# liruiluo/VLA-Adapter

Measured on AMD Instinct MI355X. Metric: fine-tune samples/sec (224px img + 32-tok prompt), adapter-only, fwd+bwd+AdamW, higher is better.
Workload: dtype bf16

## Files before the change

### vla_adapter_amd/csrc/gemm_tn.hip

```cpp
#include <algorithm>
#include "gemm_epilogue.h"
#include "gemm_params.h"

namespace {

constexpr int TBK = 64;
constexpr int TILE_BYTES = TBK * 256;
constexpr int STAGE_BYTES = 2 * TILE_BYTES;
constexpr int LDS_BYTES = 2 * STAGE_BYTES;

struct TnP {
  const bf16_t* A; const bf16_t* B; bf16_t* C; const bf16_t* R; float* ws;
  int M, N1, N2, lda, ldb, ldc, ldr;
  long long sA, sB, sC, sR;
  float alpha;
  int gA, gB; long long sgA, sgB;
  int cgA, cgsA;
  int tiles_n2, ntiles, split, mslice;
};

__device__ __forceinline__ bf16x4 tr_read(const char* p) {
  return __builtin_amdgcn_ds_read_tr16_b64_v4i16((__attribute__((address_space(3))) bf16x4*)p);
}

__device__ __forceinline__ void tn_tile(const TnP& p, const int swz, const int bz, char* smem) {
  const int tid = threadIdx.x, lane = tid & 63;
  const int wid = __builtin_amdgcn_readfirstlane(tid >> 6);
  const int wr = wid >> 2, wc = wid & 3;
  const int b1 = swz / p.tiles_n2, b2 = swz - b1 * p.tiles_n2;
  const int n1_0 = b1 * 128, n2_0 = b2 * 128;
  const int zb = bz / p.split, zs = bz - zb * p.split;
  const int m_begin = zs * p.mslice, m_end = min(p.M, m_begin + p.mslice);
  const int nt = (m_end - m_begin + TBK - 1) / TBK;
  const char* Ab = reinterpret_cast<const char*>(p.A + (long long)zb * p.sA);
  const char* Bb = reinterpret_cast<const char*>(p.B + (long long)zb * p.sB);

  const bool isA = wid < 4;
  const int ld = isA ? p.lda : p.ldb, ncols = isA ? p.N1 : p.N2, c0 = isA ? n1_0 : n2_0;
  const int grp = isA ? p.gA : p.gB;
  const long long sgrp = isA ? p.sgA : p.sgB;
  const char* base = isA ? Ab : Bb;
  int rloc[4];
  long long coff[4];
#pragma unroll
  for (int i = 0; i < 4; ++i) {
    const int qp = (wid & 3) * 4 + i;
    const int r = 4 * qp + (lane >> 4);
    const int f = ((r & 3) << 2) | ((r >> 2) & 3);
    int col = c0 + (((lane & 15) ^ f) << 3);
    col = min(col, ncols - 8);
    if (isA && p.cgA > 0) col = (col / p.cgA) * p.cgsA + col % p.cgA;
    rloc[i] = r;
    coff[i] = (long long)col * 2;
  }
  auto stage = [&](int buf, int t) {
    const int mt = m_begin + t * TBK;
    const long long tb = grouped_row(mt, grp, sgrp, ld);
    const int lim = m_end - 1 - mt;
    char* dst = smem + buf * STAGE_BYTES + (isA ? 0 : TILE_BYTES) + (wid & 3) * 4096;
#pragma unroll
    for (int i = 0; i < 4; ++i) glds16(base + (tb + (long long)min(rloc[i], lim) * ld) * 2 + coff[i], dst + i * 1024);
  };

  const int kq = lane >> 4, qq = (lane >> 2) & 3, pp = lane & 3;
  int fa[4][2], fb[2][2];
#pragma unroll
  for (int e = 0; e < 2; ++e) {
    const int row = 8 * kq + qq + 4 * e, f = (qq << 2) | ((2 * kq + e) & 3);
#pragma unroll
    for (int i = 0; i < 4; ++i) fa[i][e] = 256 * row + ((((wr * 64 + i * 16) >> 3) + (pp >> 1)) ^ f) * 16 + 8 * (pp & 1);
#pragma unroll
    for (int i = 0; i < 2; ++i) fb[i][e] = TILE_BYTES + 256 * row + ((((wc * 32 + i * 16) >> 3) + (pp >> 1)) ^ f) * 16 + 8 * (pp & 1);
  }

  f32x4 acc[2][4];
#pragma unroll
  for (int a = 0; a < 2; ++a)
#pragma unroll
    for (int b = 0; b < 4; ++b) acc[a][b] = f32x4{0.f, 0.f, 0.f, 0.f};

  if (nt > 0) stage(0, 0);
  int buf = 0;
  for (int t = 0; t < nt; ++t) {
    asm volatile("s_waitcnt vmcnt(0)" ::: "memory");
    __builtin_amdgcn_s_barrier();
    asm volatile("" ::: "memory");
    if (t + 1 < nt) stage(buf ^ 1, t + 1);
    const char* sb = smem + buf * STAGE_BYTES;
    const int valid = m_end - (m_begin + t * TBK);
    bf16x8 fm[2][4], fn[2][2];
#pragma unroll
    for (int ks = 0; ks < 2; ++ks) {
#pragma unroll
      for (int i = 0; i < 4; ++i) {
        const bf16x4 lo = tr_read(sb + ks * 8192 + fa[i][0]), hi = tr_read(sb + ks * 8192 + fa[i][1]);
        fm[ks][i] = bf16x8{lo[0], lo[1], lo[2], lo[3], hi[0], hi[1], hi[2], hi[3]};
      }
#pragma unroll
      for (int i = 0; i < 2; ++i) {
        const bf16x4 lo = tr_read(sb + ks * 8192 + fb[i][0]), hi = tr_read(sb + ks * 8192 + fb[i][1]);
        fn[ks][i] = bf16x8{lo[0], lo[1], lo[2], lo[3], hi[0], hi[1], hi[2], hi[3]};
      }
    }
    if (valid < TBK) {
#pragma unroll
      for (int ks = 0; ks < 2; ++ks)
#pragma unroll
        for (int e = 0; e < 8; ++e)
          if (ks * 32 + 8 * kq + e >= valid) {
#pragma unroll
            for (int i = 0; i < 2; ++i) fn[ks][i][e] = 0;
          }
    }
#pragma unroll
    for (int ks = 0; ks < 2; ++ks)
#pragma unroll
      for (int ni = 0; ni < 2; ++ni)
#pragma unroll
        for (int mi = 0; mi < 4; ++mi)
          acc[ni][mi] = __builtin_amdgcn_mfma_f32_16x16x32_bf16(fn[ks][ni], fm[ks][mi], acc[ni][mi], 0, 0, 0);
    buf ^= 1;
  }

  const int w1 = n1_0 + wr * 64, w2 = n2_0 + wc * 32;
  const int lq = lane >> 4, lr = lane & 15;
  if (p.ws != nullptr) {
    float* plane = p.ws + ((long long)bz) * p.N1 * p.N2;
#pragma unroll
    for (int ni = 0; ni < 2; ++ni)
#pragma unroll
      for (int mi = 0; mi < 4; ++mi) {
        const int r = w1 + mi * 16 + lr, c = w2 + ni * 16 + lq * 4;
        if (r < p.N1 && c + 3 < p.N2) *reinterpret_cast<f32x4*>(plane + (long long)r * p.N2 + c) = acc[ni][mi];
      }
    return;
  }
  bf16_t* Cb = p.C + (long long)zb * p.sC;
  const bf16_t* Rb = p.R ? p.R + (long long)zb * p.sR : nullptr;
#pragma unroll
  for (int ni = 0; ni < 2; ++ni)
#pragma unroll
    for (int mi = 0; mi < 4; ++mi) {
      const int r = w1 + mi * 16 + lr, c = w2 + ni * 16 + lq * 4;
      if (r >= p.N1 || c + 3 >= p.N2) continue;
      float v[4];
#pragma unroll
      for (int j = 0; j < 4; ++j) v[j] = acc[ni][mi][j] * p.alpha;
      if (Rb) add_residual4(v, *reinterpret_cast<const uint2*>(Rb + (long long)r * p.ldr + c));
      *reinterpret_cast<uint2*>(Cb + (long long)r * p.ldc + c) = pack4(v);
    }
}

constexpr int T2_HT = 16384;
constexpr int T2_LDS = 8 * T2_HT;

#define TN_MMA_QUADRANT(Q, FN, FM)                                                                             \
  do {                                                                                                         \
    _Pragma("unroll") for (int ks = 0; ks < 2; ++ks)                                                           \
      _Pragma("unroll") for (int ni = 0; ni < 2; ++ni)                                                         \
        _Pragma("unroll") for (int mi = 0; mi < 4; ++mi)                                                       \
          Q[ni][mi] = __builtin_amdgcn_mfma_f32_16x16x32_bf16(FN[ks][ni], FM[ks][mi], Q[ni][mi], 0, 0, 0);     \
  } while (0)

__device__ __forceinline__ void tn256_tile(const TnP& p, const int swz, const int zb, char* smem) {
  const int tid = threadIdx.x, lane = tid & 63;
  const int wid = __builtin_amdgcn_readfirstlane(tid >> 6);
  const int wr = wid >> 2, wc = wid & 3;
  const int b1 = swz / p.tiles_n2, b2 = swz - b1 * p.tiles_n2;
  const int n1_0 = b1 * 256, n2_0 = b2 * 256;
  const int nt = (p.M + TBK - 1) / TBK;
  const char* Ab = reinterpret_cast<const char*>(p.A + (long long)zb * p.sA);
  const char* Bb = reinterpret_cast<const char*>(p.B + (long long)zb * p.sB);

  const int r0 = wid * 8 + (lane >> 4);
  unsigned ca[2][2], cb[2][2];
#pragma unroll
  for (int j = 0; j < 2; ++j) {
    const int r = r0 + 4 * j;
    const int f = ((r & 3) << 2) | ((r >> 2) & 3);
    const int lc = ((lane & 15) ^ f) << 3;
#pragma unroll
    for (int h = 0; h < 2; ++h) {
      int ga = n1_0 + (lc >> 6) * 128 + h * 64 + (lc & 63);
      ga = min(ga, p.N1 - 8);
      if (p.cgA > 0) ga = (ga / p.cgA) * p.cgsA + ga % p.cgA;
      ca[h][j] = (unsigned)ga * 2u;
      const int gb = min(n2_0 + (lc >> 5) * 64 + h * 32 + (lc & 31), p.N2 - 8);
      cb[h][j] = (unsigned)gb * 2u;
    }
  }
  const unsigned wdst = (unsigned)(size_t)((__attribute__((address_space(3))) char*)smem) + wid * 2048;
  auto stage_a = [&](int slot, int h, int t) {
    const int mt = t * TBK;
    const char* base = Ab + grouped_row(mt, p.gA, p.sgA, p.lda) * 2;
    const unsigned lim = (unsigned)(p.M - 1 - mt), ld2 = (unsigned)p.lda * 2u;
    glds16s(base, min((unsigned)r0, lim) * ld2 + ca[h][0], wdst + slot * T2_HT);
    glds16s(base, min((unsigned)r0 + 4u, lim) * ld2 + ca[h][1], wdst + slot * T2_HT + 1024);
  };
  auto stage_b = [&](int slot, int h, int t) {
    const int mt = t * TBK;
    const char* base = Bb + grouped_row(mt, p.gB, p.sgB, p.ldb) * 2;
    const unsigned lim = (unsigned)(p.M - 1 - mt), ld2 = (unsigned)p.ldb * 2u;
    glds16s(base, min((unsigned)r0, lim) * ld2 + cb[h][0], wdst + slot * T2_HT);
    glds16s(base, min((unsigned)r0 + 4u, lim) * ld2 + cb[h][1], wdst + slot * T2_HT + 1024);
  };

  const int kq = lane >> 4, qq = (lane >> 2) & 3, pp = lane & 3;
  int fa[4][2], fb[2][2];
#pragma unroll
  for (int e = 0; e < 2; ++e) {
    const int row = 8 * kq + qq + 4 * e, f = (qq << 2) | ((2 * kq + e) & 3);
#pragma unroll
    for (int i = 0; i < 4; ++i) fa[i][e] = 256 * row + ((((wr * 64 + i * 16) >> 3) + (pp >> 1)) ^ f) * 16 + 8 * (pp & 1);
#pragma unroll
    for (int i = 0; i < 2; ++i) fb[i][e] = 256 * row + ((((wc * 32 + i * 16) >> 3) + (pp >> 1)) ^ f) * 16 + 8 * (pp & 1);
  }
  auto read_a = [&](const char* sb, bf16x8 (&fm)[2][4]) {
#pragma unroll
    for (int ks = 0; ks < 2; ++ks)
#pragma unroll
      for (int i = 0; i < 4; ++i) {
        const bf16x4 lo = tr_read(sb + ks * 8192 + fa[i][0]), hi = tr_read(sb + ks * 8192 + fa[i][1]);
        fm[ks][i] = bf16x8{lo[0], lo[1], lo[2], lo[3], hi[0], hi[1], hi[2], hi[3]};
      }
  };
  auto read_b = [&](const char* sb, bf16x8 (&fn)[2][2]) {
#pragma unroll
    for (int ks = 0; ks < 2; ++ks)
#pragma unroll
      for (int i = 0; i < 2; ++i) {
        const bf16x4 lo = tr_read(sb + ks * 8192 + fb[i][0]), hi = tr_read(sb + ks * 8192 + fb[i][1]);
        fn[ks][i] = bf16x8{lo[0], lo[1], lo[2], lo[3], hi[0], hi[1], hi[2], hi[3]};
      }
  };
  auto mask_tail = [&](bf16x8 (&fn)[2][2], int valid) {
#pragma unroll
    for (int ks = 0; ks < 2; ++ks)
#pragma unroll
      for (int e = 0; e < 8; ++e)
        if (ks * 32 + 8 * kq + e >= valid) {
#pragma unroll
          for (int i = 0; i < 2; ++i) fn[ks][i][e] = 0;
        }
  };

  stage_b(0, 0, 0); stage_a(1, 0, 0); stage_b(2, 1, 0); stage_a(3, 1, 0);
  if (nt > 1) {
    stage_b(4, 0, 1); stage_a(5, 0, 1); stage_b(6, 1, 1);
    asm volatile("s_waitcnt vmcnt(6)" ::: "memory");
  } else {
    asm volatile("s_waitcnt vmcnt(0)" ::: "memory");
  }
  VLA_BARRIER();
  if (wr == 1) VLA_BARRIER();

  f32x4 acc[2][2][2][4];
#pragma unroll
  for (int a = 0; a < 2; ++a)
#pragma unroll
    for (int b = 0; b < 2; ++b)
#pragma unroll
      for (int c = 0; c < 2; ++c)
#pragma unroll
        for (int e = 0; e < 4; ++e) acc[a][b][c][e] = f32x4{0.f, 0.f, 0.f, 0.f};

  bf16x8 fm[2][4], fn0[2][2], fn1[2][2];
  int d = 0;
  for (int t = 0; t < nt; ++t) {
    const char* kb = smem + d * 4 * T2_HT;
    const int so = d * 4, sn = (d ^ 1) * 4;
    const int valid = p.M - t * TBK;
    {
      read_b(kb + 0 * T2_HT, fn0);
      read_a(kb + 1 * T2_HT, fm);
      read_b(kb + 2 * T2_HT, fn1);
      __builtin_amdgcn_sched_barrier(0);
      if (t + 1 < nt) {
        stage_a(sn + 3, 1, t + 1);
        if (t > 0) asm volatile("s_waitcnt vmcnt(8)" ::: "memory");
      } else if (t > 0) {
        asm volatile("s_waitcnt vmcnt(0)" ::: "memory");
      }
      asm volatile("s_waitcnt lgkmcnt(0)" ::: "memory");
      if (valid < TBK) { mask_tail(fn0, valid); mask_tail(fn1, valid); }
      VLA_BARRIER();
      __builtin_amdgcn_s_setprio(1);
      TN_MMA_QUADRANT(acc[0][0], fn0, fm);
      TN_MMA_QUADRANT(acc[0][1], fn1, fm);
      __builtin_amdgcn_s_setprio(0);
      VLA_BARRIER();
    }
    {
      read_a(kb + 3 * T2_HT, fm);
      __builtin_amdgcn_sched_barrier(0);
      if (t + 2 < nt) {
        stage_b(so + 0, 0, t + 2); stage_a(so + 1, 0, t + 2); stage_b(so + 2, 1, t + 2);
        asm volatile("s_waitcnt vmcnt(8)" ::: "memory");
      } else if (t + 1 < nt) {
        asm volatile("s_waitcnt vmcnt(2)" ::: "memory");
      } else {
        asm volatile("s_waitcnt vmcnt(0)" ::: "memory");
      }
      asm volatile("s_waitcnt lgkmcnt(0)" ::: "memory");
      VLA_BARRIER();
      __builtin_amdgcn_s_setprio(1);
      TN_MMA_QUADRANT(acc[1][1], fn1, fm);
      TN_MMA_QUADRANT(acc[1][0], fn0, fm);
      __builtin_amdgcn_s_setprio(0);
      VLA_BARRIER();
    }
    d ^= 1;
  }
  if (wr == 0) VLA_BARRIER();

  const int lq = lane >> 4, lr = lane & 15;
  bf16_t* Cb = p.C + (long long)zb * p.sC;
  const bf16_t* Rb = p.R ? p.R + (long long)zb * p.sR : nullptr;
#pragma unroll
  for (int mh = 0; mh < 2; ++mh)
#pragma unroll
    for (int nh = 0; nh < 2; ++nh)
#pragma unroll
      for (int ni = 0; ni < 2; ++ni)
#pragma unroll
        for (int mi = 0; mi < 4; ++mi) {
          const int r = n1_0 + wr * 128 + mh * 64 + mi * 16 + lr, c = n2_0 + wc * 64 + nh * 32 + ni * 16 + lq * 4;
          if (r >= p.N1 || c + 3 >= p.N2) continue;
          float v[4];
#pragma unroll
          for (int j = 0; j < 4; ++j) v[j] = acc[mh][nh][ni][mi][j] * p.alpha;
          if (Rb) add_residual4(v, *reinterpret_cast<const uint2*>(Rb + (long long)r * p.ldr + c));
          *reinterpret_cast<uint2*>(Cb + (long long)r * p.ldc + c) = pack4(v);
        }
}

__global__ __launch_bounds__(512) void gemm_tn256_kernel(TnP p) {
  extern __shared__ __attribute__((aligned(16))) char smem[];
  tn256_tile(p, xcd_order(blockIdx.x, p.ntiles), blockIdx.z, smem);
}

__global__ __launch_bounds__(512) void gemm_tn_kernel(TnP p) {
  extern __shared__ __attribute__((aligned(16))) char smem[];
  tn_tile(p, xcd_order(blockIdx.x, p.ntiles), blockIdx.z, smem);
}

constexpr int TN_GROUP_MAX = 48;
struct TnG {
  const bf16_t* A; const bf16_t* B; bf16_t* C;
  int M, N1, N2, lda, ldb, ldc, cgA, cgsA;
  float alpha; int tiles_n2;
};
struct TnGroup { TnG g[TN_GROUP_MAX]; int start[TN_GROUP_MAX + 1]; int count, total; };

__global__ __launch_bounds__(512) void gemm_tn_grouped_kernel(TnGroup G) {
  extern __shared__ __attribute__((aligned(16))) char smem[];
  const int t = xcd_order(blockIdx.x, G.total);
  int pi = 0;
  while (pi + 1 < G.count && t >= G.start[pi + 1]) ++pi;
  const TnG& g = G.g[pi];
  TnP p;
  p.A = g.A; p.B = g.B; p.C = g.C; p.R = nullptr; p.ws = nullptr;
  p.M = g.M; p.N1 = g.N1; p.N2 = g.N2; p.lda = g.lda; p.ldb = g.ldb; p.ldc = g.ldc; p.ldr = 0;
  p.sA = p.sB = p.sC = p.sR = 0;
  p.alpha = g.alpha;
  p.gA = p.gB = 0; p.sgA = p.sgB = 0;
  p.cgA = g.cgA; p.cgsA = g.cgsA;
  p.tiles_n2 = g.tiles_n2; p.ntiles = 0; p.split = 1; p.mslice = g.M;
  tn_tile(p, t - G.start[pi], 0, smem);
}

__global__ __launch_bounds__(512) void gemm_tn256_grouped_kernel(TnGroup G) {
  extern __shared__ __attribute__((aligned(16))) char smem[];
  const int t = xcd_order(blockIdx.x, G.total);
  int pi = 0;
  while (pi + 1 < G.count && t >= G.start[pi + 1]) ++pi;
  const TnG& g = G.g[pi];
  TnP p;
  p.A = g.A; p.B = g.B; p.C = g.C; p.R = nullptr; p.ws = nullptr;
  p.M = g.M; p.N1 = g.N1; p.N2 = g.N2; p.lda = g.lda; p.ldb = g.ldb; p.ldc = g.ldc; p.ldr = 0;
  p.sA = p.sB = p.sC = p.sR = 0;
  p.alpha = g.alpha;
  p.gA = p.gB = 0; p.sgA = p.sgB = 0;
  p.cgA = g.cgA; p.cgsA = g.cgsA;
  p.tiles_n2 = g.tiles_n2; p.ntiles = 0; p.split = 1; p.mslice = g.M;
  tn256_tile(p, t - G.start[pi], 0, smem);
}

constexpr int TN256_MIN_TILES = 128;
int tn_forced() {
  const char* e = getenv("VLA_TN_TILE");
  return e != nullptr ? atoi(e) : 0;
}
bool tn_eligible_256(int M, int N1, int N2, int split) { return split <= 1 && M >= 1024 && N1 >= 192 && N2 >= 192; }
long long tn_tiles_256(int N1, int N2) { return (long long)((N1 + 255) / 256) * ((N2 + 255) / 256); }

int tn_slices(int M, int asked) {
  if (asked <= 1) return 1;
  const int per = ((M + asked - 1) / asked + TBK - 1) / TBK * TBK;
  return (M + per - 1) / per;
}
struct TnPlan { int kernel, split; };
TnPlan plan_tn(const vla_gemm_tn_desc* d, int ncu, int forced, bool auto_split) {
  int asked = d->split;
  if (asked <= 1 && auto_split) {
    const long long tiles = (long long)((d->N1 + 127) / 128) * ((d->N2 + 127) / 128) * d->batch;
    asked = tiles * 2 <= ncu && d->M >= 1024 ? (int)std::max(1LL, std::min({16LL, 2 * ncu / tiles, (long long)d->M / 256})) : 1;
  }
  const int split = tn_slices(d->M, asked);
  const bool on256 = split <= 1 && forced != 128 &&
                     (forced == 256 || (tn_eligible_256(d->M, d->N1, d->N2, split) && tn_tiles_256(d->N1, d->N2) * d->batch >= TN256_MIN_TILES));
  return {on256 ? VLA_KERNEL_TN_256 : VLA_KERNEL_TN_128, split};
}

__global__ void tn_finalize_kernel(const float* __restrict__ ws, const bf16_t* __restrict__ R, bf16_t* __restrict__ C, int N1, int N2,
                                   int ldc, int ldr, long long sC, long long sR, float alpha, int split) {
  const long long plane = (long long)N1 * N2, total = plane / 4;
  const int b = blockIdx.y;
  const float* w = ws + (long long)b * split * plane;
  for (long long i = (long long)blockIdx.x * blockDim.x + threadIdx.x; i < total; i += (long long)gridDim.x * blockDim.x) {
    const int r = (int)(i * 4 / N2), c = (int)(i * 4 - (long long)r * N2);
    f32x4 a = *reinterpret_cast<const f32x4*>(w + i * 4);
    for (int s = 1; s < split; ++s) a += *reinterpret_cast<const f32x4*>(w + s * plane + i * 4);
    float v[4];
#pragma unroll
    for (int j = 0; j < 4; ++j) v[j] = a[j] * alpha;
    if (R) add_residual4(v, *reinterpret_cast<const uint2*>(R + b * sR + (long long)r * ldr + c));
    *reinterpret_cast<uint2*>(C + b * sC + (long long)r * ldc + c) = pack4(v);
  }
}

}

extern "C" int vla_gemm_bf16_tn(void* stream, const vla_gemm_tn_desc* d) {
  VLA_REQUIRE(d && d->A && d->B && d->C, "gemm_tn: null operand");
  VLA_REQUIRE(d->M > 0 && d->N1 > 0 && d->N2 > 0 && d->batch > 0, "gemm_tn: empty problem");
  VLA_REQUIRE(d->N1 % 8 == 0 && d->N2 % 8 == 0, "gemm_tn: N1 and N2 must be multiples of 8 (16-B column chunks)");
  VLA_REQUIRE(d->lda % 8 == 0 && d->ldb % 8 == 0 && d->ldc % 4 == 0, "gemm_tn: lda / ldb must be multiples of 8 elements, ldc of 4");
  VLA_REQUIRE(((uintptr_t)d->A & 15) == 0 && ((uintptr_t)d->B & 15) == 0 && ((uintptr_t)d->C & 7) == 0, "gemm_tn: A / B must be 16-B, C 8-B aligned");
  VLA_REQUIRE(d->sA % 8 == 0 && d->sB % 8 == 0 && d->sC % 4 == 0, "gemm_tn: batch strides must keep the alignment");
  VLA_REQUIRE(d->a_group >= 0 && d->b_group >= 0 && d->a_group % 64 == 0 && d->b_group % 64 == 0 && d->a_group_stride % 8 == 0 &&
                  d->b_group_stride % 8 == 0,
              "gemm_tn: contraction-row groups must be multiples of 64 rows (a K-tile never straddles a group) with 16-B aligned strides");
  VLA_REQUIRE(d->a_col_group >= 0 && d->a_col_group % 8 == 0 && d->a_col_group_stride % 8 == 0 &&
                  (d->a_col_group == 0 || d->a_col_group_stride >= d->a_col_group),
              "gemm_tn: column groups on A must be multiples of 8 columns");
  if (d->R) VLA_REQUIRE(((uintptr_t)d->R & 7) == 0 && d->ldr % 4 == 0 && d->sR % 4 == 0, "gemm_tn: R must be 8-B aligned");
  const TnPlan pl = plan_tn(d, vla_num_cus(), tn_forced(), false);
  const int split = pl.split;
  if (split > 1)
    VLA_REQUIRE(d->ws && ((uintptr_t)d->ws & 15) == 0 && d->N2 % 4 == 0, "gemm_tn: split needs an fp32 workspace [batch, split, N1, N2]");
  TnP p;
  p.A = (const bf16_t*)d->A; p.B = (const bf16_t*)d->B; p.C = (bf16_t*)d->C; p.R = (const bf16_t*)d->R;
  p.ws = split > 1 ? d->ws : nullptr;
  p.M = d->M; p.N1 = d->N1; p.N2 = d->N2; p.lda = d->lda; p.ldb = d->ldb; p.ldc = d->ldc; p.ldr = d->ldr;
  p.sA = d->sA; p.sB = d->sB; p.sC = d->sC; p.sR = d->sR;
  p.alpha = d->alpha == 0.f ? 1.f : d->alpha;
  p.gA = d->a_group; p.gB = d->b_group; p.sgA = d->a_group_stride; p.sgB = d->b_group_stride;
  p.cgA = d->a_col_group; p.cgsA = d->a_col_group_stride;
  p.tiles_n2 = (d->N2 + 127) / 128;
  p.ntiles = ((d->N1 + 127) / 128) * p.tiles_n2;
  p.split = split;
  p.mslice = split > 1 ? ((d->M + split - 1) / split + TBK - 1) / TBK * TBK : d->M;
  hipStream_t st = (hipStream_t)stream;
  if (pl.kernel == VLA_KERNEL_TN_256) {
    if (int rc = vla_lds_limit<gemm_tn256_kernel>(T2_LDS, "gemm_tn256_kernel")) return rc;
    p.tiles_n2 = (d->N2 + 255) / 256;
    p.ntiles = ((d->N1 + 255) / 256) * p.tiles_n2;
    hipLaunchKernelGGL(gemm_tn256_kernel, dim3(p.ntiles, 1, d->batch), dim3(512), T2_LDS, st, p);
    VLA_CHECK_LAUNCH("gemm_bf16_tn (256)");
    return VLA_OK;
  }
  if (int rc = vla_lds_limit<gemm_tn_kernel>(LDS_BYTES, "gemm_tn_kernel")) return rc;
  hipLaunchKernelGGL(gemm_tn_kernel, dim3(p.ntiles, 1, d->batch * split), dim3(512), LDS_BYTES, st, p);
  VLA_CHECK_LAUNCH("gemm_bf16_tn");
  if (split > 1) {
    const long long total = (long long)d->N1 * d->N2 / 4;
    const unsigned nblk = (unsigned)((total + 255) / 256 < 1024 ? (total + 255) / 256 : 1024);
    hipLaunchKernelGGL(tn_finalize_kernel, dim3(nblk, d->batch), dim3(256), 0, st, (const float*)d->ws, (const bf16_t*)d->R, (bf16_t*)d->C,
                       d->N1, d->N2, d->ldc, d->ldr, d->sC, d->sR, p.alpha, split);
    VLA_CHECK_LAUNCH("gemm_tn_finalize");
  }
  return VLA_OK;
}

extern "C" int vla_gemm_bf16_tn_grouped(void* stream, const vla_gemm_tn_desc* descs, int count) {
  VLA_REQUIRE(descs && count > 0 && count <= TN_GROUP_MAX, "gemm_tn_grouped: 1 .. 48 problems per launch");
  TnGroup G[2];
  int total[2] = {0, 0}, cnt[2] = {0, 0};
  const int forced = tn_forced();
  long long big = 0;
  for (int i = 0; i < count; ++i)
    if (tn_eligible_256(descs[i].M, descs[i].N1, descs[i].N2, descs[i].split)) big += tn_tiles_256(descs[i].N1, descs[i].N2);
  const bool any256 = forced == 256 || (forced != 128 && big >= TN256_MIN_TILES);
  for (int i = 0; i < count; ++i) {
    const vla_gemm_tn_desc* d = descs + i;
    VLA_REQUIRE(d->A && d->B && d->C && d->M > 0 && d->N1 > 0 && d->N2 > 0, "gemm_tn_grouped: null operand / empty problem");
    VLA_REQUIRE(d->batch == 1 && d->split <= 1 && !d->R && d->a_group == 0 && d->b_group == 0,
                "gemm_tn_grouped: plain problems only (batch 1, no split / addend / row groups)");
    VLA_REQUIRE(d->N1 % 8 == 0 && d->N2 % 8 == 0 && d->lda % 8 == 0 && d->ldb % 8 == 0 && d->ldc % 4 == 0, "gemm_tn_grouped: N1, N2, lda, ldb % 8, ldc % 4");
    VLA_REQUIRE(((uintptr_t)d->A & 15) == 0 && ((uintptr_t)d->B & 15) == 0 && ((uintptr_t)d->C & 7) == 0, "gemm_tn_grouped: alignment");
    VLA_REQUIRE(d->a_col_group >= 0 && d->a_col_group % 8 == 0 && d->a_col_group_stride % 8 == 0 &&
                    (d->a_col_group == 0 || d->a_col_group_stride >= d->a_col_group), "gemm_tn_grouped: bad column groups");
    const int k = (any256 && (forced == 256 || tn_eligible_256(d->M, d->N1, d->N2, d->split))) ? 1 : 0, tile = k ? 256 : 128;
    TnG& g = G[k].g[cnt[k]];
    g.A = (const bf16_t*)d->A; g.B = (const bf16_t*)d->B; g.C = (bf16_t*)d->C;
    g.M = d->M; g.N1 = d->N1; g.N2 = d->N2; g.lda = d->lda; g.ldb = d->ldb; g.ldc = d->ldc;
    g.cgA = d->a_col_group; g.cgsA = d->a_col_group_stride;
    g.alpha = d->alpha == 0.f ? 1.f : d->alpha;
    g.tiles_n2 = (d->N2 + tile - 1) / tile;
    G[k].start[cnt[k]] = total[k];
    total[k] += ((d->N1 + tile - 1) / tile) * g.tiles_n2;
    ++cnt[k];
  }
  for (int k = 1; k >= 0; --k) {
    if (cnt[k] == 0) continue;
    G[k].start[cnt[k]] = total[k];
    G[k].count = cnt[k]; G[k].total = total[k];
    if (k == 1) {
      if (int rc = vla_lds_limit<gemm_tn256_grouped_kernel>(T2_LDS, "gemm_tn256_grouped_kernel")) return rc;
      hipLaunchKernelGGL(gemm_tn256_grouped_kernel, dim3(total[k]), dim3(512), T2_LDS, (hipStream_t)stream, G[k]);
    } else {
      if (int rc = vla_lds_limit<gemm_tn_grouped_kernel>(LDS_BYTES, "gemm_tn_grouped_kernel")) return rc;
      hipLaunchKernelGGL(gemm_tn_grouped_kernel, dim3(total[k]), dim3(512), LDS_BYTES, (hipStream_t)stream, G[k]);
    }
    VLA_CHECK_LAUNCH("gemm_bf16_tn_grouped");
  }
  return VLA_OK;
}

extern "C" int vla_gemm_tn_plan(const vla_gemm_tn_desc* d, int num_cus, int* split) {
  if (!d || d->M <= 0 || d->N1 <= 0 || d->N2 <= 0 || d->batch <= 0) return VLA_ERR_ARG;
  const int ncu = num_cus > 0 ? num_cus : vla_num_cus(), forced = tn_forced();
  if (split) *split = plan_tn(d, ncu, forced, true).split;
  return plan_tn(d, ncu, forced, false).kernel;
}
```

### vla_adapter_amd/engine.py

```python
from __future__ import annotations

import contextlib
import math
import os
from dataclasses import dataclass, field
from typing import Dict, List, Optional, Tuple

import torch

from . import ops, schedule
from .ops import ACT_GELU, ACT_GELU_TANH, ACT_NONE, ACT_RELU, ACT_SWIGLU, BF16
from .schedule import Segment, capture_graph, chunks, turnaround_chunks

NUM_TOKENS = 64
IGNORE_INDEX = -100


def rup(n: int, m: int) -> int:
    return (n + m - 1) // m * m


def copy_flat(dst: torch.Tensor, src: torch.Tensor):
    n = src.numel()
    ops.copy2d(src, dst, 1, n, n, n)


@dataclass
class ViTCfg:
    d: int = 1152
    depth: int = 27
    heads: int = 16
    mlp: int = 4304
    patch: int = 14
    img: int = 224
    n_prefix: int = 0
    layerscale: bool = False
    eps: float = 1e-6
    gelu_tanh: bool = False

    @property
    def n_patches(self):
        return (self.img // self.patch) ** 2

    def as_oracle(self):
        return dict(d=self.d, depth=self.depth, heads=self.heads, mlp=self.mlp, patch=self.patch, n_prefix=self.n_prefix,
                    layerscale=self.layerscale, eps=self.eps, gelu_tanh=self.gelu_tanh)


SIGLIP_SO400M = ViTCfg(1152, 27, 16, 4304, 14, 224, 0, False)
DINOV2_L_REG4 = ViTCfg(1024, 24, 16, 4096, 14, 224, 5, True)


@dataclass
class LLMCfg:
    d: int = 896
    n_layers: int = 24
    heads: int = 14
    kv_heads: int = 2
    dh: int = 64
    inter: int = 4864
    eps: float = 1e-6
    theta: float = 1e6
    vocab: int = 151936

    def as_oracle(self):
        return dict(n_layers=self.n_layers, heads=self.heads, kv_heads=self.kv_heads, dh=self.dh, eps=self.eps, theta=self.theta)


@dataclass
class VLACfg:
    vit: List[ViTCfg] = field(default_factory=lambda: [SIGLIP_SO400M])
    llm: LLMCfg = field(default_factory=LLMCfg)
    n_img: int = 1
    num_blocks: int = 24
    action_dim: int = 7
    chunk: int = 8
    proprio_dim: int = 8
    pro: bool = True

    @property
    def fused(self):
        return len(self.vit) == 2

    @property
    def n_patches(self):
        return self.vit[0].n_patches * self.n_img

    @property
    def vis_dim(self):
        return sum(v.d for v in self.vit)


def config2() -> VLACfg:
    return VLACfg()


def tiny_config() -> VLACfg:
    return VLACfg(vit=[ViTCfg(192, 3, 3, 768, 14, 56, 0, False)],
                  llm=LLMCfg(256, 2, 4, 2, 64, 512, 1e-6, 1e6, 1024), num_blocks=2)


def config5_backbone() -> VLACfg:
    return VLACfg(vit=[DINOV2_L_REG4, SIGLIP_SO400M], llm=LLMCfg(1536, 28, 12, 2, 128, 8960, 1e-6, 1e6, 151936))


def qwen15b_geometry_config(n_layers: int = 2) -> VLACfg:
    return VLACfg(vit=[ViTCfg(192, 3, 3, 768, 14, 56, 0, False)],
                  llm=LLMCfg(1536, n_layers, 12, 2, 128, 8960, 1e-6, 1e6, 1024), num_blocks=n_layers)


def tiny_fused_config() -> VLACfg:
    return VLACfg(vit=[ViTCfg(192, 3, 3, 768, 14, 56, 5, True), ViTCfg(128, 3, 2, 512, 14, 56, 0, False)], n_img=2,
                  llm=LLMCfg(256, 2, 4, 2, 64, 512, 1e-6, 1e6, 1024), num_blocks=2)


def tiny_twin_config() -> VLACfg:
    return VLACfg(vit=[ViTCfg(128, 2, 2, 512, 14, 56, 5, True), ViTCfg(128, 2, 2, 512, 14, 56, 5, False)], n_img=2,
                  llm=LLMCfg(256, 2, 4, 2, 64, 512, 1e-6, 1e6, 1024), num_blocks=2)


def dinosiglip_05b_config(n_img: int = 2) -> VLACfg:
    return VLACfg(vit=[DINOV2_L_REG4, SIGLIP_SO400M], llm=LLMCfg(), n_img=n_img)


def _config5_two_images() -> VLACfg:
    c = config5_backbone()
    c.n_img = 2
    return c


NAMED_CONFIGS = {"config2": config2, "dinosiglip-0_5b": dinosiglip_05b_config, "config5": config5_backbone, "tiny": tiny_config,
                 "tiny_fused": tiny_fused_config, "tiny_twin": tiny_twin_config, "qwen15b-geometry": qwen15b_geometry_config}


class Linear:

    trains_vectors = False
    taps = None
    keep_norm_out = False
    _lane = "M"

    def __init__(self, device):
        self.dev = device
        self.fp8 = False
        self.Q: Dict[str, Tuple[torch.Tensor, torch.Tensor]] = {}
        self._qbuf, self._xq = {}, None

    def _q8_norm(self, x) -> bool:
        return self.fp8

    def _qscratch(self, rows: int, cols: int, slot: str):
        k = (rows, cols, slot, self._lane)
        b = self._qbuf.get(k)
        if b is None:
            b = self._qbuf[k] = (torch.empty(rows, cols, device=self.dev, dtype=torch.uint8), torch.empty(rows, device=self.dev, dtype=torch.float32))
        return b

    def _hand_over(self, y, q, s_):
        h = q if y is None else y
        self._xq = ((h.data_ptr(), tuple(h.shape)), q, s_)
        return h

    def _quant(self, x, slot: str):
        if self._xq is not None and self._xq[0] == (x.data_ptr(), tuple(x.shape)):
            hit, self._xq = self._xq, None
            return hit[1], hit[2]
        q, s_ = self._qscratch(x.shape[0], x.shape[1], slot)
        return ops.quant_fp8_rows(x, q, s_)

    def _ln(self, x, w, b, y, st, eps):
        if not self._q8_norm(x):
            return ops.layernorm_fwd(x, w, b, eps, out=y, stats=st)
        q, s_ = self._qscratch(x.shape[0], x.shape[1], "n")
        y = y if self.keep_norm_out else None
        ops.layernorm_fwd_q8(x, w, b, eps, q, s_, y=y, stats=st)
        return self._hand_over(y, q, s_)

    def _rms(self, x, w, out, rstd, eps):
        if not self._q8_norm(x):
            return ops.rmsnorm_fwd(x, w, eps, out=out, rstd=rstd)
        q, s_ = self._qscratch(x.shape[0], x.shape[1], "n")
        ops.rmsnorm_fwd_q8(x, w, eps, q, s_, rstd=rstd, y=out if self.keep_norm_out else None)
        return self._hand_over(out, q, s_)

    def _lin(self, key, x, W, bias=None, **kw):
        wq = self.Q.get(key)
        if wq is not None:
            xq, xs = self._quant(x, "f")
            return ops.gemm_nt(xq, wq[0], bias=bias, fp8=(xs, wq[1]), **kw)
        return ops.gemm_nt(x, W, bias=bias, **kw)

    def _lin_bwd(self, key, dy, x, WT, out=None, swiglu_gu=None, **kw):
        if swiglu_gu is not None:
            return ops.gemm_swiglu_bwd(dy, WT, swiglu_gu, out=out, **kw)
        return ops.gemm_nt(dy, WT, out=out)


class ViT:

    def __init__(self, cfg: ViTCfg, sd: Dict[str, torch.Tensor], device, j: int = 0):
        self.cfg, self.key = cfg, f"vit{j}."
        self.lin = Linear(device)
        d, P = cfg.d, cfg.patch
        g = lambda k: sd[k].to(device=device, dtype=BF16).contiguous()
        self.kpe = rup(3 * P * P, 64)
        wpe = torch.zeros(d, self.kpe, device=device, dtype=BF16)
        wpe[:, :3 * P * P] = g("patch_embed.proj.weight").reshape(d, -1)
        self.wpe, self.bpe = wpe, g("patch_embed.proj.bias")
        self.pos = g("pos_embed").reshape(-1, d)
        assert self.pos.shape[0] == cfg.n_patches, "pos_embed covers patches only (no_embed_class / no cls token)"
        self.prefix = None
        if cfg.n_prefix:
            toks = [g("cls_token").reshape(1, d)] + ([g("reg_token").reshape(-1, d)] if "reg_token" in sd else [])
            self.prefix = torch.cat(toks, 0)
            assert self.prefix.shape[0] == cfg.n_prefix
        self.mlp_pad = rup(cfg.mlp, 128)
        self.blocks = []
        for i in range(cfg.depth - 1):
            p = f"blocks.{i}."
            w1 = torch.zeros(self.mlp_pad, d, device=device, dtype=BF16)
            w1[:cfg.mlp] = g(p + "mlp.fc1.weight")
            b1 = torch.zeros(self.mlp_pad, device=device, dtype=BF16)
            b1[:cfg.mlp] = g(p + "mlp.fc1.bias")
            w2 = torch.zeros(d, self.mlp_pad, device=device, dtype=BF16)
            w2[:, :cfg.mlp] = g(p + "mlp.fc2.weight")
            wproj, bproj, b2 = g(p + "attn.proj.weight"), g(p + "attn.proj.bias"), g(p + "mlp.fc2.bias")
            blk = dict(n1w=g(p + "norm1.weight"), n1b=g(p + "norm1.bias"), wqkv=g(p + "attn.qkv.weight"),
                       bqkv=g(p + "attn.qkv.bias"), wproj=wproj, bproj=bproj, n2w=g(p + "norm2.weight"),
                       n2b=g(p + "norm2.bias"), w1=w1, b1=b1, w2=w2, b2=b2)
            if cfg.layerscale:
                blk["ls1"], blk["ls2"] = g(p + "ls1.scale_factor"), g(p + "ls2.scale_factor")
            self.blocks.append(blk)
        self.ls_folded = False
        self.fold_layerscale(True)

    def fold_layerscale(self, on: bool):
        if not self.cfg.layerscale or on == self.ls_folded:
            self.ls_folded = on and self.cfg.layerscale
            return
        for b in self.blocks:
            if on:
                ls1, ls2 = b["ls1"].float(), b["ls2"].float()
                b["wproj_f"], b["bproj_f"] = (b["wproj"].float() * ls1[:, None]).to(BF16), (b["bproj"].float() * ls1).to(BF16)
                b["w2_f"], b["b2_f"] = (b["w2"].float() * ls2[:, None]).to(BF16), (b["b2"].float() * ls2).to(BF16)
            else:
                for k in ("wproj_f", "bproj_f", "w2_f", "b2_f"):
                    b.pop(k, None)
        self.ls_folded = on

    def enable_fp8(self):
        for i, b in enumerate(self.blocks):
            self.lin.Q[f"{self.key}{i}.qkv"] = ops.quant_fp8_rows(b["wqkv"])
            self.lin.Q[f"{self.key}{i}.fc1"] = ops.quant_fp8_rows(b["w1"])
        self.lin.fp8 = True

    def forward(self, pixels: torch.Tensor, c0: int, out: Optional[torch.Tensor] = None, lin: Optional[Linear] = None, st=None):
        cfg = self.cfg
        lin = self.lin if lin is None else lin
        Bv, Np, d, T = pixels.shape[0], cfg.n_patches, cfg.d, cfg.n_patches + cfg.n_prefix
        cols = ops.im2col_patch(pixels, c0, cfg.patch, self.kpe)
        x = st["X"][0] if st is not None else torch.empty(Bv * T, d, device=pixels.device, dtype=BF16)
        if cfg.n_prefix:
            pe = ops.gemm_nt(cols, self.wpe, bias=self.bpe, residual=self.pos, res_mod=Np, out=st["pe"] if st is not None else None)
            x3 = x.view(Bv, T, d)
            ops.copy_rows3d(pe, x3[0, cfg.n_prefix:], Bv, Np, d, Np * d, d, T * d, d)
            ops.copy_rows3d(self.prefix, x3, Bv, cfg.n_prefix, d, 0, d, T * d, d)
        else:
            ops.gemm_nt(cols, self.wpe, bias=self.bpe, residual=self.pos, res_mod=Np, out=x)
        if st is not None:
            st["cols"] = cols
        nb = len(self.blocks)
        for i in range(nb):
            if st is not None:
                x = self.block(i, x, lin, st, st["X"][i + 1])
            else:
                x = self.block(i, x, lin, None, out if i == nb - 1 and out is not None else x)
        return x

    def block(self, i: int, x: torch.Tensor, lin: Linear, st, x_out: torch.Tensor) -> torch.Tensor:
        cfg, b, k = self.cfg, self.blocks[i], f"{self.key}{i}."
        d, T = cfg.d, cfg.n_patches + cfg.n_prefix
        Bv = x.shape[0] // T
        keep = lambda name: st[name][i] if st is not None and name in st else None
        sfx = "_f" if self.ls_folded else ""
        h = lin._ln(x, b["n1w"], b["n1b"], keep("H1"), keep("S1"), cfg.eps)
        qkv = lin._lin(k + "qkv", h, b["wqkv"], b["bqkv"], out=keep("QKV")).view(Bv, T, 3 * d)
        a = ops.attn_fwd(qkv[:, :, :d], qkv[:, :, d:2 * d], qkv[:, :, 2 * d:], cfg.heads, cfg.heads, d // cfg.heads, False,
                         out=st["A"][i].view(Bv, T, d) if st is not None else None, lse=keep("LSE")).view(Bv * T, d)
        xm = x if st is None else st["Xm"][i]
        self._residual(lin, k + "proj", a, b["wproj" + sfx], b["bproj" + sfx], b.get("ls1"), x, xm, keep("PA"))
        h = lin._ln(xm, b["n2w"], b["n2b"], keep("H2"), keep("S2"), cfg.eps)
        if st is None:
            m = lin._lin(k + "fc1", h, b["w1"], b["b1"], act=ACT_GELU_TANH if cfg.gelu_tanh else ACT_GELU)
        else:
            m = ops.gelu_fwd(lin._lin(k + "fc1", h, b["w1"], b["b1"], out=st["Mpre"][i]), out=st["Mact"][i])
        self._residual(lin, k + "fc2", m, b["w2" + sfx], b["b2" + sfx], b.get("ls2"), xm, x_out, keep("PM"))
        return x_out

    def _residual(self, lin, key, a, w, bias, ls, x, out, pre):
        if ls is not None and not self.ls_folded:
            ops.layerscale_fwd(lin._lin(key, a, w, bias, out=pre), ls, x, out=out)
        else:
            lin._lin(key, a, w, bias, out=out, residual=x)


class _BufferSets:

    def _track_alloc(self, before: dict):
        names = getattr(self, "_buf_names", set())
        self._buf_names = names | {k for k, v in self.__dict__.items() if k != "_buf_names" and (k not in before or before[k] is not v)}

    def buffer_set(self) -> dict:
        return {k: self.__dict__[k] for k in self._buf_names}

    def bind_buffer_set(self, bufs: dict):
        self.__dict__.update(bufs)


class LLM(_BufferSets):

    def __init__(self, cfg: LLMCfg, sd: Dict[str, torch.Tensor], device):
        self.cfg, self.device = cfg, device
        self.lin = Linear(device)
        D, H, KV, dh, I = cfg.d, cfg.heads, cfg.kv_heads, cfg.dh, cfg.inter
        assert D % 64 == 0 and I % 64 == 0 and (H + 2 * KV) * dh % 64 == 0 and I % 16 == 0
        g = lambda k: sd[k].to(device=device, dtype=BF16).contiguous()
        self.layers = []
        for i in range(cfg.n_layers):
            p = f"layers.{i}."
            wqkv = torch.cat([g(p + "self_attn.q_proj.weight"), g(p + "self_attn.k_proj.weight"), g(p + "self_attn.v_proj.weight")], 0)
            bqkv = torch.cat([g(p + "self_attn.q_proj.bias"), g(p + "self_attn.k_proj.bias"), g(p + "self_attn.v_proj.bias")], 0)
            wg, wu = g(p + "mlp.gate_proj.weight"), g(p + "mlp.up_proj.weight")
            wgu = torch.stack([wg.view(I // 16, 16, D), wu.view(I // 16, 16, D)], 1).reshape(2 * I, D).contiguous()
            wo, wd = g(p + "self_attn.o_proj.weight"), g(p + "mlp.down_proj.weight")
            self.layers.append(dict(n1=g(p + "input_layernorm.weight"), n2=g(p + "post_attention_layernorm.weight"),
                                    wqkv=wqkv.contiguous(), bqkv=bqkv.contiguous(), wo=wo, wgu=wgu, wd=wd,
                                    wqkvT=wqkv.t().contiguous(), woT=wo.t().contiguous(), wguT=wgu.t().contiguous(),
                                    wdT=wd.t().contiguous()))
        self.norm = g("norm.weight")
        self.embed = g("embed_tokens.weight")
        self._buf_key = None
        self.gu_row0 = 0
        self.per_layer, self.norm_grads = False, False
        self._flin = self._blin = self.lin

    def keep_per_layer(self, norm_grads: bool):
        self.per_layer, self.norm_grads = True, norm_grads
        self._buf_key = None

    def _alloc(self, B: int, S: int):
        if self._buf_key == (B, S):
            return
        before = dict(self.__dict__)
        c, dev = self.cfg, self.device
        n, M, D = c.n_layers, B * S, c.d
        W = (c.heads + 2 * c.kv_heads) * c.dh
        e = lambda *s, dt=BF16: torch.empty(*s, device=dev, dtype=dt)
        self.HS = e(n + 2, B, S, D)
        self.X1, self.QKV, self.AO = e(n, M, D), e(n, M, W), e(n, M, c.heads * c.dh)
        self.GU = e(n, M, 2 * c.inter)
        self.LSE = e(n, B, c.heads, S, dt=torch.float32)
        self.R1, self.R2, self.RF = e(n, M, dt=torch.float32), e(n, M, dt=torch.float32), e(M, dt=torch.float32)
        self.nbuf, self.hbuf = e(M, D), e(M, c.inter)
        self.d_a, self.d_b, self.d_gu, self.d_qkv, self.d_n = e(M, D), e(M, D), e(M, 2 * c.inter), e(M, W), e(M, D)
        if self.per_layer:
            self.N1, self.N2, self.Hs = e(n, M, D), e(n, M, D), e(n, M, c.inter)
            self.G_res, self.G_d1, self.G_gu, self.G_qkv = e(n, M, D), e(n, M, D), e(n, M, 2 * c.inter), e(n, M, W)
            self.d_last = e(M, D)
            if self.norm_grads:
                self.G_n1, self.G_n2 = e(n, M, D), e(n, M, D)
        self.cos, self.sin = ops.rope_half_tables(S, c.dh, c.theta, dev)
        self._buf_key = (B, S)
        self._track_alloc(before)

    def out_slot(self, i: int) -> int:
        n = self.cfg.n_layers
        return i + 1 if i < n - 1 else n + 1

    def forward(self, B: int, S: int, kmask_u8: torch.Tensor, keep_from_row: int = 0, n_run: Optional[int] = None):
        self.fwd_begin(B, S, kmask_u8, keep_from_row)
        self.fwd_layers(0, self.cfg.n_layers if n_run is None else n_run)

    def fwd_layers(self, lo: int, hi: int):
        for i in range(lo, hi):
            self.fwd_layer(i)
        if hi == self.cfg.n_layers:
            self.fwd_final()

    def fwd_begin(self, B: int, S: int, kmask_u8: torch.Tensor, keep_from_row: int = 0, lin: Optional[Linear] = None):
        self.kmask, self.B, self.S = kmask_u8, B, S
        self.gu_row0 = keep_from_row
        self._flin = self.lin if lin is None else lin

    def _keeps(self, i: int):
        return (self.N1[i], self.N2[i], self.Hs[i]) if self.per_layer else (self.nbuf, self.nbuf, self.hbuf)

    def _attn_views(self, t3):
        c = self.cfg
        a, b = c.heads * c.dh, (c.heads + c.kv_heads) * c.dh
        return t3[:, :, :a], t3[:, :, a:b], t3[:, :, b:]

    def fwd_layer(self, i: int):
        c, B, S, lin = self.cfg, self.B, self.S, self._flin
        D, H, KV, dh = c.d, c.heads, c.kv_heads, c.dh
        L, k = self.layers[i], f"llm.{i}."
        x, qkv, x1 = self.HS[i].view(-1, D), self.QKV[i], self.X1[i]
        n1, n2, h = self._keeps(i)
        n1 = lin._rms(x, L["n1"], n1, self.R1[i], c.eps)
        if dh in (64, 128):
            lin._lin(k + "qkv", n1, L["wqkv"], L["bqkv"], out=qkv, rope=(1, self.cos, self.sin, S, dh, (H + KV) * dh))
        else:
            lin._lin(k + "qkv", n1, L["wqkv"], L["bqkv"], out=qkv)
            ops.rope_half_(qkv[:, :H * dh], self.cos, self.sin, S, H, dh)
            ops.rope_half_(qkv[:, H * dh:(H + KV) * dh], self.cos, self.sin, S, KV, dh)
        ops.attn_fwd(*self._attn_views(qkv.view(B, S, -1)), H, KV, dh, True, self.kmask, out=self.AO[i].view(B, S, -1), lse=self.LSE[i])
        lin._lin(k + "o", self.AO[i], L["wo"], None, out=x1, residual=x)
        n2 = lin._rms(x1, L["n2"], n2, self.R2[i], c.eps)
        lin._lin(k + "gu", n2, L["wgu"], None, act=ACT_SWIGLU, out=self.GU[i], out2=h, c_live=(S, self.gu_row0) if self.gu_row0 else None)
        lin._lin(k + "down", h, L["wd"], None, out=self.HS[self.out_slot(i)].view(-1, D), residual=x1)

    def fwd_final(self):
        n, D = self.cfg.n_layers, self.cfg.d
        ops.rmsnorm_fwd(self.HS[n + 1].view(-1, D), self.norm, self.cfg.eps, out=self.HS[n].view(-1, D), rstd=self.RF)

    def enable_fp8(self):
        for i, L in enumerate(self.layers):
            self.lin.Q[f"llm.{i}.qkv"] = ops.quant_fp8_rows(L["wqkv"])
            self.lin.Q[f"llm.{i}.gu"] = ops.quant_fp8_rows(L["wgu"])
        self.lin.fp8 = True

    def backward(self, dHS: torch.Tensor, B: int, S: int, row0: int = 0, n_run: Optional[int] = None) -> torch.Tensor:
        n_run = self.cfg.n_layers if n_run is None else n_run
        self.bwd_begin(dHS, row0, n_run)
        for i in range(n_run - 1, -1, -1):
            self.bwd_layer(i, dHS)
        return self.bwd_result()

    def bwd_begin(self, dHS: torch.Tensor, row0: Optional[int] = 0, n_run: Optional[int] = None, lin: Optional[Linear] = None):
        n, S, D = self.cfg.n_layers, self.S, self.cfg.d
        self._n_run = n if n_run is None else n_run
        self._blin = lin = self.lin if lin is None else lin
        if row0 is None:
            self.r0, self.Rl, self._win = 0, S, None
        else:
            assert 0 <= row0 < S and row0 % 32 == 0, "live-row window must start on a multiple of 32"
            assert row0 >= self.gu_row0, "the forward dropped backward-only rows this window needs"
            self.r0, self.Rl = row0, S - row0
            self._win = (self.Rl, S, row0)
        Mr = self.B * self.Rl
        assert tuple(dHS.shape[1:]) == (self.B, self.Rl, D)
        d = (self.G_res[self._n_run - 1] if self.per_layer else self.d_a)[:Mr]
        if self._n_run == n:
            self._d = ops.rmsnorm_bwd(dHS[n].view(Mr, D), self.HS[n + 1].view(-1, D), self.norm, self.RF, out=d, x_rows=self._win)
            if lin.trains_vectors:
                ops.rmsnorm_dw(dHS[n].view(Mr, D), self.HS[n + 1].view(-1, D), self.RF, lin.A("llm.norm"))
        else:
            self._d = ops.copy2d(dHS[self._n_run].view(Mr, D), d, Mr, D, D, D)

    def bwd_layer(self, i: int, dHS: torch.Tensor):
        c, B, S, r0, R, lin = self.cfg, self.B, self.S, self.r0, self.Rl, self._blin
        M, D, H, KV, dh, I = B * S, c.d, c.heads, c.kv_heads, c.dh, c.inter
        Mr, tv, win = B * R, lin.trains_vectors, self._win
        L, k, d = self.layers[i], f"llm.{i}.", self._d
        _, n2, h = self._keeps(i)
        if self.per_layer:
            d1_out, d_out = self.G_d1[i], (self.G_res[i - 1] if i > 0 else self.d_last)[:Mr]
            d_gu, d_qkv = self.G_gu[i][:Mr], self.G_qkv[i][:Mr]
        else:
            d1_out, d_out, d_gu, d_qkv = self.d_b[:Mr], d, self.d_gu[:Mr], self.d_qkv[:Mr]
        if i < self._n_run - 1:
            ops.add_(d, dHS[i + 1].view(Mr, D))
        tap = lin.taps.get(("llm", i)) if lin.taps is not None else None
        if tap is not None:
            tap["d_out"] = d.clone()
        d_gu = lin._lin_bwd(k + "down", d, h, L["wdT"], out=d_gu, swiglu_gu=self.GU[i][r0:], **({"gu_group": (R, S * 2 * I)} if win else {}))
        d_n = lin._lin_bwd(k + "gu", d_gu, n2, L["wguT"], out=self.G_n2[i] if tv else self.d_n[:Mr])
        if tv:
            lin._defer(lambda dy=d_n, x=self.X1[i], r=self.R2[i], acc=lin.A(k + "n2"): ops.rmsnorm_dw(dy, x, r, acc))
        d1 = ops.rmsnorm_bwd(d_n, self.X1[i], L["n2"], self.R2[i], dres=d, out=d1_out, x_rows=win)
        dao = lin._lin_bwd(k + "o", d1, self.AO[i], L["woT"], out=self.d_n[:Mr])
        q, kk, v = self._attn_views(self.QKV[i].view(B, S, -1))
        dq, dk, dv = self._attn_views(d_qkv.view(B, R, -1))
        ops.attn_bwd(dao.view(B, R, -1), q[:, r0:], kk, v, self.AO[i].view(B, S, -1)[:, r0:], self.LSE[i], H, KV, dh, True,
                     self.kmask, dq=dq, dk=dk, dv=dv, rope=(self.cos, self.sin) if dh in (64, 128) else None, row0=r0)
        if dh not in (64, 128):
            cs, sn = self.cos[r0:], self.sin[r0:]
            ops.rope_half_(d_qkv[:, :H * dh], cs, sn, R, H, dh, sign=-1)
            ops.rope_half_(d_qkv[:, H * dh:(H + KV) * dh], cs, sn, R, KV, dh, sign=-1)
        d_n = lin._lin_bwd(k + "qkv", d_qkv, self._keeps(i)[0], L["wqkvT"], out=self.G_n1[i] if tv else self.d_n[:Mr])
        if tv:
            lin._defer(lambda dy=d_qkv, acc=lin.A(k + "bqkv"): ops.colsum_(dy, acc))
            lin._defer(lambda dy=d_n, x=self.HS[i].view(M, D), r=self.R1[i], acc=lin.A(k + "n1"): ops.rmsnorm_dw(dy, x, r, acc))
        self._d = ops.rmsnorm_bwd(d_n, self.HS[i].view(M, D), L["n1"], self.R1[i], dres=d1, out=d_out, x_rows=win)
        if tap is not None:
            tap["d_in"] = self._d.clone()

    def bwd_result(self) -> torch.Tensor:
        return self._d.view(self.B, self.Rl, self.cfg.d)


class FlatParams:

    def __init__(self, spec: List[Tuple[str, Tuple[int, ...]]], device):
        self.offsets, off = {}, 0
        for name, shape in spec:
            n = math.prod(shape)
            self.offsets[name] = (off, shape)
            off += rup(n, 8)
        self.numel = off
        self.data = torch.zeros(off, device=device, dtype=BF16)
        self.grad = torch.zeros(off, device=device, dtype=BF16)
        self.m = torch.zeros(off, device=device, dtype=BF16)
        self.v = torch.zeros(off, device=device, dtype=BF16)

    def view(self, name, buf=None):
        off, shape = self.offsets[name]
        return (self.data if buf is None else buf)[off:off + math.prod(shape)].view(shape)

    def g(self, name):
        return self.view(name, self.grad)


class Head(_BufferSets):

    H = 8

    def __init__(self, cfg: VLACfg, device):
        self.cfg, self.device, self.pro = cfg, device, cfg.pro
        D, nb, Da, Pd = cfg.llm.d, cfg.num_blocks, cfg.action_dim, cfg.proprio_dim
        assert D % 64 == 0 and (D // self.H) % 8 == 0
        self.D, self.nb, self.Din = D, nb, Da * D
        assert self.Din % 64 == 0
        seg = [("w_adp", (nb, 2 * D, D)), ("b_adp", (nb, 2 * D)),
               ("w_task", (nb, 2 * D, D)), ("b_task", (nb, 2 * D))] if cfg.pro else []
        spec = [("w_x", (nb, 3 * D, D)), ("b_x", (nb, 3 * D))] + seg + [
                ("w_o", (nb, D, D)), ("b_o", (nb, D)), ("w_ffn", (nb, D, D)), ("b_ffn", (nb, D)),
                ("ln_w", (nb, D)), ("ln_b", (nb, D)), ("gate", (nb, 8)),
                ("ln1_w", (self.Din,)), ("ln1_b", (self.Din,)), ("fc1_w", (D, self.Din)), ("fc1_b", (D,)),
                ("ln2_w", (D,)), ("ln2_b", (D,)), ("fc2_w", (Da, D)), ("fc2_b", (Da,)),
                ("p_fc1_w", (D, Pd)), ("p_fc1_b", (D,)), ("p_fc2_w", (D, D)), ("p_fc2_b", (D,)),
                ("action_queries", (NUM_TOKENS, D))]
        self.P = FlatParams(spec, device)
        self.film = {}
        z = lambda *s: torch.zeros(*s, device=device, dtype=BF16)
        self.T = dict(w_x=z(nb, D, 3 * D), w_o=z(nb, D, D), w_ffn=z(nb, D, D), p_fc2_w=z(D, D))
        if cfg.pro:
            self.T.update(w_adp=z(nb, D, 2 * D), w_task=z(nb, D, 2 * D))
        self.fc2T = z(D, 64)
        self.pfc1_pad = z(D, 64)
        self.dirty = True
        self._key = None
        self._prep_key = None
        self.rope_tab = None
        self.ref_softmax = bool(int(os.environ.get("VLA_HEAD_REF_SOFTMAX", "0")))

    _BLK_PRO = [("q_proj", "w_x", "b_x", 0), ("k_self", "w_x", "b_x", 1), ("v_self", "w_x", "b_x", 2),
                ("k_adapter", "w_adp", "b_adp", 0), ("v_adapter", "w_adp", "b_adp", 1),
                ("k_task", "w_task", "b_task", 0), ("v_task", "w_task", "b_task", 1),
                ("o_proj", "w_o", "b_o", 0), ("ffn.1", "w_ffn", "b_ffn", 0)]
    _BLK_ORIG = [("q_proj", "w_x", "b_x", 0), ("k_proj", "w_x", "b_x", 1), ("v_proj", "w_x", "b_x", 2),
                 ("o_proj", "w_o", "b_o", 0), ("ffn.1", "w_ffn", "b_ffn", 0)]

    @property
    def _BLK(self):
        return self._BLK_PRO if self.pro else self._BLK_ORIG

    def _kv(self, which: str, i: int):
        D = self.D
        if self.pro:
            return self.P.view("w_" + which)[i], self.P.view("b_" + which)[i], self.T["w_" + which][i]
        return self.P.view("w_x")[i, D:], self.P.view("b_x")[i, D:], self.T["w_x"][i][:, D:]

    def named_views(self, buf=None) -> Dict[str, torch.Tensor]:
        P, D, out = self.P, self.D, {}
        v = lambda n: P.view(n, buf)
        for i in range(self.nb):
            pre = f"model.mlp_resnet_blocks.{i}."
            for name, w, b, k in self._BLK:
                out[pre + name + ".weight"] = v(w)[i, k * D:(k + 1) * D]
                out[pre + name + ".bias"] = v(b)[i, k * D:(k + 1) * D]
            out[pre + "ffn.0.weight"], out[pre + "ffn.0.bias"] = v("ln_w")[i], v("ln_b")[i]
            out[pre + "gating_factor"] = v("gate")[i, :1]
        for a, b in (("model.layer_norm1.weight", "ln1_w"), ("model.layer_norm1.bias", "ln1_b"), ("model.fc1.weight", "fc1_w"),
                     ("model.fc1.bias", "fc1_b"), ("model.layer_norm2.weight", "ln2_w"), ("model.layer_norm2.bias", "ln2_b"),
                     ("model.fc2.weight", "fc2_w"), ("model.fc2.bias", "fc2_b")):
            out[a] = v(b)
        return out

    def proprio_views(self, buf=None):
        v = lambda n: self.P.view(n, buf)
        return {"fc1.weight": v("p_fc1_w"), "fc1.bias": v("p_fc1_b"), "fc2.weight": v("p_fc2_w"), "fc2.bias": v("p_fc2_b")}

    def load_state_dicts(self, head_sd: Dict[str, torch.Tensor], proprio_sd: Dict[str, torch.Tensor],
                         action_queries: Optional[torch.Tensor] = None):
        nv = self.named_views()
        for k, t in nv.items():
            t.copy_(head_sd[k].to(self.device, BF16).reshape(t.shape))
        for k, t in head_sd.items():
            if "film_gen" in k:
                self.film[k] = t.to(self.device, BF16)
        for k, t in self.proprio_views().items():
            t.copy_(proprio_sd[k].to(self.device, BF16))
        if action_queries is not None:
            self.P.view("action_queries").copy_(action_queries.to(self.device, BF16))
        self.dirty = True

    def head_state_dict(self):
        sd = {k: v.clone() for k, v in self.named_views().items()}
        sd.update(self.film)
        return sd

    @property
    def dirty(self) -> bool:
        return self._stale_fwd or self._stale_bwd

    @dirty.setter
    def dirty(self, v: bool):
        self._stale_fwd = self._stale_bwd = bool(v)

    def refresh_forward_operands(self):
        if self._stale_fwd:
            pd = self.cfg.proprio_dim
            ops.copy2d(self.P.view("p_fc1_w"), self.pfc1_pad, self.D, pd, pd, self.pfc1_pad.stride(0))
            self._stale_fwd = False

    def refresh_transposes(self):
        if not self._stale_bwd:
            return
        P = self.P
        for k in (("w_x", "w_adp", "w_task", "w_o", "w_ffn") if self.pro else ("w_x", "w_o", "w_ffn")):
            ops.transpose(P.view(k), out=self.T[k])
        ops.transpose(P.view("p_fc2_w"), out=self.T["p_fc2_w"])
        ops.transpose(P.view("fc2_w"), out=self.fc2T)
        self._stale_bwd = False

    def _alloc(self, B: int, Kt: int):
        if self._key == (B, Kt):
            return
        before = dict(self.__dict__)
        D, nb, T, dev = self.D, self.nb, self.cfg.chunk, self.device
        Ka = NUM_TOKENS + 1
        e = lambda *s, dt=BF16: torch.empty(*s, device=dev, dtype=dt)
        z = lambda *s, dt=BF16: torch.zeros(*s, device=dev, dtype=dt)
        R = B * T
        self.Ka, self.Kt, self.R = Ka, Kt, R
        self.h_adp = e(nb, B, Ka, D)
        self.KV_adp, self.KV_task = e(nb, B * Ka, 2 * D), e(nb, B * Kt, 2 * D)
        self.dKV_adp, self.dKV_task = e(nb, B * Ka, 2 * D), e(nb, B * Kt, 2 * D)
        self.X = e(nb + 1, R, D)
        self.QKVx, self.dQKVx = e(nb, R, 3 * D), e(nb, R, 3 * D)
        self.AOx, self.O2, self.LNo = e(nb, R, D), e(nb, R, D), e(nb, R, D)
        self.dO2, self.dFF = e(nb, R, D), e(nb, R, D)
        self.probs = e(nb, B, self.H, T, T + Ka + Kt, dt=torch.float32)
        self.stats = e(nb, R, 2, dt=torch.float32)
        bkeys = tuple(k for k in ("b_x", "b_adp", "b_task", "b_o", "b_ffn", "fc1_b", "fc2_b", "p_fc1_b", "p_fc2_b") if k in self.P.offsets)
        shapes = [("dgate", (nb,)), ("ln_dw", (nb, D)), ("ln_db", (nb, D)), ("ln1_dw", (self.Din,)), ("ln1_db", (self.Din,)),
                  ("ln2_dw", (D,)), ("ln2_db", (D,)), ("d_pf", (B, D))] + [("b:" + k, tuple(self.P.offsets[k][1])) for k in bkeys]
        self.acc32 = z(sum(rup(math.prod(sh), 4) for _, sh in shapes), dt=torch.float32)
        off, views = 0, {}
        for name, sh in shapes:
            views[name] = self.acc32[off:off + math.prod(sh)].view(sh)
            off += rup(math.prod(sh), 4)
        self.dgate, self.ln_dw, self.ln_db = views["dgate"], views["ln_dw"], views["ln_db"]
        self.ln1_dw, self.ln1_db, self.ln2_dw, self.ln2_db = views["ln1_dw"], views["ln1_db"], views["ln2_dw"], views["ln2_db"]
        self.b_f32 = {k: views["b:" + k] for k in bkeys}
        self.d_pf32 = views["d_pf"]
        self.row_idx_ka = torch.empty(B, Ka, device=dev, dtype=torch.int32)
        self.row_idx_live_ka = torch.empty(B, Ka, device=dev, dtype=torch.int32)
        self._idx_scratch = torch.empty(B, Ka, device=dev, dtype=torch.int32)
        self.guard = torch.zeros(1, device=dev, dtype=torch.float32)
        self.x_in = z(R, self.Din)
        self.pr_in = z(B, 64)
        self.h_task_c = e(nb, B * Kt, D) if Kt % 64 else None
        self.dfc2 = e(64, D)
        self.dpfc1 = e(D, 64)
        self.dh_adp = e(nb, B * Ka, D)
        self.dpad = z(R, 64)
        self.rope_tab = ops.rope_inter_tables(max(T, Ka, Kt), D // self.H, dev)
        self._key = (B, Kt)
        self._prep_key = None
        self._track_alloc(before)

    def forward(self, HS: torch.Tensor, pos1: torch.Tensor, proprio: torch.Tensor, Np: int,
                noise: Optional[torch.Tensor] = None) -> torch.Tensor:
        self.fwd_begin(HS, pos1, proprio, Np, noise)
        for i in range(self.nb):
            self.fwd_layer(i)
        return self.fwd_end()

    def fwd_begin(self, HS, pos1, proprio, Np, noise=None):
        cfg, P = self.cfg, self.P
        B, S = HS.shape[1], HS.shape[2]
        T = cfg.chunk
        self._alloc(B, Np)
        self.refresh_forward_operands()
        self.HSref, self.Np, self.S, self.B, self.pos1 = HS, Np, S, B, pos1
        assert proprio.dim() == 2 and proprio.stride(1) == 1 and proprio.dtype in (BF16, torch.float32)
        ops.copy2d(proprio, self.pr_in, B, cfg.proprio_dim, proprio.stride(0), 64)
        self.pp_pre = ops.gemm_nt(self.pr_in, self.pfc1_pad, bias=P.view("p_fc1_b"))
        self.pp_act = ops.gelu_fwd(self.pp_pre)
        self.pf = ops.gemm_nt(self.pp_act, P.view("p_fc2_w"), bias=P.view("p_fc2_b"))
        ops.head_index_prep(pos1, pos1, pos1, self.row_idx_ka, self._idx_scratch, None, B, S, Np, 0)
        ops.copy2d(self.pf, self.h_adp[0, 0, NUM_TOKENS], self.nb * B, self.D, self.D, self.Ka * self.D, src_mod=B)
        if noise is not None:
            assert tuple(noise.shape) == (T, self.Din) and noise.is_contiguous()
            ops.copy2d(noise, self.x_in, B * T, self.Din, self.Din, self.Din, src_mod=T)
        else:
            ops.zero_(self.x_in)
        self.x_ln, self.st1 = ops.layernorm_fwd(self.x_in, P.view("ln1_w"), P.view("ln1_b"), 1e-5, want_stats=True)
        ops.gemm_nt(self.x_ln, P.view("fc1_w"), bias=P.view("fc1_b"), act=ACT_RELU, out=self.X[0])

    def fwd_layer(self, i: int):
        cfg, P, D, H = self.cfg, self.P, self.D, self.H
        HS, B, S, Kt, Ka, T = self.HSref, self.B, self.S, self.Kt, self.Ka, cfg.chunk
        dh = D // H
        rc, rs_ = self.rope_tab
        hs2 = HS[i + 1].view(B * S, D)
        ops.gather_rows(hs2, self.row_idx_ka.view(-1), self.h_adp[i].view(B * Ka, D))
        fuse = self.pro and D % 64 == 0 and not os.environ.get("VLA_NO_KV_ROPE_FUSE")
        wa, ba, _ = self._kv("adp", i)
        ops.gemm_nt(self.h_adp[i].view(B * Ka, D), wa, bias=ba, out=self.KV_adp[i], rope=(2, rc, rs_, Ka, dh, D) if fuse else None)
        wt, bt, _ = self._kv("task", i)
        ops.gemm_nt(hs2[:B * Kt], wt, bias=bt, out=self.KV_task[i], a_group=(Kt, S * D), bias_post_round=B > 1,
                    rope=(2, rc, rs_, Kt, dh, D) if fuse else None)
        x = self.X[i]
        if self.pro:
            if not fuse:
                ops.rope_inter_(self.KV_adp[i][:, :D], rc, rs_, Ka, H, dh, 0)
                ops.rope_inter_(self.KV_task[i][:, :D], rc, rs_, Kt, H, dh, 0)
            ops.gemm_nt(x, P.view("w_x")[i], bias=P.view("b_x")[i], out=self.QKVx[i], rope=(2, rc, rs_, T, dh, 2 * D))
        else:
            ops.gemm_nt(x, P.view("w_x")[i], bias=P.view("b_x")[i], out=self.QKVx[i])
        self._attn(i, fwd=True)
        ops.gemm_nt(self.AOx[i], P.view("w_o")[i], bias=P.view("b_o")[i], residual=x, out=self.O2[i])
        ops.layernorm_fwd(self.O2[i], P.view("ln_w")[i], P.view("ln_b")[i], 1e-5, out=self.LNo[i], stats=self.stats[i])
        ops.gemm_nt(self.LNo[i], P.view("w_ffn")[i], bias=P.view("b_ffn")[i], act=ACT_RELU, out=self.X[i + 1])

    def fwd_end(self) -> torch.Tensor:
        P, nb = self.P, self.nb
        self.xf_ln, self.st2 = ops.layernorm_fwd(self.X[nb], P.view("ln2_w"), P.view("ln2_b"), 1e-5, want_stats=True)
        self.pred = ops.gemm_nt(self.xf_ln, P.view("fc2_w"), bias=P.view("fc2_b"))
        return self.pred.view(self.B, self.cfg.chunk, self.cfg.action_dim)

    def _attn(self, i: int, fwd: bool, dout=None):
        B, T, D, Ka, Kt, H = self.B, self.cfg.chunk, self.D, self.Ka, self.Kt, self.H
        qkv = self.QKVx[i].view(B, T, 3 * D)
        ka = self.KV_adp[i].view(B, Ka, 2 * D)
        kt = self.KV_task[i].view(B, Kt, 2 * D)
        args = (qkv[:, :, :D], qkv[:, :, D:2 * D], qkv[:, :, 2 * D:], ka[:, :, :D], ka[:, :, D:], kt[:, :, :D], kt[:, :, D:])
        gate = self.P.view("gate")[i]
        out = self.AOx[i].view(B, T, D)
        if fwd:
            ops.head_attn_fwd(*args, gate, H, self.ref_softmax, out=out, probs=self.probs[i])
        else:
            g = self.dQKVx[i].view(B, T, 3 * D)
            ga = self.dKV_adp[i].view(B, Ka, 2 * D)
            gt = self.dKV_task[i].view(B, Kt, 2 * D)
            ops.head_attn_bwd(dout.view(B, T, D), out, *args, gate, self.probs[i], self.dgate[i:i + 1], g[:, :, :D], g[:, :, D:2 * D],
                              g[:, :, 2 * D:], ga[:, :, :D], ga[:, :, D:], gt[:, :, :D], gt[:, :, D:], H,
                              rope=self.rope_tab if self.pro else None)

    def backward(self, dpred: torch.Tensor, dHS: torch.Tensor, row0: int = 0):
        self.prep_backward(self.pos1, self.Np, self.B, self.S, row0)
        self.bwd_begin(dpred, row0)
        for i in range(self.nb - 1, -1, -1):
            self.bwd_layer(i, dHS)
        self.bwd_end()

    def prep_backward(self, pos1: torch.Tensor, Np: int, B: int, S: int, row0: int, pos0=None, cnt0=None):
        self._alloc(B, Np)
        g = self.guard if pos0 is not None else None
        ops.head_index_prep(pos1, pos0 if pos0 is not None else pos1, cnt0 if cnt0 is not None else pos1, self._idx_scratch,
                            self.row_idx_live_ka, g, B, S, Np, row0)
        self._prep_key = (B, S, Np, row0)

    def bwd_begin(self, dpred: torch.Tensor, row0: int = 0):
        cfg, P, nb = self.cfg, self.P, self.nb
        R, Da = self.R, cfg.action_dim
        self.row0 = row0
        assert self._prep_key == (self.B, self.S, self.Np, row0), "prep_backward() first"
        self.refresh_transposes()
        ops.zero_(self.acc32)
        dp = dpred.reshape(R, Da)
        ops.zero_(self.dpad)
        ops.copy2d(dp, self.dpad, R, Da, Da, 64)
        ops.colsum_(dp, self.b_f32["fc2_b"])
        self._dw(self.dpad, self.xf_ln, out=self.dfc2)
        ops.copy2d(self.dfc2, P.g("fc2_w"), Da, self.D, self.D, self.D)
        d_ln2 = ops.gemm_nt(self.dpad, self.fc2T)
        self.dx = ops.layernorm_bwd(d_ln2, self.X[nb], P.view("ln2_w"), self.st2, self.ln2_dw, self.ln2_db)

    def bwd_layer(self, i: int, dHS: torch.Tensor):
        P, D = self.P, self.D
        B, S, Kt, Ka = self.B, self.S, self.Kt, self.Ka
        dff = self.dFF[i]
        ops.relu_bwd(self.dx, self.X[i + 1], out=dff)
        d_ln = ops.gemm_nt(dff, self.T["w_ffn"][i])
        do2 = self.dO2[i]
        ops.layernorm_bwd(d_ln, self.O2[i], P.view("ln_w")[i], self.stats[i], self.ln_dw[i], self.ln_db[i], out=do2)
        d_ao = ops.gemm_nt(do2, self.T["w_o"][i])
        self._attn(i, fwd=False, dout=d_ao)
        self.dx = ops.gemm_nt(self.dQKVx[i], self.T["w_x"][i], residual=do2)
        ops.gemm_nt(self.dKV_adp[i], self._kv("adp", i)[2], out=self.dh_adp[i])
        ops.scatter_add_rows(self.dh_adp[i], self.row_idx_live_ka.view(-1), dHS[i + 1].view(-1, D))
        if self.row0 == 0:
            ops.gemm_nt(self.dKV_task[i], self._kv("task", i)[2], out=dHS[i + 1].view(B * S, D)[:B * Kt], c_group=(Kt, S * D))

    def bwd_end(self):
        cfg, P, D, nb = self.cfg, self.P, self.D, self.nb
        B, Ka = self.B, self.Ka
        G = P.g
        dy1 = ops.relu_bwd(self.dx, self.X[0])
        ops.colsum_(dy1, self.b_f32["fc1_b"])
        self._dw(dy1, self.x_ln, out=G("fc1_w"))
        d_xln = ops.gemm_nt(dy1, self._t(P.view("fc1_w")))
        ops.layernorm_bwd(d_xln, self.x_in, P.view("ln1_w"), self.st1, self.ln1_dw, self.ln1_db, want_dx=False)
        ops.colsum_(self.dh_adp.view(nb, B, Ka, D)[:, :, NUM_TOKENS].transpose(0, 1), self.d_pf32)
        d_pf = ops.cast_f32_bf16(self.d_pf32)
        ops.colsum_(d_pf, self.b_f32["p_fc2_b"])
        self._dw(d_pf, self.pp_act, out=G("p_fc2_w"))
        d_act = ops.gemm_nt(d_pf, self.T["p_fc2_w"])
        d_pre = ops.gelu_bwd(d_act, self.pp_pre)
        ops.colsum_(d_pre, self.b_f32["p_fc1_b"])
        self._dw(d_pre, self.pr_in, out=self.dpfc1)
        ops.copy2d(self.dpfc1, G("p_fc1_w"), D, cfg.proprio_dim, 64, cfg.proprio_dim)
        Kt, S = self.Kt, self.S
        h_adp = self.h_adp.view(nb, B * Ka, D)
        if self.h_task_c is None:
            h_task, tg = self.HSref[1:nb + 1, 0, :Kt], (Kt, S * D)
        else:
            for i in range(nb):
                ops.copy_rows3d(self.HSref[i + 1], self.h_task_c[i], B, Kt, D, S * D, D, Kt * D, D)
            h_task, tg = self.h_task_c, None
        ops.gemm_tn(self.dQKVx, self.X[:nb], out=G("w_x"))
        ops.gemm_tn(self.dO2, self.AOx, out=G("w_o"))
        ops.gemm_tn(self.dFF, self.LNo, out=G("w_ffn"))
        ops.colsum_(self.dQKVx, self.b_f32["b_x"]); ops.colsum_(self.dO2, self.b_f32["b_o"]); ops.colsum_(self.dFF, self.b_f32["b_ffn"])
        if self.pro:
            ops.gemm_tn(self.dKV_adp, h_adp, out=G("w_adp"))
            ops.gemm_tn(self.dKV_task, h_task, out=G("w_task"), rows=B * Kt, b_group=tg)
            ops.colsum_(self.dKV_adp, self.b_f32["b_adp"]); ops.colsum_(self.dKV_task, self.b_f32["b_task"])
        else:
            gkv = G("w_x")[:, self.D:]
            ops.gemm_tn(self.dKV_adp, h_adp, out=gkv, accumulate=True)
            ops.gemm_tn(self.dKV_task, h_task, out=gkv, accumulate=True, rows=B * Kt, b_group=tg)
            bkv = self.b_f32["b_x"][:, self.D:]
            ops.colsum_(self.dKV_adp, bkv); ops.colsum_(self.dKV_task, bkv)
        for k, t in self.b_f32.items():
            ops.cast_f32_bf16(t, out=G(k))
        ops.cast_f32_bf16(self.ln_dw, out=G("ln_w")); ops.cast_f32_bf16(self.ln_db, out=G("ln_b"))
        ops.cast_f32_bf16(self.ln1_dw, out=G("ln1_w")); ops.cast_f32_bf16(self.ln1_db, out=G("ln1_b"))
        ops.cast_f32_bf16(self.ln2_dw, out=G("ln2_w")); ops.cast_f32_bf16(self.ln2_db, out=G("ln2_b"))
        ops.copy2d(self.dgate, G("gate"), nb, 1, 1, 8)

    def _t(self, w2d):
        return ops.transpose(w2d.contiguous())

    def _dw(self, dy, x, out=None):
        return ops.gemm_tn(dy, x, out=out, split=0)


class VLAEngine(schedule.StepControls):

    def __init__(self, cfg: VLACfg, weights: Dict, device="cuda"):
        self.cfg, self.device = cfg, device
        self.vits = [ViT(c, sd, device, j) for j, (c, sd) in enumerate(zip(cfg.vit, weights["vit"]))]
        self.llm = LLM(cfg.llm, weights["llm"], device)
        self.head = Head(cfg, device)
        self.head.load_state_dicts(weights["head"], weights["proprio"], weights.get("action_queries"))
        g = lambda k: weights["proj"][k].to(device=device, dtype=BF16).contiguous()
        self.proj = {k: g(k) for k in weights["proj"]}
        self.step_count = 0
        self._dHS = None
        self.full_llm_backward = bool(int(os.environ.get("VLA_FULL_LLM_BWD", "0")))
        self._row0 = None
        self.reducer = None
        self._init_step_controls(copy_flat, ops.add_)
        self.executed_steps = 0
        self.n_act = min(cfg.llm.n_layers, cfg.num_blocks)
        self.fp8_frozen = False
        self.side = None
        self._vis_bufs = {}
        self._val_pred = None
        self._predict_graphs, self._val_graphs = {}, None
        self._timeline = None
        self._graphs = self._g_vis = self._vis_ev = self._px_copied = self._pending_lr = self._reduced = None
        if os.environ.get("VLA_FP8_FROZEN"):
            self.enable_fp8_frozen()

    def enable_fp8_frozen(self):
        for v in self.vits:
            v.enable_fp8()
        self.llm.enable_fp8()
        self.fp8_frozen = True

    def _grad_buffers(self):
        return [self.head.P.grad]

    def _state_buffers(self):
        return [("head", self.head.P)]

    @property
    def frozen_row0(self) -> Optional[int]:
        return self._row0

    def _set_clip(self, clip):
        self.flush()
        self._clip = clip
        if clip is not None:
            clip.begin(self._clip_ranges())
            self._clip_events = (torch.cuda.Event(), torch.cuda.Event())

    def _clip_ranges(self):
        g, aq_off = self.head.P.grad, self.head.P.offsets["action_queries"][0]
        return [(g, 0, aq_off), (g, aq_off, self.head.P.numel)]

    def forward(self, batch: Dict[str, torch.Tensor], noise: Optional[torch.Tensor] = None, for_training: bool = False):
        self.forward_vlm(batch, for_training)
        return self.head.forward(self.llm.HS, self.pos1, batch["proprio"], self.Np, noise)

    def predict(self, batch: Dict[str, torch.Tensor], latency_hint: Optional[bool] = None) -> torch.Tensor:
        hint = batch["input_ids"].shape[0] == 1 if latency_hint is None else bool(latency_hint)
        key = (tuple(batch["input_ids"].shape), tuple(batch["pixel_values"].shape), batch["pixel_values"].dtype, hint)
        cache = self._predict_graphs
        if os.environ.get("VLA_PREDICT_EAGER"):
            return self.forward(batch, None)
        self._ensure_streams()
        if key not in cache:
            static = {k: v.clone() for k, v in batch.items()}
            with (ops.latency_hint() if hint else contextlib.nullcontext()):
                for _ in range(2):
                    self.forward(static, None)
                torch.cuda.synchronize()
                segs = self._predict_segments(static)
                graphs = schedule.capture(segs, {}, self._cap_stream)
            torch.cuda.synchronize()
            bound = dict(llm=self.llm.buffer_set(), head=self.head.buffer_set(),
                         eng={k: getattr(self, k) for k in ("B", "S", "Np", "feats", "patches", "qidx0", "pos0", "cnt0", "pos1", "cnt1", "_pred_out")},
                         hint=hint)
            cache[key] = (graphs, static, segs, bound)
        graphs, static, segs, bound = cache[key]
        self.llm.bind_buffer_set(bound["llm"])
        self.head.bind_buffer_set(bound["head"])
        self.__dict__.update(bound["eng"])
        for k, v in batch.items():
            static[k].copy_(v)
        self.head.refresh_forward_operands()
        ev = schedule.run(segs, self._stream_of, graphs, timeline=self._timeline)
        torch.cuda.current_stream().wait_event(ev[("end", 0)])
        return self._pred_out

    def _predict_segments(self, batch, noise: Optional[torch.Tensor] = None, loss_of: Optional[torch.Tensor] = None):
        llm, head = self.llm, self.head
        self._vision_begin(batch)
        segs = [Segment(f"V{j}", (lambda j=j: self._vision_backbone(j, batch)), None, ("v", j)) for j in range(len(self.vits))]
        ch = turnaround_chunks(self.n_act, 6, [4, 2], 1)

        def llm_fwd(c, lo, hi):
            if c == 0:
                self._vision_project()
                llm.fwd_begin(self.B, self.S, self._embed(batch), 0)
            llm.fwd_layers(lo, hi)

        def at_end():
            self._pred_out = head.fwd_end()
            if loss_of is not None:
                self._val_pred = self._pred_out
                self._val_loss3 = ops.l1_loss(self._pred_out, self._to_bf16(loss_of), want_grad=False)[0]

        return segs + schedule.pipeline_forward(head, ch, llm_fwd, lambda: (llm.HS, self.pos1, batch["proprio"], self.Np, noise), at_end,
                                                wait=[sg.signal for sg in segs], signal=("end", 0))

    def forward_vlm(self, batch: Dict[str, torch.Tensor], for_training: bool = False, action_queries: bool = True):
        self._vision(batch)
        mm = self._embed(batch, action_queries)
        self.llm.forward(self.B, self.S, mm, self.live_row0() if (for_training and action_queries) else 0,
                         n_run=self.n_act if for_training else None)

    def token_ce(self, labels: torch.Tensor):
        llm, B, S, Np = self.llm, self.B, self.S, self.Np
        n, D = self.cfg.llm.n_layers, self.cfg.llm.d
        W = getattr(llm, "lm_head", None)
        W = llm.embed if W is None else W
        V = W.shape[0]
        assert V % 8 == 0 and tuple(labels.shape) == (B, S - Np)
        logits = ops.gemm_nt(llm.HS[n].view(B * S, D), W, split_k=0).view(B, S, V)
        tgt = torch.full((B, S), IGNORE_INDEX, device=self.device, dtype=torch.int64)
        tgt[:, Np:S - 1] = labels[:, 1:]
        out2 = ops.token_ce(logits, tgt, torch.zeros(2, device=self.device, dtype=torch.float32))
        return out2[0] / out2[1], logits

    def _vision_and_embed(self, batch: Dict[str, torch.Tensor]) -> torch.Tensor:
        self._vision(batch)
        return self._embed(batch)

    def _vision(self, batch: Dict[str, torch.Tensor]):
        self._vision_begin(batch)
        for j in range(len(self.vits)):
            self._vision_backbone(j, batch)
        self._vision_project()

    def _vision_begin(self, batch: Dict[str, torch.Tensor]):
        cfg = self.cfg
        B, L = batch["input_ids"].shape
        Np = cfg.n_patches
        self.llm._alloc(B, L + Np)
        bufs = self._vis_bufs
        if (B, Np) not in bufs:
            bufs[(B, Np)] = (torch.empty(B, Np, cfg.vis_dim, device=self.device, dtype=BF16),
                             torch.empty(B, Np, cfg.llm.d, device=self.device, dtype=BF16))
        self.feats, self.patches = bufs[(B, Np)]
        self.B, self.S, self.Np = B, L + Np, Np

    def _vision_backbone(self, j: int, batch: Dict[str, torch.Tensor]):
        vit = self.vits[j]
        direct = len(self.vits) == 1 and self.cfg.n_img == 1 and vit.cfg.n_prefix == 0
        x = vit.forward(*self._stacked_pixels(j, batch["pixel_values"]), out=self.feats.view(self.B * self.Np, -1) if direct else None)
        if not direct:
            self._scatter_feats(j, x)

    def _stacked_pixels(self, j: int, px: torch.Tensor):
        cfg, nbk = self.cfg, len(self.cfg.vit)
        if cfg.n_img == 1:
            return px, 3 * j
        return torch.cat([px[:, 3 * (im * nbk + j):3 * (im * nbk + j) + 3] for im in range(cfg.n_img)], 0).contiguous(), 0

    def _scatter_feats(self, j: int, x: torch.Tensor):
        cfg, vc, B, feats = self.cfg, self.vits[j].cfg, self.B, self.feats
        npi, T, d, vis = vc.n_patches, vc.n_patches + vc.n_prefix, vc.d, cfg.vis_dim
        col = sum(v.cfg.d for v in self.vits[:j])
        x3 = x.view(-1, T, d)
        for im in range(cfg.n_img):
            ops.copy_rows3d(x3[im * B, vc.n_prefix:], feats[0, im * npi:, col:], B, npi, d, T * d, d, feats.shape[1] * vis, vis)

    def _vision_project(self):
        cfg, B, Np = self.cfg, self.B, self.Np
        f2 = self.feats.view(B * Np, -1)
        h = ops.gemm_nt(f2, self.proj["fc1.weight"], bias=self.proj["fc1.bias"], act=ACT_GELU)
        dst = self.patches.view(B * Np, cfg.llm.d)
        if cfg.fused:
            h = ops.gemm_nt(h, self.proj["fc2.weight"], bias=self.proj["fc2.bias"], act=ACT_GELU)
            ops.gemm_nt(h, self.proj["fc3.weight"], bias=self.proj["fc3.bias"], out=dst)
        else:
            ops.gemm_nt(h, self.proj["fc2.weight"], bias=self.proj["fc2.bias"], out=dst)

    def _embed(self, batch: Dict[str, torch.Tensor], action_queries: bool = True) -> torch.Tensor:
        cfg, llm = self.cfg, self.llm
        ids, labels, am = batch["input_ids"], batch.get("labels"), batch["attention_mask"]
        B, L = ids.shape
        Np = cfg.n_patches
        S = L + Np
        llm._alloc(B, S)
        X0 = llm.HS[0]
        ops.copy2d(self.patches, X0[0, 1], B * Np, cfg.llm.d, cfg.llm.d, cfg.llm.d, d_group=(Np, S * cfg.llm.d))
        if action_queries:
            self.qidx0, self.pos0, self.cnt0 = ops.action_mask(labels, 0)
            _, self.pos1, self.cnt1 = ops.action_mask(labels, 1)
        else:
            self.qidx0 = torch.full((B, L), -1, device=self.device, dtype=torch.int32)
        mm = torch.empty(B, S, device=self.device, dtype=torch.uint8)
        am8 = am.view(torch.uint8) if am.dtype == torch.bool and am.is_contiguous() else am.to(torch.uint8).contiguous()
        ops.embed_splice(ids, am8, self.qidx0, llm.embed, self.head.P.view("action_queries"), X0, mm, Np)
        self.B, self.S, self.Np = B, S, Np
        return mm

    def live_row0(self) -> int:
        if self.full_llm_backward:
            return 0
        first = self.pos0[:, 0]
        if bool((self.cnt0 < 1).any()):
            return 0
        return (self.Np + int(first.min())) // 32 * 32

    def _to_bf16(self, t: torch.Tensor) -> torch.Tensor:
        if t.dtype == BF16:
            return t
        t = t.contiguous()
        out = torch.empty(t.shape, device=t.device, dtype=BF16)
        n = t.shape[-1]
        return ops.copy2d(t, out, t.numel() // n, n, n, n)

    def _dhs(self, row0: int) -> torch.Tensor:
        B, S, D, n = self.B, self.S, self.cfg.llm.d, self.cfg.llm.n_layers
        if self._dHS is None or tuple(self._dHS.shape[1:3]) != (B, S - row0):
            self._dHS = torch.empty(n + 1, B, S - row0, D, device=self.device, dtype=BF16)
        ops.zero_(self._dHS)
        return self._dHS

    def _prep_backward(self, actions, row0: Optional[int] = None):
        frozen = row0 is not None
        self._row0_used = row0 = row0 if frozen else self.live_row0()
        self._dhs(row0)
        self.head.prep_backward(self.pos1, self.Np, self.B, self.S, row0, self.pos0, self.cnt0)
        self._guard = self.head.guard if frozen and row0 else None
        self._actions_bf = self._to_bf16(actions)

    def _turn_around(self, pred, gscale: float) -> torch.Tensor:
        loss3, dpred = ops.l1_loss(pred, self._actions_bf, True, gscale)
        if self._guard is not None:
            ops.add_scalar_f32_(loss3, self._guard)
        self.head.bwd_begin(dpred, self._row0_used)
        return loss3

    def _query_grad(self):
        dq = ops.action_query_grad(self.llm.bwd_result().contiguous(), self.pos0, self.Np, self._row0_used)
        ops.cast_f32_bf16(dq, out=self.head.P.g("action_queries"))

    def loss_and_backward(self, pred, actions, gscale: float = 1.0, exchange: bool = True):
        llm, head = self.llm, self.head
        exchange = exchange and self.reducer is not None
        self._prep_backward(actions)
        loss3 = self._turn_around(pred, gscale)
        for i in range(head.nb - 1, -1, -1):
            head.bwd_layer(i, self._dHS)
        head.bwd_end()
        aq_off = head.P.offsets["action_queries"][0]
        if exchange:
            self.reducer.reduce_async(head.P.grad, 0, aq_off)
        llm.backward(self._dHS, self.B, self.S, self._row0_used, n_run=self.n_act)
        self._query_grad()
        if exchange:
            self.reducer.reduce_async(head.P.grad, aq_off, None)
        return loss3

    def optimizer_step(self, lr: float, beta1=0.9, beta2=0.999, eps=1e-8, wd=0.01):
        self._apply_update(lr, beta1, beta2, eps, wd, two_stream=False, join=False)

    def train_step(self, batch, lr: float, noise=None):
        self.executed_steps += 1
        pred = self.forward(batch, noise, for_training=True)
        loss3 = self.loss_and_backward(pred, batch["actions"], 1.0 / self.ga, exchange=self.ga == 1)
        if self._accum.fold():
            if self.ga > 1 and self.reducer is not None:
                self.reducer.reduce_async(self.head.P.grad, 0, None)
            self.optimizer_step(lr)
        return loss3

    def _ensure_streams(self):
        if self.side is None:
            self.side = torch.cuda.Stream()
            self._cap_main = torch.cuda.Stream()
            self.vis_stream = torch.cuda.Stream()
            self._vstreams = [self.vis_stream] + [torch.cuda.Stream() for _ in range(max(0, len(self.vits) - 1))]

    def _segments(self, batch, noise):
        llm, head = self.llm, self.head
        n = self.n_act
        fch = turnaround_chunks(n, 4, [2, 1, 1], 1)
        if os.environ.get("VLA_FWD_CHUNKS"):
            fch = chunks(n, [int(x) for x in os.environ["VLA_FWD_CHUNKS"].split(",")])

        def llm_fwd(c, lo, hi):
            if c == 0:
                mm = self._embed(batch)
                self._prep_backward(batch["actions"], self._row0)
                llm.fwd_begin(self.B, self.S, mm, self._row0_used)
            llm.fwd_layers(lo, hi)

        def turn_around():
            self._loss3 = self._turn_around(head.fwd_end(), 1.0 / self.ga)

        def llm_bwd(k, lo, hi):
            if k == 0:
                llm.bwd_begin(self._dHS, self._row0_used, n)
            for i in range(hi - 1, lo - 1, -1):
                llm.bwd_layer(i, self._dHS)
            if k == len(fch) - 1:
                self._query_grad()

        return (schedule.pipeline_forward(head, fch, llm_fwd, lambda: (llm.HS, self.pos1, batch["proprio"], self.Np, noise), turn_around,
                                          refresh=True)
                + schedule.pipeline_backward(head, fch, llm_bwd, lambda: self._dHS)
                + [Segment("H", head.bwd_end, None, ("end", 0))])

    def _stream_of(self, name: str, main):
        return main if name == "M" else self.side if name == "H" else self._vstreams[int(name[1:])]

    def _cap_stream(self, name: str):
        return self._cap_main if name == "M" else self._stream_of(name, None)

    def _fwd_bwd(self, batch, noise, vision: bool = True):
        self.executed_steps += 1
        if vision:
            self._vision(batch)
        torch.cuda.current_stream().wait_event(schedule.run(self._segments(batch, noise), self._stream_of)[("end", 0)])
        return self._loss3

    def capture(self, batch: Dict[str, torch.Tensor], noise: Optional[torch.Tensor] = None, warmup: int = 2,
                conservative_rows: bool = False, row0: Optional[int] = None):
        self._ensure_streams()
        self._static_batch, self._static_noise = batch, noise
        self._row0 = None
        self._vision_and_embed(batch)
        self._row0 = self.live_row0()
        if conservative_rows and not self.full_llm_backward:
            self._row0 = min(self._row0, (self.cfg.n_patches + 1) // 32 * 32)
        if row0 is not None:
            assert 0 <= int(row0) < self.S and int(row0) % 32 == 0, f"row0 {row0}: a multiple of 32 inside the sequence"
            self._row0 = int(row0)
        for _ in range(warmup):
            self.head.dirty = True
            self._fwd_bwd(batch, noise)
        torch.cuda.synchronize()
        self.head.dirty = True
        self._next_px = batch["pixel_values"].clone()
        self._px_stage = batch["pixel_values"].clone()
        self._g_vis = capture_graph(lambda: self._vision(dict(batch, pixel_values=self._px_stage)), torch.cuda.graph_pool_handle(),
                                    self.vis_stream)
        self._vis_ev = None
        self._segs = self._segments(batch, noise)
        self._graphs = schedule.capture(self._segs, {}, self._cap_stream)
        torch.cuda.synchronize()
        self._pending_lr = None
        m_fwd = [k for k, sg in enumerate(self._segs) if sg.stream == "M" and sg.signal is not None and sg.signal[0] == "f"]
        self._vis_after = m_fwd[min(len(m_fwd) - 1, max(0, int(os.environ.get("VLA_VIS_AFTER", len(m_fwd) - 4))))]
        assert self._segs[self._vis_after].signal is not None
        self._launch_vision()

    def stage_next_pixels(self, pixel_values: torch.Tensor):
        if self._px_copied is not None:
            torch.cuda.current_stream().wait_event(self._px_copied)
        self._next_px.copy_(pixel_values)

    def _launch_vision(self, after_event=None):
        V, cur = self.vis_stream, torch.cuda.current_stream()
        if after_event is not None:
            V.wait_event(after_event)
        else:
            V.wait_stream(cur)
        tl = self._timeline
        with torch.cuda.stream(V):
            if tl is not None:
                t0 = torch.cuda.Event(enable_timing=True)
                t0.record(V)
            copy_flat(self._px_stage, self._next_px)
            self._px_copied = torch.cuda.Event()
            self._px_copied.record(V)
            self._g_vis.replay()
            self._vis_ev = torch.cuda.Event(enable_timing=tl is not None)
            self._vis_ev.record(V)
            if tl is not None:
                tl.append(("V", -1, t0, self._vis_ev))

    def train_step_pipelined(self, batch, lr: float, noise=None):
        self._ensure_streams()
        loss3 = self._fwd_bwd(batch, noise)
        if self.reducer is not None:
            self.reducer.reduce_async(self.head.P.grad, 0, None)
        self.optimizer_step(lr)
        return loss3

    def train_step_graphed(self, lr: float):
        cur = torch.cuda.current_stream()
        self.executed_steps += 1
        self.flush(join=False)
        cur.wait_event(self._vis_ev)
        def after(k, seg, ev):
            if k == self._vis_after:
                self._launch_vision(ev)
        self._h_end = schedule.run(self._segs, self._stream_of, self._graphs, after=after,
                                   timeline=self._timeline)[("end", 0)]
        cur.wait_event(self._px_copied)
        if self.ga > 1:
            cur.wait_event(self._h_end)
            if not self._accum.fold():
                return self._loss3
            self._h_end = torch.cuda.Event()
            self._h_end.record(cur)
        if self.reducer is not None:
            aq_off = self.head.P.offsets["action_queries"][0]
            ev_aq = self.reducer.reduce_async(self.head.P.grad, aq_off, None)
            ev_head = self.reducer.reduce_async(self.head.P.grad, 0, aq_off, after_event=self._h_end)
            self._reduced = (ev_aq, ev_head)
        self._pending_lr = lr
        return self._loss3

    def flush(self, join: bool = True):
        if self._pending_lr is None:
            return
        lr, self._pending_lr = self._pending_lr, None
        self._apply_update(lr, two_stream=True, join=join)

    def _apply_update(self, lr: float, beta1=0.9, beta2=0.999, eps=1e-8, wd=0.01, *, two_stream: bool, join: bool):
        cur, P, clip = torch.cuda.current_stream(), self.head.P, self._clip
        hs = self.side if two_stream else cur
        aq_off = P.offsets["action_queries"][0]
        assert aq_off + rup(math.prod(P.offsets["action_queries"][1]), 8) == P.numel, "action_queries must close the flat buffer"
        self.step_count += 1
        gscale = 1.0
        if self.reducer is not None:
            ev_aq, ev_head = self._reduced or (None, None)
            if ev_aq is not None and ev_head is not None:
                cur.wait_event(ev_aq)
                hs.wait_event(ev_head)
                self.reducer.joined()
            else:
                self.reducer.wait(*((cur, hs) if two_stream else (cur,)))
            self._reduced = None
            gscale = self.reducer.grad_scale
        if two_stream and self.ga > 1:
            hs.wait_event(self._h_end)
        if clip is not None:
            r_head, r_aq = self._clip_ranges()
            head_summed, finalised = self._clip_events
            clip.begin([r_head, r_aq])
            with torch.cuda.stream(hs):
                clip.sumsq(*r_head, gscale)
                head_summed.record(hs)
            clip.sumsq(*r_aq, gscale)
            cur.wait_event(head_summed)
            clip.finalise()
            finalised.record(cur)
            hs.wait_event(finalised)

        def adam(sl):
            args = (self.step_count, lr, beta1, beta2, eps, wd)
            if clip is None:
                ops.adamw_(P.data[sl], P.grad[sl], P.m[sl], P.v[sl], *args, gscale=gscale)
            else:
                ops.adamw_clipped_(P.data[sl], P.grad[sl], P.m[sl], P.v[sl], clip.coef, *args, gscale=gscale)
        with torch.cuda.stream(hs):
            adam(slice(None, aq_off))
            side_done = torch.cuda.Event()
            side_done.record()
        adam(slice(aq_off, None))
        if join:
            cur.wait_event(side_done)
        self.head.dirty = True

    def begin_validation(self):
        self.flush()
        if self._vis_ev is not None:
            torch.cuda.current_stream().wait_event(self._vis_ev)
        self.head.refresh_forward_operands()

    def end_validation(self):
        if self._g_vis is not None:
            self._launch_vision()

    def val_forward(self, batch: Dict[str, torch.Tensor], noise: Optional[torch.Tensor] = None) -> torch.Tensor:
        pred = self._val_pred = self.forward(batch, noise)
        return ops.l1_loss(pred, self._to_bf16(batch["actions"]), want_grad=False)[0]

    @property
    def val_pred(self) -> torch.Tensor:
        return self._val_pred.view(self.B, self.cfg.chunk, self.cfg.action_dim)

    def val_step_graphed(self, batch: Dict[str, torch.Tensor], noise: Optional[torch.Tensor] = None) -> torch.Tensor:
        self._ensure_streams()

        def make():
            segs = self._predict_segments(batch, noise, loss_of=batch["actions"])
            return schedule.capture(segs, {}, self._cap_stream), segs

        def replay(graphs, segs):
            self.head.refresh_forward_operands()
            torch.cuda.current_stream().wait_event(schedule.run(segs, self._stream_of, graphs)[("end", 0)])
        return schedule.captured_validation(self, batch, noise, make, replay)
```

### vla_adapter_amd/native.py

```python
from __future__ import annotations

import ctypes as C
import os

_HERE = os.path.dirname(os.path.abspath(__file__))
LIB_PATH = (os.environ.get("VLA_NATIVE_LIB") or None) or os.path.join(_HERE, "libvla_native.so")

ACT_NONE, ACT_GELU, ACT_RELU, ACT_GELU_TANH, ACT_SWIGLU, ACT_SWIGLU_BWD = 0, 1, 2, 3, 4, 5
KERNEL_NT_SKINNY, KERNEL_NT_64x128_S6, KERNEL_NT_128x128_S4, KERNEL_NT_128x128, KERNEL_NT_128x64, KERNEL_NT_256 = 0, 8, 9, 10, 11, 12
KERNEL_TN_128, KERNEL_TN_256 = 16, 17
ABI_VERSION = 8


class NativeLibraryMissing(ImportError):
    pass


class GemmDesc(C.Structure):
    _fields_ = [("A", C.c_void_p), ("B", C.c_void_p), ("C", C.c_void_p), ("bias", C.c_void_p), ("R", C.c_void_p),
                ("C2", C.c_void_p),
                ("M", C.c_int), ("N", C.c_int), ("K", C.c_int), ("lda", C.c_int), ("ldb", C.c_int), ("ldc", C.c_int),
                ("ldr", C.c_int), ("ldc2", C.c_int), ("res_mod", C.c_int), ("act", C.c_int), ("batch", C.c_int),
                ("sA", C.c_longlong), ("sB", C.c_longlong), ("sC", C.c_longlong), ("sR", C.c_longlong),
                ("sC2", C.c_longlong), ("sBias", C.c_longlong), ("alpha", C.c_float),
                ("a_group", C.c_int), ("c_group", C.c_int), ("a_group_stride", C.c_longlong), ("c_group_stride", C.c_longlong),
                ("rope_mode", C.c_int), ("rope_T", C.c_int), ("rope_dh", C.c_int), ("rope_cols", C.c_int),
                ("rope_cos", C.c_void_p), ("rope_sin", C.c_void_p),
                ("r_group", C.c_int), ("r_group_stride", C.c_longlong), ("c_live_mod", C.c_int), ("c_live_from", C.c_int),
                ("split_k", C.c_int), ("ws", C.c_void_p), ("bias_post_round", C.c_int),
                ("fp8", C.c_int), ("a_scale", C.c_void_p), ("b_scale", C.c_void_p),
                ("A2", C.c_void_p), ("B2", C.c_void_p), ("K2", C.c_int), ("lda2", C.c_int), ("ldb2", C.c_int)]


class GemmTnDesc(C.Structure):
    _fields_ = [("A", C.c_void_p), ("B", C.c_void_p), ("C", C.c_void_p), ("R", C.c_void_p),
                ("M", C.c_int), ("N1", C.c_int), ("N2", C.c_int), ("lda", C.c_int), ("ldb", C.c_int), ("ldc", C.c_int),
                ("ldr", C.c_int), ("batch", C.c_int),
                ("sA", C.c_longlong), ("sB", C.c_longlong), ("sC", C.c_longlong), ("sR", C.c_longlong), ("alpha", C.c_float),
                ("a_group", C.c_int), ("b_group", C.c_int), ("a_group_stride", C.c_longlong), ("b_group_stride", C.c_longlong),
                ("a_col_group", C.c_int), ("a_col_group_stride", C.c_int), ("split", C.c_int), ("ws", C.c_void_p)]


class AttnDesc(C.Structure):
    _fields_ = [("q", C.c_void_p), ("k", C.c_void_p), ("v", C.c_void_p), ("o", C.c_void_p), ("lse", C.c_void_p),
                ("kmask", C.c_void_p),
                ("q_sb", C.c_longlong), ("k_sb", C.c_longlong), ("v_sb", C.c_longlong), ("o_sb", C.c_longlong),
                ("q_ss", C.c_int), ("k_ss", C.c_int), ("v_ss", C.c_int), ("o_ss", C.c_int),
                ("B", C.c_int), ("Sq", C.c_int), ("Sk", C.c_int), ("Hq", C.c_int), ("Hkv", C.c_int), ("dh", C.c_int),
                ("causal", C.c_int), ("scale", C.c_float),
                ("dout", C.c_void_p), ("dq", C.c_void_p), ("dk", C.c_void_p), ("dv", C.c_void_p), ("delta", C.c_void_p),
                ("do_sb", C.c_longlong), ("dq_sb", C.c_longlong), ("dk_sb", C.c_longlong), ("dv_sb", C.c_longlong),
                ("do_ss", C.c_int), ("dq_ss", C.c_int), ("dk_ss", C.c_int), ("dv_ss", C.c_int),
                ("rope_cos", C.c_void_p), ("rope_sin", C.c_void_p),
                ("q_off", C.c_int), ("dkv_k0", C.c_int), ("lse_hs", C.c_int)]


class HeadAttnDesc(C.Structure):
    _fields_ = [("q", C.c_void_p), ("k_self", C.c_void_p), ("v_self", C.c_void_p), ("k_adp", C.c_void_p),
                ("v_adp", C.c_void_p), ("k_task", C.c_void_p), ("v_task", C.c_void_p), ("gate", C.c_void_p),
                ("out", C.c_void_p), ("probs", C.c_void_p),
                ("B", C.c_int), ("T", C.c_int), ("Ka", C.c_int), ("Kt", C.c_int), ("H", C.c_int), ("dh", C.c_int),
                ("ld_q", C.c_int), ("ld_self", C.c_int), ("ld_adp", C.c_int), ("ld_task", C.c_int), ("ld_out", C.c_int),
                ("gate_on_adapter", C.c_int),
                ("dout", C.c_void_p), ("dq", C.c_void_p), ("dk_self", C.c_void_p), ("dv_self", C.c_void_p),
                ("dk_adp", C.c_void_p), ("dv_adp", C.c_void_p), ("dk_task", C.c_void_p), ("dv_task", C.c_void_p),
                ("dgate", C.c_void_p), ("rope_cos", C.c_void_p), ("rope_sin", C.c_void_p),
                ("ws", C.c_void_p), ("ws_floats", C.c_longlong), ("ref_softmax", C.c_int)]


_P, _I, _L, _F, _D = C.c_void_p, C.c_int, C.c_longlong, C.c_float, C.c_double
_PROTOS = {
    "vla_version": ([], _I),
    "vla_desc_size": ([_I], _I),
    "vla_gemm256_extent_ok": ([C.POINTER(GemmDesc)], _I),
    "vla_gemm_nt_plan": ([C.POINTER(GemmDesc), _I, _I, C.POINTER(C.c_int)], _I),
    "vla_gemm_tn_plan": ([C.POINTER(GemmTnDesc), _I, C.POINTER(C.c_int)], _I),
    "vla_gemm_latency_hint": ([C.c_int], _I),
    "vla_gemm_bf16_tn": ([_P, C.POINTER(GemmTnDesc)], _I),
    "vla_gemm_bf16_tn_grouped": ([_P, C.POINTER(GemmTnDesc), _I], _I),
    "vla_copy_rows3d": ([_P, _P, _P, _I, _I, _I, _L, _L, _L, _L], _I),
    "vla_layerscale_fwd": ([_P, _P, _P, _P, _P, _L, _I], _I),
    "vla_layerscale_bwd": ([_P, _P, _P, _P, _P, _P, _I, _I], _I),
    "vla_gemm_bf16_nt": ([_P, C.POINTER(GemmDesc)], _I),
    "vla_transpose_bf16": ([_P, _P, _P, _I, _I, _I, _I, _I, _L, _L], _I),
    "vla_layernorm_fwd": ([_P, _P, _P, _P, _P, _P, _I, _I, _I, _I, _F], _I),
    "vla_layernorm_bwd": ([_P, _P, _P, _P, _P, _P, _P, _P, _I, _I, _I, _I, _I], _I),
    "vla_rmsnorm_fwd": ([_P, _P, _P, _P, _P, _I, _I, _F], _I),
    "vla_rmsnorm_bwd": ([_P, _P, _P, _P, _P, _P, _P, _I, _I, _I, _I, _I], _I),
    "vla_attn_fwd": ([_P, C.POINTER(AttnDesc)], _I),
    "vla_attn_bwd": ([_P, C.POINTER(AttnDesc)], _I),
    "vla_rope_half": ([_P, _P, _P, _P, _I, _I, _I, _I, _I, _I], _I),
    "vla_rope_interleaved": ([_P, _P, _P, _P, _I, _I, _I, _I, _I, _I], _I),
    "vla_im2col_patch": ([_P, _P, _P, _I, _I, _I, _I, _I, _I, _I, _I], _I),
    "vla_image_normalize_u8": ([_P, _P, _P, _I, _I, _I, _I, _I, C.POINTER(C.c_float), C.POINTER(C.c_float), _I], _I),
    "vla_action_tokenize": ([_P, _P, _P, _P, _L, _I, _F, _F, _L], _I),
    "vla_action_mask": ([_P, _P, _P, _P, _P, _I, _I, _I], _I),
    "vla_embed_splice": ([_P, _P, _P, _P, _P, _P, _P, _P, _I, _I, _I, _I, _I], _I),
    "vla_action_query_grad": ([_P, _P, _P, _P, _I, _I, _I, _I, _I], _I),
    "vla_gather_rows": ([_P, _P, _P, _P, _I, _I, _I, _I], _I),
    "vla_scatter_add_rows": ([_P, _P, _P, _P, _I, _I, _I, _I], _I),
    "vla_add_bf16": ([_P, _P, _P, _P, _L], _I),
    "vla_gelu_fwd": ([_P, _P, _P, _L], _I),
    "vla_gelu_bwd": ([_P, _P, _P, _P, _L], _I),
    "vla_relu_bwd": ([_P, _P, _P, _P, _L], _I),
    "vla_swiglu_bwd": ([_P, _P, _P, _P, _I, _I], _I),
    "vla_swiglu_fwd": ([_P, _P, _P, _I, _I], _I),
    "vla_colsum_bf16": ([_P, _P, _P, _I, _I, _I, _I, _L, _L], _I),
    "vla_cast_f32_bf16": ([_P, _P, _P, _L], _I),
    "vla_cast_bf16_f32": ([_P, _P, _P, _L], _I),
    "vla_rmsnorm_dw": ([_P, _P, _P, _P, _P, _I, _I], _I),
    "vla_embed_grad": ([_P, _P, _P, _P, _P, _I, _I, _I, _I, _I], _I),
    "vla_resample_u8": ([_P, _P, _P, _L, _I, _I, _I, _P, _P, _I], _I),
    "vla_augment_slab_floats": ([_I, _I, _I], _L),
    "vla_augment_stats": ([_P, _P, _P, _P, _I, _I, _I, _I, C.c_uint, C.POINTER(C.c_float), C.c_ulonglong, _L, _L], _I),
    "vla_augment_apply": ([_P, _P, _P, _P, _P, _P, _I, _I, _I, _I, _I, C.POINTER(C.c_float), C.POINTER(C.c_float), _I, C.c_uint,
                           C.POINTER(C.c_float), C.c_ulonglong, _L, _L], _I),
    "vla_token_ce": ([_P, _P, _L, _P, _I, _I, _P], _I),
    "vla_token_ce_bwd": ([_P, _P, _L, _P, _I, _I, _P, _F, _P, _L], _I),
    "vla_token_ce_metrics": ([_P, _P, _L, _P, _P, _I, _I, _P, _P, _P, _L, _I], _I),
    "vla_token_metrics_finish": ([_P, _P, _D, _P], _I),
    "vla_token_row_class": ([_P, _P, _P, _I, _I, _I, _L, _I], _I),
    "vla_copy2d": ([_P, _P, _P, _L, _I, _L, _L, _I, _I, _I, _I, _L], _I),
    "vla_fill_zero": ([_P, _P, _L], _I),
    "vla_dropout_bf16": ([_P, _P, _P, _L, C.c_int, _L, _L, C.c_float, C.c_ulonglong, _P], _I),
    "vla_dropout_bwd_add_bf16": ([_P, _P, _P, _L, C.c_int, _L, _L, C.c_float, C.c_ulonglong, _P], _I),
    "vla_inc_i32": ([_P, _P], _I),
    "vla_quant_fp8_rows": ([_P, _P, _P, _P, _I, _I, _I, _I], _I),
    "vla_rmsnorm_fwd_q8": ([_P, _P, _P, _P, _P, _P, _P, _I, _I, _I, _F], _I),
    "vla_layernorm_fwd_q8": ([_P, _P, _P, _P, _P, _P, _P, _P, _I, _I, _I, _I, _I, _F], _I),
    "vla_head_index_prep": ([_P, _P, _P, _P, _P, _P, _P, _I, _I, _I, _I], _I),
    "vla_add_scalar_f32": ([_P, _P, _P, _I], _I),
    "vla_head_attn_fwd": ([_P, C.POINTER(HeadAttnDesc)], _I),
    "vla_head_attn_bwd": ([_P, C.POINTER(HeadAttnDesc)], _I),
    "vla_l1_loss": ([_P, _P, _P, _P, _P, _I, _I, _I, _F], _I),
    "vla_adamw_bf16": ([_P, _P, _P, _P, _P, _L, _D, _D, _D, _D, _D, _I, _I, _F], _I),
    "vla_adamw_clipped_bf16": ([_P, _P, _P, _P, _P, _L, _D, _D, _D, _D, _D, _I, _I, _F, _P], _I),
    "vla_grad_sumsq_slots": ([_L], _L),
    "vla_grad_sumsq": ([_P, _P, _L, _I, _F, _P], _I),
    "vla_grad_norm_finalise": ([_P, _P, _L, _F, _P], _I),
    "vla_normalize_bounds": ([_P, _P, _P, _L, _I, _P, _P, _P, _P], _I),
    "vla_collate_tokens": ([_P, _P, _P, _L, _P, _P, _P, _P, _P, _I, _I, _I, _I, _F, _F, _L, _L, _L, _I, C.c_ulonglong, _L, _L], _I),
}
ABI_SYMBOLS = sorted(list(_PROTOS) + ["vla_last_error"])


SERVE_PROTOS = {
    "vla_serve_tokens": ([_P, _P, _P, _L, _P, _P, _P, _P, _P, _I, _I, _I, _L, _L, _L, _L, _L], _I),
    "vla_normalize_proprio_serve": ([_P, _P, _I, _P, _L, _I, _P, _P, _P], _I),
    "vla_unnormalize_actions": ([_P, _P, _P, _I, _I, _I, _I, _I, _P, _P, _P, _P], _I),
    "vla_serve_gather_hidden": ([_P, _P, _P, _P, _I, _I, _I, _I, _I, _L, _I], _I),
}
SERVE_SYMBOLS = sorted(SERVE_PROTOS)

EPISODE_PROTOS = {
    "vla_episode_sample": ([_P, _P, _P, _P, _I, C.c_ulonglong, _L, _L, _L, _I, _I, _P, _P, _P], _I),
    "vla_episode_gather": ([_P, _P, _P, _P, _P, _P, _P, _P, _P, _P, _P, _P, _P, _P, _I, _I, _L, _L, _I, _I, _I, _L, _I], _I),
}
EPISODE_SYMBOLS = sorted(EPISODE_PROTOS)

MIXTURE_PROTOS = {
    "vla_mixture_sample": ([_P, _P, _P, _P, _P, _P, _I, _I, C.c_ulonglong, _L, _L, _L, _I, _I, _P, _P, _P, _P], _I),
    "vla_normalize_bounds_rows": ([_P, _P, _P, _L, _I, _I, _P, _I, _P, _P, _P, _P], _I),
}
MIXTURE_SYMBOLS = sorted(MIXTURE_PROTOS)

HELDOUT_PROTOS = {
    "vla_heldout_sweep": ([_P, _P, _P, _P, _P, _I, _I, _L, _L, _L, _L, _I, _I, _P, _P, _P, _P, _P], _I),
    "vla_heldout_l1_accumulate": ([_P, _P, _P, _P, _P, _I, _I, _I, _I, _P, _P], _I),
}
HELDOUT_SYMBOLS = sorted(HELDOUT_PROTOS)

DIGEST_PROTOS = {
    "vla_state_digest_slots": ([], _I),
    "vla_state_digest": ([_P, _P, _L, C.c_ulonglong, _P, _L, _P], _I),
    "vla_token_ce_metrics_ordered": ([_P, _P, _L, _P, _P, _I, _I, _P, _P, _P, _L, _I, _P], _I),
}
DIGEST_SYMBOLS = sorted(DIGEST_PROTOS)

_lib = None


def load():
    global _lib
    if _lib is not None:
        return _lib
    if not os.path.exists(LIB_PATH):
        raise NativeLibraryMissing(
            f"{LIB_PATH} not found: build it with `python -c 'import __graft_entry__ as g; g.build()'` "
            f"(or `make -C {os.path.join(_HERE, 'csrc')}`).  There is no CPU/PyTorch fallback.")
    lib = C.CDLL(LIB_PATH)
    for name, (args, res) in list(_PROTOS.items()) + list(SERVE_PROTOS.items()) + list(EPISODE_PROTOS.items()) + list(MIXTURE_PROTOS.items()) + list(HELDOUT_PROTOS.items()) + list(DIGEST_PROTOS.items()):
        fn = getattr(lib, name, None)
        if fn is None:
            raise NativeLibraryMissing(f"{LIB_PATH} does not export {name}: it was built from an older source tree, rebuild (make -C csrc)")
        fn.argtypes, fn.restype = args, res
    lib.vla_last_error.argtypes, lib.vla_last_error.restype = [], C.c_char_p
    if lib.vla_version() != ABI_VERSION:
        raise NativeLibraryMissing(f"{LIB_PATH} speaks ABI {lib.vla_version()}, this binding ABI {ABI_VERSION}: rebuild (make -C csrc)")
    for which, st in enumerate((GemmDesc, AttnDesc, HeadAttnDesc, GemmTnDesc)):
        if lib.vla_desc_size(which) != C.sizeof(st):
            raise NativeLibraryMissing(f"{LIB_PATH}: sizeof({st.__name__}) is {lib.vla_desc_size(which)} in the library, {C.sizeof(st)} in the binding")
    _lib = lib
    return lib


class NativeError(RuntimeError):
    pass


def check(rc: int, what: str = ""):
    if rc != 0:
        msg = load().vla_last_error().decode(errors="replace")
        raise NativeError(f"libvla_native: {what} failed with code {rc}: {msg}")
```

### vla_adapter_amd/ops.py

```python
from __future__ import annotations

import ctypes as C
import math
from typing import Optional, Tuple

import torch

from . import native as N
from .native import ACT_GELU, ACT_GELU_TANH, ACT_NONE, ACT_RELU, ACT_SWIGLU, ACT_SWIGLU_BWD

BF16 = torch.bfloat16


def _lib():
    return N.load()


def _st():
    return C.c_void_p(torch.cuda.current_stream().cuda_stream)


def _p(t: Optional[torch.Tensor]):
    return None if t is None else C.c_void_p(t.data_ptr())


def _chk_bf16(*ts):
    for t in ts:
        if t is not None:
            assert t.is_cuda and t.dtype == BF16, f"expected CUDA bf16 tensor, got {t.device} {t.dtype}"


def gemm_nt(a: torch.Tensor, b: torch.Tensor, *, bias=None, residual=None, res_mod: int = 0, act: int = ACT_NONE,
            out: Optional[torch.Tensor] = None, out2: Optional[torch.Tensor] = None, alpha: float = 1.0,
            want_pre: bool = True, a_group=None, c_group=None, r_group=None, rope=None, c_live=None,
            split_k: Optional[int] = None, bias_post_round: bool = False, fp8=None, ext=None, query_256: bool = False,
            query_plan: bool = False):
    if fp8 is not None:
        assert a.dtype == torch.uint8 and b.dtype == torch.uint8 and a.dim() == 2 and split_k in (None, 0, 1)
        _chk_bf16(bias, residual, out, out2)
        split_k = 0
    else:
        _chk_bf16(a, b, bias, residual, out, out2)
    assert a.stride(-1) == 1 and b.stride(-1) == 1
    batched = a.dim() == 3
    if batched:
        nb, M, K = a.shape
        sA = a.stride(0)
        sB = b.stride(0) if b.dim() == 3 else 0
        Nn = b.shape[-2]
    else:
        nb, (M, K), sA, sB, Nn = 1, a.shape, 0, 0, b.shape[0]
    assert b.shape[-1] == K, f"K mismatch {a.shape} x {b.shape}"
    d = N.GemmDesc()
    d.A, d.B = a.data_ptr(), b.data_ptr()
    d.M, d.N, d.K, d.lda, d.ldb, d.batch = M, Nn, K, a.stride(-2), b.stride(-2), nb
    d.sA, d.sB, d.act, d.alpha, d.res_mod = sA, sB, act, alpha, res_mod
    shape = (nb, M, Nn) if batched else (M, Nn)
    if act == ACT_SWIGLU:
        if out is None and want_pre:
            out = torch.empty(shape, device=a.device, dtype=BF16)
        hshape = shape[:-1] + (Nn // 2,)
        if out2 is None:
            out2 = torch.empty(hshape, device=a.device, dtype=BF16)
        assert out2.shape == hshape and out2.stride(-1) == 1
        d.C2, d.ldc2, d.sC2 = out2.data_ptr(), out2.stride(-2), (out2.stride(0) if batched else 0)
    elif out is None:
        out = torch.empty(shape, device=a.device, dtype=BF16)
    if out is not None:
        assert tuple(out.shape) == tuple(shape) and out.stride(-1) == 1, f"out shape {out.shape} != {shape}"
        d.C, d.ldc, d.sC = out.data_ptr(), out.stride(-2), (out.stride(0) if batched else 0)
    if bias is not None:
        assert bias.shape[-1] == Nn and bias.stride(-1) == 1
        d.bias = bias.data_ptr()
        d.sBias = bias.stride(0) if bias.dim() == 2 else 0
    if residual is not None:
        assert residual.stride(-1) == 1 and residual.shape[-1] == Nn
        assert res_mod > 0 or r_group is not None or tuple(residual.shape) == tuple(shape)
        d.R, d.ldr = residual.data_ptr(), residual.stride(-2)
        d.sR = residual.stride(0) if (batched and residual.dim() == 3) else 0
    if a_group is not None:
        d.a_group, d.a_group_stride = a_group
    if c_group is not None:
        d.c_group, d.c_group_stride = c_group
    if r_group is not None:
        d.r_group, d.r_group_stride = r_group
    if c_live is not None:
        d.c_live_mod, d.c_live_from = c_live
    if rope is not None:
        mode, cos_t, sin_t, T, dh, ncols = rope
        assert cos_t.dtype == torch.float32 and cos_t.is_contiguous() and sin_t.is_contiguous() and cos_t.shape[0] >= T
        assert cos_t.shape[1] == (dh // 2 if mode == 1 else dh)
        d.rope_mode, d.rope_T, d.rope_dh, d.rope_cols = mode, T, dh, ncols
        d.rope_cos, d.rope_sin = cos_t.data_ptr(), sin_t.data_ptr()
    if fp8 is not None:
        sa, sb = fp8
        assert sa.dtype == torch.float32 and sb.dtype == torch.float32 and sa.numel() == M and sb.numel() == Nn and sa.is_contiguous() and sb.is_contiguous()
        d.fp8, d.a_scale, d.b_scale = 1, sa.data_ptr(), sb.data_ptr()
    if ext is not None:
        a2, b2 = ext
        _chk_bf16(a2, b2)
        assert not batched and a2.dim() == 2 and b2.dim() == 2 and a2.shape[0] == M and b2.shape[0] == Nn and a2.shape[1] == b2.shape[1]
        assert a2.stride(1) == 1 and b2.stride(1) == 1 and a2.shape[1] % 64 == 0 and split_k in (None, 0, 1)
        d.A2, d.B2, d.K2, d.lda2, d.ldb2 = a2.data_ptr(), b2.data_ptr(), a2.shape[1], a2.stride(0), b2.stride(0)
        split_k = 0
    if bias_post_round:
        assert bias is not None
        d.bias_post_round = 1
    if split_k is None and not batched and K >= 2048:
        split_k = _nt_plan(d)[1]
    if split_k and split_k > 1:
        d.split_k, d.ws = split_k, _splitk_ws(split_k * M * Nn, a.device).data_ptr()
    if query_plan or query_256:
        plan = _nt_plan(d)
        return plan if query_plan else plan[0] == N.KERNEL_NT_256
    N.check(_lib().vla_gemm_bf16_nt(_st(), C.byref(d)), "gemm_bf16_nt")
    if act == ACT_SWIGLU:
        return out, out2
    return out


def _nt_plan(d) -> Tuple[int, int]:
    split = C.c_int(0)
    kernel = _lib().vla_gemm_nt_plan(C.byref(d), -1, 0, C.byref(split))
    N.check(min(kernel, 0), "gemm_nt_plan")
    return kernel, split.value


def gemm_plan(a: torch.Tensor, b: torch.Tensor, **kw) -> Tuple[int, int]:
    return gemm_nt(a, b, query_plan=True, **kw)


class latency_hint:

    def __enter__(self):
        self.prev = _lib().vla_gemm_latency_hint(1)
        return self

    def __exit__(self, *exc):
        _lib().vla_gemm_latency_hint(self.prev)
        return False


_SPLITK_WS = {}


def _splitk_ws(numel: int, device) -> torch.Tensor:
    key = (torch.cuda.current_stream().cuda_stream, str(device))
    ws = _SPLITK_WS.get(key)
    if ws is None or ws.numel() < numel:
        ws = _SPLITK_WS[key] = torch.empty(max(numel, 8 << 20), device=device, dtype=torch.float32)
    return ws


def gemm_swiglu_bwd(d: torch.Tensor, w_downT: torch.Tensor, gu: torch.Tensor, out: Optional[torch.Tensor] = None,
                    gu_group=None, ext=None, fp8=None, query_plan: bool = False):
    if fp8 is not None:
        assert ext is not None and d.dtype == torch.uint8 and w_downT.dtype == torch.uint8
        _chk_bf16(gu, out)
    else:
        _chk_bf16(d, w_downT, gu, out)
    M, K = d.shape
    I = w_downT.shape[0]
    assert gu.shape[-1] == 2 * I and gu.stride(-1) == 1 and w_downT.shape[1] == K
    assert gu_group is not None or gu.shape[0] == M
    if out is None:
        out = torch.empty(M, 2 * I, device=d.device, dtype=BF16)
    assert out.shape == (M, 2 * I)
    desc = N.GemmDesc()
    desc.A, desc.B, desc.C, desc.R = d.data_ptr(), w_downT.data_ptr(), out.data_ptr(), gu.data_ptr()
    desc.M, desc.N, desc.K, desc.lda, desc.ldb, desc.ldc, desc.ldr, desc.batch = M, I, K, d.stride(0), w_downT.stride(0), out.stride(0), gu.stride(0), 1
    desc.act, desc.alpha = ACT_SWIGLU_BWD, 1.0
    if gu_group is not None:
        desc.r_group, desc.r_group_stride = gu_group
    if ext is not None:
        a2, b2 = ext
        _chk_bf16(a2, b2)
        assert a2.shape == (M, b2.shape[1]) and b2.shape[0] == I and a2.stride(1) == 1 and b2.stride(1) == 1 and a2.shape[1] % 64 == 0
        desc.A2, desc.B2, desc.K2, desc.lda2, desc.ldb2 = a2.data_ptr(), b2.data_ptr(), a2.shape[1], a2.stride(0), b2.stride(0)
    if fp8 is not None:
        sa, sb = fp8
        assert sa.dtype == torch.float32 and sb.dtype == torch.float32 and sa.numel() == M and sb.numel() == I and sa.is_contiguous() and sb.is_contiguous()
        desc.fp8, desc.a_scale, desc.b_scale = 1, sa.data_ptr(), sb.data_ptr()
    if query_plan:
        return _nt_plan(desc)
    N.check(_lib().vla_gemm_bf16_nt(_st(), C.byref(desc)), "gemm_bf16_nt(swiglu_bwd)")
    return out


_TN_WS = {}


def gemm_tn(a: torch.Tensor, b: torch.Tensor, *, out: Optional[torch.Tensor] = None, alpha: float = 1.0, accumulate: bool = False,
            a_group=None, b_group=None, a_cols=None, rows: Optional[int] = None, split: Optional[int] = None) -> torch.Tensor:
    _chk_bf16(a, b, out)
    assert a.stride(-1) == 1 and b.stride(-1) == 1 and a.dim() == b.dim()
    batched = a.dim() == 3
    nb = a.shape[0] if batched else 1
    M = rows if rows is not None else a.shape[-2]
    assert rows is not None or b.shape[-2] == M
    N1, N2 = a.shape[-1], b.shape[-1]
    d = N.GemmTnDesc()
    a_ptr = a.data_ptr()
    if a_cols is not None:
        N1, cg, cgs, off = a_cols
        assert cg % 8 == 0 and cgs % 8 == 0 and off % 8 == 0
        d.a_col_group, d.a_col_group_stride = cg, cgs
        a_ptr += off * 2
    shape = (nb, N1, N2) if batched else (N1, N2)
    if out is None:
        assert not accumulate
        out = torch.empty(shape, device=a.device, dtype=BF16)
    assert tuple(out.shape) == shape and out.stride(-1) == 1, f"out shape {tuple(out.shape)} != {shape}"
    d.A, d.B, d.C = a_ptr, b.data_ptr(), out.data_ptr()
    d.M, d.N1, d.N2, d.lda, d.ldb, d.ldc, d.batch = M, N1, N2, a.stride(-2), b.stride(-2), out.stride(-2), nb
    d.sA, d.sB, d.sC = (a.stride(0), b.stride(0), out.stride(0)) if batched else (0, 0, 0)
    d.alpha = alpha
    if accumulate:
        d.R, d.ldr, d.sR = out.data_ptr(), out.stride(-2), d.sC
    if a_group is not None:
        d.a_group, d.a_group_stride = a_group
    if b_group is not None:
        d.b_group, d.b_group_stride = b_group
    if split is None and M >= 1024:
        split_c = C.c_int(0)
        N.check(min(_lib().vla_gemm_tn_plan(C.byref(d), 0, C.byref(split_c)), 0), "gemm_tn_plan")
        split = split_c.value
    if split and split > 1:
        key = (torch.cuda.current_stream().cuda_stream, str(a.device))
        need = nb * split * N1 * N2
        ws = _TN_WS.get(key)
        if ws is None or ws.numel() < need:
            ws = _TN_WS[key] = torch.empty(max(need, 4 << 20), device=a.device, dtype=torch.float32)
        d.split, d.ws = split, ws.data_ptr()
    N.check(_lib().vla_gemm_bf16_tn(_st(), C.byref(d)), "gemm_bf16_tn")
    return out


TN_GROUP_MAX = 48


def tn_problem(a: torch.Tensor, b: torch.Tensor, out: torch.Tensor, alpha: float = 1.0, a_cols=None) -> "N.GemmTnDesc":
    _chk_bf16(a, b, out)
    assert a.dim() == 2 and b.dim() == 2 and a.stride(1) == 1 and b.stride(1) == 1 and out.stride(1) == 1 and a.shape[0] == b.shape[0]
    d = N.GemmTnDesc()
    N1, a_ptr = a.shape[1], a.data_ptr()
    if a_cols is not None:
        N1, cg, cgs, off = a_cols
        d.a_col_group, d.a_col_group_stride = cg, cgs
        a_ptr += off * 2
    assert tuple(out.shape) == (N1, b.shape[1]), f"out shape {tuple(out.shape)} != {(N1, b.shape[1])}"
    d.A, d.B, d.C = a_ptr, b.data_ptr(), out.data_ptr()
    d.M, d.N1, d.N2, d.lda, d.ldb, d.ldc, d.batch, d.alpha = a.shape[0], N1, b.shape[1], a.stride(0), b.stride(0), out.stride(0), 1, alpha
    d._keep = (a, b, out)
    return d


def gemm_tn_grouped(problems):
    for i in range(0, len(problems), TN_GROUP_MAX):
        chunk = problems[i:i + TN_GROUP_MAX]
        arr = (N.GemmTnDesc * len(chunk))(*chunk)
        N.check(_lib().vla_gemm_bf16_tn_grouped(_st(), arr, len(chunk)), "gemm_bf16_tn_grouped")


def copy_rows3d(src: torch.Tensor, dst: torch.Tensor, groups: int, rows: int, cols: int, s_sg: int, s_sr: int, d_sg: int, d_sr: int):
    _chk_bf16(src, dst)
    N.check(_lib().vla_copy_rows3d(_st(), _p(src), _p(dst), groups, rows, cols, s_sg, s_sr, d_sg, d_sr), "copy_rows3d")
    return dst


def layerscale_fwd(a: torch.Tensor, ls: torch.Tensor, x: torch.Tensor, out: Optional[torch.Tensor] = None) -> torch.Tensor:
    _chk_bf16(a, ls, x, out)
    assert a.is_contiguous() and x.is_contiguous() and a.shape == x.shape and ls.numel() == a.shape[-1]
    out = torch.empty_like(x) if out is None else out
    N.check(_lib().vla_layerscale_fwd(_st(), _p(a), _p(ls), _p(x), _p(out), a.numel() // a.shape[-1], a.shape[-1]), "layerscale_fwd")
    return out


def layerscale_bwd(dy: torch.Tensor, a: Optional[torch.Tensor], ls: torch.Tensor, dls_f32: Optional[torch.Tensor] = None,
                   out: Optional[torch.Tensor] = None) -> torch.Tensor:
    _chk_bf16(dy, a, ls, out)
    assert dy.is_contiguous() and (a is None or (a.is_contiguous() and a.shape == dy.shape))
    out = torch.empty_like(dy) if out is None else out
    N.check(_lib().vla_layerscale_bwd(_st(), _p(dy), _p(a), _p(ls), _p(out), _p(dls_f32), dy.numel() // dy.shape[-1], dy.shape[-1]), "layerscale_bwd")
    return out


def transpose(x: torch.Tensor, ld_out: Optional[int] = None, out: Optional[torch.Tensor] = None) -> torch.Tensor:
    _chk_bf16(x, out)
    assert x.stride(-1) == 1
    batched = x.dim() == 3
    nb = x.shape[0] if batched else 1
    R, Cc = x.shape[-2:]
    ld = ld_out or R
    if out is None:
        shape = (nb, Cc, ld) if batched else (Cc, ld)
        out = torch.empty(shape, device=x.device, dtype=BF16)
        if ld != R:
            zero_(out)
    N.check(_lib().vla_transpose_bf16(_st(), _p(x), _p(out), R, Cc, x.stride(-2), out.stride(-2), nb,
                                      x.stride(0) if batched else 0, out.stride(0) if batched else 0), "transpose")
    return out


def layernorm_fwd(x, w, b, eps: float, want_stats: bool = False, out=None, stats=None):
    _chk_bf16(x, w, b)
    cols = x.shape[-1]
    x2 = x.reshape(-1, cols)
    assert x2.stride(-1) == 1
    y = torch.empty_like(x2) if out is None else out
    if want_stats and stats is None:
        stats = torch.empty(x2.shape[0], 2, device=x.device, dtype=torch.float32)
    N.check(_lib().vla_layernorm_fwd(_st(), _p(x2), _p(w), _p(b), _p(y), _p(stats), x2.shape[0], cols, x2.stride(0),
                                     y.stride(0), eps), "layernorm_fwd")
    return (y.view(x.shape), stats) if want_stats else y.view(x.shape)


def layernorm_bwd(dy, x, w, stats, dw: Optional[torch.Tensor] = None, db: Optional[torch.Tensor] = None,
                  want_dx: bool = True, out=None):
    _chk_bf16(dy, x, w)
    cols = x.shape[-1]
    x2, dy2 = x.reshape(-1, cols), dy.reshape(-1, cols)
    dx = out if out is not None else torch.empty_like(x2) if want_dx else None
    N.check(_lib().vla_layernorm_bwd(_st(), _p(dy2), _p(x2), _p(w), _p(stats), _p(dx), _p(dw), _p(db), x2.shape[0], cols,
                                     x2.stride(0), dy2.stride(0), dx.stride(0) if dx is not None else cols), "layernorm_bwd")
    return dx.view(x.shape) if dx is not None else None


def rmsnorm_fwd(x, w, eps: float, want_rstd: bool = False, out=None, rstd=None):
    _chk_bf16(x, w)
    cols = x.shape[-1]
    assert x.is_contiguous()
    rows = x.numel() // cols
    y = torch.empty_like(x) if out is None else out
    if want_rstd and rstd is None:
        rstd = torch.empty(rows, device=x.device, dtype=torch.float32)
    N.check(_lib().vla_rmsnorm_fwd(_st(), _p(x), _p(w), _p(y), _p(rstd), rows, cols, eps), "rmsnorm_fwd")
    return (y, rstd) if want_rstd else y


def rmsnorm_fwd_q8(x, w, eps: float, q8: torch.Tensor, qscale: torch.Tensor, rstd: Optional[torch.Tensor] = None, y: Optional[torch.Tensor] = None):
    _chk_bf16(x, w, y)
    cols = x.shape[-1]
    assert x.is_contiguous() and q8.dtype == torch.uint8 and q8.stride(-1) == 1
    rows = x.numel() // cols
    N.check(_lib().vla_rmsnorm_fwd_q8(_st(), _p(x), _p(w), _p(y), _p(rstd), _p(q8), _p(qscale), rows, cols, q8.stride(-2), eps), "rmsnorm_fwd_q8")
    return q8, qscale


def layernorm_fwd_q8(x2, w, b, eps: float, q8: torch.Tensor, qscale: torch.Tensor, y: Optional[torch.Tensor] = None, stats=None):
    _chk_bf16(x2, w, b, y)
    rows, cols = x2.shape
    assert x2.stride(-1) == 1 and q8.dtype == torch.uint8 and q8.stride(-1) == 1
    N.check(_lib().vla_layernorm_fwd_q8(_st(), _p(x2), _p(w), _p(b), _p(y), _p(stats), _p(q8), _p(qscale), rows, cols, x2.stride(0),
                                        y.stride(0) if y is not None else 0, q8.stride(0), eps), "layernorm_fwd_q8")
    return q8, qscale


def rmsnorm_bwd(dy, x, w, rstd, dres=None, out=None, x_rows=None):
    _chk_bf16(dy, x, w, dres)
    cols = x.shape[-1]
    assert x.is_contiguous() and dy.is_contiguous()
    rows = dy.numel() // cols
    g, gr, r0 = x_rows if x_rows is not None else (0, 0, 0)
    if x_rows is None:
        assert x.numel() == dy.numel()
    else:
        assert rows % g == 0 and (rows // g) * gr * cols <= x.numel() and rstd.numel() * cols >= (rows // g) * gr * cols
    dx = torch.empty_like(dy) if out is None else out
    if dres is not None:
        assert dres.is_contiguous() and dres.numel() >= dy.numel()
    N.check(_lib().vla_rmsnorm_bwd(_st(), _p(dy), _p(x), _p(w), _p(rstd), _p(dres), _p(dx), rows, cols, g, gr, r0), "rmsnorm_bwd")
    return dx


def rmsnorm_dw(dy, x, rstd, acc_f32):
    rows, cols = dy.shape
    N.check(_lib().vla_rmsnorm_dw(_st(), _p(dy), _p(x), _p(rstd), _p(acc_f32), rows, cols), "rmsnorm_dw")
    return acc_f32


def _attn_desc(q, k, v, o, lse, kmask, causal, scale, Hq, Hkv, dh):
    d = N.AttnDesc()
    B, Sq, Sk = q.shape[0], q.shape[1], k.shape[1]
    d.q, d.k, d.v, d.o = q.data_ptr(), k.data_ptr(), v.data_ptr(), o.data_ptr()
    d.lse = lse.data_ptr() if lse is not None else None
    d.kmask = kmask.data_ptr() if kmask is not None else None
    d.q_sb, d.k_sb, d.v_sb, d.o_sb = q.stride(0), k.stride(0), v.stride(0), o.stride(0)
    d.q_ss, d.k_ss, d.v_ss, d.o_ss = q.stride(1), k.stride(1), v.stride(1), o.stride(1)
    d.B, d.Sq, d.Sk, d.Hq, d.Hkv, d.dh, d.causal, d.scale = B, Sq, Sk, Hq, Hkv, dh, int(causal), scale
    return d


def attn_fwd(q, k, v, Hq: int, Hkv: int, dh: int, causal: bool, kmask=None, scale: Optional[float] = None,
             want_lse: bool = False, out=None, lse=None):
    _chk_bf16(q, k, v)
    assert q.stride(-1) == 1 and k.stride(-1) == 1 and v.stride(-1) == 1
    B, Sq = q.shape[:2]
    if kmask is not None:
        assert kmask.dtype == torch.uint8 and kmask.is_contiguous() and tuple(kmask.shape) == (B, k.shape[1])
    o = torch.empty(B, Sq, Hq * dh, device=q.device, dtype=BF16) if out is None else out
    if want_lse and lse is None:
        lse = torch.empty(B, Hq, Sq, device=q.device, dtype=torch.float32)
    d = _attn_desc(q, k, v, o, lse, kmask, causal, scale if scale is not None else dh ** -0.5, Hq, Hkv, dh)
    N.check(_lib().vla_attn_fwd(_st(), C.byref(d)), "attn_fwd")
    return (o, lse) if want_lse else o


def attn_bwd(dout, q, k, v, o, lse, Hq: int, Hkv: int, dh: int, causal: bool, kmask=None,
             scale: Optional[float] = None, dq=None, dk=None, dv=None, rope=None, row0: int = 0, delta=None):
    _chk_bf16(dout, q, k, v, o)
    B, Sq, Sk = q.shape[0], q.shape[1], k.shape[1]
    assert Sq + row0 == Sk or row0 == 0
    dq = torch.empty(B, Sq, Hq * dh, device=q.device, dtype=BF16) if dq is None else dq
    dk = torch.empty(B, Sk - row0, Hkv * dh, device=q.device, dtype=BF16) if dk is None else dk
    dv = torch.empty(B, Sk - row0, Hkv * dh, device=q.device, dtype=BF16) if dv is None else dv
    if delta is None:
        delta = torch.empty(B, Hq, Sq, device=q.device, dtype=torch.float32)
    assert delta.dtype == torch.float32 and delta.is_contiguous() and delta.numel() >= B * Hq * Sq
    d = _attn_desc(q, k, v, o, lse, kmask, causal, scale if scale is not None else dh ** -0.5, Hq, Hkv, dh)
    if row0:
        assert causal and row0 % 32 == 0 and lse.shape == (B, Hq, Sk) and lse.is_contiguous()
        d.q_off, d.dkv_k0, d.lse_hs = row0, row0, Sk
        d.lse = lse.data_ptr() + 4 * row0
    d.dout, d.dq, d.dk, d.dv, d.delta = dout.data_ptr(), dq.data_ptr(), dk.data_ptr(), dv.data_ptr(), delta.data_ptr()
    d.do_sb, d.dq_sb, d.dk_sb, d.dv_sb = dout.stride(0), dq.stride(0), dk.stride(0), dv.stride(0)
    d.do_ss, d.dq_ss, d.dk_ss, d.dv_ss = dout.stride(1), dq.stride(1), dk.stride(1), dv.stride(1)
    if rope is not None:
        assert rope[0].shape == (Sk, dh // 2) and rope[0].dtype == torch.float32
        d.rope_cos, d.rope_sin = rope[0].data_ptr(), rope[1].data_ptr()
    N.check(_lib().vla_attn_bwd(_st(), C.byref(d)), "attn_bwd")
    return dq, dk, dv


def rope_half_tables(S: int, dh: int, theta: float, device) -> Tuple[torch.Tensor, torch.Tensor]:
    inv = 1.0 / (theta ** (torch.arange(0, dh, 2, dtype=torch.float32) / dh))
    f = torch.arange(S, dtype=torch.float32)[:, None] * inv[None, :]
    return (f.cos().to(BF16).float().to(device).contiguous(), f.sin().to(BF16).float().to(device).contiguous())


def rope_half_(x2d: torch.Tensor, cos_t, sin_t, S: int, nheads: int, dh: int, sign: int = 1):
    _chk_bf16(x2d)
    assert x2d.stride(-1) == 1 and cos_t.shape == (S, dh // 2)
    N.check(_lib().vla_rope_half(_st(), _p(x2d), _p(cos_t), _p(sin_t), x2d.shape[0], S, nheads, dh, x2d.stride(0), sign),
            "rope_half")
    return x2d


def rope_inter_tables(T: int, dh: int, device, base: float = 10000.0):
    inv = (1.0 / (base ** (torch.arange(0, dh, 2).float() / dh))).to(BF16)
    f = torch.einsum("i,j->ij", torch.arange(T, dtype=BF16), inv)
    e = torch.cat([f, f], dim=-1)
    return (e.cos().float().to(device).contiguous(), e.sin().float().to(device).contiguous())


def rope_inter_(x2d: torch.Tensor, cos_t, sin_t, T: int, nheads: int, dh: int, mode: int = 0):
    _chk_bf16(x2d)
    assert x2d.stride(-1) == 1 and cos_t.shape[0] >= T and cos_t.shape[1] == dh
    N.check(_lib().vla_rope_interleaved(_st(), _p(x2d), _p(cos_t), _p(sin_t), x2d.shape[0], T, nheads, dh, x2d.stride(0),
                                        mode), "rope_interleaved")
    return x2d


def im2col_patch(pixels: torch.Tensor, c0: int, P: int, ldo: int) -> torch.Tensor:
    assert pixels.is_cuda and pixels.is_contiguous() and pixels.dtype in (BF16, torch.float32)
    B, Ct, H, W = pixels.shape
    out = torch.empty(B * (H // P) * (W // P), ldo, device=pixels.device, dtype=BF16)
    N.check(_lib().vla_im2col_patch(_st(), _p(pixels), _p(out), B, Ct, c0, H, W, P, ldo,
                                    int(pixels.dtype == torch.float32)), "im2col_patch")
    return out


def action_mask(labels: torch.Tensor, shift: int):
    assert labels.is_cuda and labels.dtype == torch.int64 and labels.is_contiguous()
    B, L = labels.shape
    qidx = torch.empty(B, L - shift, device=labels.device, dtype=torch.int32)
    pos = torch.empty(B, 64, device=labels.device, dtype=torch.int32)
    cnt = torch.empty(B, device=labels.device, dtype=torch.int32)
    N.check(_lib().vla_action_mask(_st(), _p(labels), _p(qidx), _p(pos), _p(cnt), B, L, shift), "action_mask")
    return qidx, pos, cnt


def embed_splice(ids, attn_mask_u8, qidx, table, action_queries, out, mm_mask, Np: int):
    B, L = ids.shape
    D = table.shape[1]
    assert ids.dtype == torch.int64 and ids.is_contiguous() and out.is_contiguous() and tuple(out.shape) == (B, L + Np, D)
    assert tuple(action_queries.shape) == (64, D) and qidx.shape == (B, L)
    N.check(_lib().vla_embed_splice(_st(), _p(ids), _p(attn_mask_u8), _p(qidx), _p(table), _p(action_queries), _p(out),
                                    _p(mm_mask), B, L, Np, D, table.shape[0]), "embed_splice")


def action_query_grad(dx, pos, Np: int, row0: int = 0) -> torch.Tensor:
    B, S, D = dx.shape
    assert dx.is_contiguous()
    dq = torch.empty(64, D, device=dx.device, dtype=torch.float32)
    N.check(_lib().vla_action_query_grad(_st(), _p(dx), _p(pos), _p(dq), B, S, Np, D, row0), "action_query_grad")
    return dq


def gather_rows(src2d, idx, out2d):
    N.check(_lib().vla_gather_rows(_st(), _p(src2d), _p(idx), _p(out2d), idx.numel(), out2d.shape[-1], src2d.stride(0),
                                   out2d.stride(0)), "gather_rows")
    return out2d


def scatter_add_rows(src2d, idx, out2d):
    N.check(_lib().vla_scatter_add_rows(_st(), _p(src2d), _p(idx), _p(out2d), idx.numel(), src2d.shape[-1], src2d.stride(0),
                                        out2d.stride(0)), "scatter_add_rows")
    return out2d


def add_(a, b):
    assert a.is_contiguous() and b.is_contiguous() and a.numel() == b.numel()
    N.check(_lib().vla_add_bf16(_st(), _p(a), _p(b), _p(a), a.numel()), "add_bf16")
    return a


def gelu_fwd(x, out=None):
    y = torch.empty_like(x) if out is None else out
    N.check(_lib().vla_gelu_fwd(_st(), _p(x), _p(y), x.numel()), "gelu_fwd")
    return y


def gelu_bwd(dy, x, out=None):
    dx = torch.empty_like(x) if out is None else out
    N.check(_lib().vla_gelu_bwd(_st(), _p(dy), _p(x), _p(dx), x.numel()), "gelu_bwd")
    return dx


def relu_bwd(dy, y, out=None):
    dx = torch.empty_like(y) if out is None else out
    N.check(_lib().vla_relu_bwd(_st(), _p(dy), _p(y), _p(dx), y.numel()), "relu_bwd")
    return dx


def swiglu_bwd(dh, gu, out=None):
    M, I = dh.shape
    assert gu.shape == (M, 2 * I) and dh.is_contiguous() and gu.is_contiguous()
    dgu = torch.empty_like(gu) if out is None else out
    N.check(_lib().vla_swiglu_bwd(_st(), _p(dh), _p(gu), _p(dgu), M, I), "swiglu_bwd")
    return dgu


def swiglu_fwd(gu, out=None):
    M, I2 = gu.shape
    assert gu.is_contiguous() and I2 % 32 == 0
    h = torch.empty(M, I2 // 2, device=gu.device, dtype=BF16) if out is None else out
    N.check(_lib().vla_swiglu_fwd(_st(), _p(gu), _p(h), M, I2 // 2), "swiglu_fwd")
    return h


def colsum_(x, out_f32):
    if x.dim() == 3:
        assert out_f32.shape == (x.shape[0], x.shape[2]) and out_f32.stride(-1) == 1 and x.stride(-1) == 1
        N.check(_lib().vla_colsum_bf16(_st(), _p(x), _p(out_f32), x.shape[1], x.shape[2], x.stride(1), x.shape[0], x.stride(0),
                                       out_f32.stride(0)), "colsum")
    else:
        N.check(_lib().vla_colsum_bf16(_st(), _p(x), _p(out_f32), x.shape[0], x.shape[1], x.stride(0), 1, 0, 0), "colsum")
    return out_f32


def cast_f32_bf16(x, out=None):
    y = torch.empty(x.shape, device=x.device, dtype=BF16) if out is None else out
    N.check(_lib().vla_cast_f32_bf16(_st(), _p(x), _p(y), x.numel()), "cast")
    return y


def head_attn_desc(q, ks, vs, ka, va, kt, vt, gate, probs, out, H: int):
    d = N.HeadAttnDesc()
    B, T = q.shape[:2]
    d.q, d.k_self, d.v_self, d.k_adp, d.v_adp, d.k_task, d.v_task = (t.data_ptr() for t in (q, ks, vs, ka, va, kt, vt))
    d.gate, d.probs, d.out = gate.data_ptr(), probs.data_ptr(), out.data_ptr()
    d.B, d.T, d.Ka, d.Kt, d.H, d.dh = B, T, ka.shape[1], kt.shape[1], H, out.shape[-1] // H
    d.ld_q, d.ld_self, d.ld_adp, d.ld_task, d.ld_out = q.stride(1), ks.stride(1), ka.stride(1), kt.stride(1), out.stride(1)
    for t, n in ((vs, ks), (va, ka), (vt, kt)):
        assert t.stride(1) == n.stride(1) and t.stride(-1) == 1
    return d


def head_attn_fwd(q, ks, vs, ka, va, kt, vt, gate, H: int = 8, ref_softmax: bool = False, out=None, probs=None):
    _chk_bf16(q, ks, vs, ka, va, kt, vt, gate)
    B, T = q.shape[:2]
    D = q.shape[-1]
    Nn = T + ka.shape[1] + kt.shape[1]
    out = torch.empty(B, T, D, device=q.device, dtype=BF16) if out is None else out
    probs = torch.empty(B, H, T, Nn, device=q.device, dtype=torch.float32) if probs is None else probs
    d = head_attn_desc(q, ks, vs, ka, va, kt, vt, gate, probs, out, H)
    d.ref_softmax = int(ref_softmax)
    N.check(_lib().vla_head_attn_fwd(_st(), C.byref(d)), "head_attn_fwd")
    return out, probs


def head_attn_bwd(dout, out, q, ks, vs, ka, va, kt, vt, gate, probs, dgate_f32, dq, dks, dvs, dka, dva, dkt, dvt, H: int = 8,
                  rope=None):
    _chk_bf16(dout, out, dq, dks, dvs, dka, dva, dkt, dvt)
    d = head_attn_desc(q, ks, vs, ka, va, kt, vt, gate, probs, out, H)
    d.dout = dout.data_ptr()
    assert dout.stride(1) == out.stride(1) and dout.stride(-1) == 1
    for g, f in ((dq, q), (dks, ks), (dvs, vs), (dka, ka), (dva, va), (dkt, kt), (dvt, vt)):
        assert g.stride(1) == f.stride(1) and g.stride(-1) == 1, "grad views must mirror forward strides"
    d.dq, d.dk_self, d.dv_self, d.dk_adp, d.dv_adp, d.dk_task, d.dv_task = (t.data_ptr() for t in (dq, dks, dvs, dka, dva, dkt, dvt))
    d.dgate = dgate_f32.data_ptr()
    if rope is not None:
        assert rope[0].shape[0] >= max(q.shape[1], ka.shape[1], kt.shape[1]) and rope[0].shape[1] == d.dh
        d.rope_cos, d.rope_sin = rope[0].data_ptr(), rope[1].data_ptr()
    ntile = (d.T + d.Ka + d.Kt + 31) // 32
    ws = _splitk_ws(d.B * d.H * ntile * (d.T * d.dh + 1), q.device)
    d.ws, d.ws_floats = ws.data_ptr(), ws.numel()
    N.check(_lib().vla_head_attn_bwd(_st(), C.byref(d)), "head_attn_bwd")


def l1_loss(pred, target, want_grad: bool = True, gscale: float = 1.0):
    _chk_bf16(pred, target)
    B, Cc, Da = pred.shape
    loss3 = torch.empty(3, device=pred.device, dtype=torch.float32)
    dpred = torch.empty_like(pred) if want_grad else None
    N.check(_lib().vla_l1_loss(_st(), _p(pred.contiguous()), _p(target.contiguous()), _p(loss3), _p(dpred), B, Cc, Da, gscale),
            "l1_loss")
    return loss3, dpred


def adamw_(p, g, m, v, step: int, lr: float, beta1=0.9, beta2=0.999, eps=1e-8, wd=0.01, gscale: float = 1.0):
    assert p.dtype == BF16 and m.dtype == BF16 and v.dtype == BF16 and g.dtype in (BF16, torch.float32)
    assert p.is_contiguous() and g.is_contiguous() and m.is_contiguous() and v.is_contiguous()
    assert p.numel() == g.numel() == m.numel() == v.numel()
    N.check(_lib().vla_adamw_bf16(_st(), _p(p), _p(g), _p(m), _p(v), p.numel(), lr, beta1, beta2, eps, wd, step,
                                  int(g.dtype == torch.float32), gscale), "adamw")


def grad_sumsq_slots(n: int) -> int:
    return int(_lib().vla_grad_sumsq_slots(int(n)))


def grad_sumsq_(g, slots, gscale: float = 1.0) -> int:
    assert g.dtype in (BF16, torch.float32) and g.is_contiguous() and slots.dtype == torch.float32 and slots.is_contiguous()
    k = grad_sumsq_slots(g.numel())
    assert 0 < k <= slots.numel(), "grad_sumsq_: slot buffer too short"
    N.check(_lib().vla_grad_sumsq(_st(), _p(g), g.numel(), int(g.dtype == torch.float32), gscale, _p(slots)), "grad_sumsq")
    return k


def grad_norm_finalise_(slots, max_norm: float, out):
    assert slots.dtype == torch.float32 and slots.is_contiguous() and out.dtype == torch.float32 and out.is_contiguous() and out.numel() >= 2
    N.check(_lib().vla_grad_norm_finalise(_st(), _p(slots), slots.numel(), float(max_norm), _p(out)), "grad_norm_finalise")
    return out


def adamw_clipped_(p, g, m, v, coef, step: int, lr: float, beta1=0.9, beta2=0.999, eps=1e-8, wd=0.01, gscale: float = 1.0):
    assert p.dtype == BF16 and m.dtype == BF16 and v.dtype == BF16 and g.dtype in (BF16, torch.float32)
    assert p.is_contiguous() and g.is_contiguous() and m.is_contiguous() and v.is_contiguous()
    assert p.numel() == g.numel() == m.numel() == v.numel()
    assert coef.dtype == torch.float32 and coef.numel() == 1 and coef.device == p.device
    N.check(_lib().vla_adamw_clipped_bf16(_st(), _p(p), _p(g), _p(m), _p(v), p.numel(), lr, beta1, beta2, eps, wd, step,
                                          int(g.dtype == torch.float32), gscale, _p(coef)), "adamw_clipped")


_DT = {BF16: 0, torch.float32: 1}


def copy2d(src: torch.Tensor, dst: torch.Tensor, rows: int, cols: int, ld_src: int, ld_dst: int, src_mod: int = 0, d_group=None):
    g, gs = d_group if d_group is not None else (0, 0)
    N.check(_lib().vla_copy2d(_st(), _p(src), _p(dst), rows, cols, ld_src, ld_dst, _DT[src.dtype], _DT[dst.dtype], src_mod, g, gs), "copy2d")
    return dst


def quant_fp8_rows(x: torch.Tensor, out: Optional[torch.Tensor] = None, scale: Optional[torch.Tensor] = None):
    assert x.dtype == BF16 and x.dim() == 2 and x.stride(1) == 1
    rows, cols = x.shape
    if out is None:
        out = torch.empty(rows, cols, device=x.device, dtype=torch.uint8)
    if scale is None:
        scale = torch.empty(rows, device=x.device, dtype=torch.float32)
    assert out.dtype == torch.uint8 and out.stride(1) == 1 and tuple(out.shape) == (rows, cols)
    N.check(_lib().vla_quant_fp8_rows(_st(), _p(x), _p(out), _p(scale), rows, cols, x.stride(0), out.stride(0)), "quant_fp8_rows")
    return out, scale


def dropout(x: torch.Tensor, out: torch.Tensor, p: float, seed: int, step: Optional[torch.Tensor] = None):
    _chk_bf16(x, out)
    assert x.dim() == 2 and x.shape == out.shape and x.stride(1) == 1 and out.stride(1) == 1
    N.check(_lib().vla_dropout_bf16(_st(), _p(x), _p(out), x.shape[0], x.shape[1], x.stride(0), out.stride(0), float(p), int(seed) & (2 ** 64 - 1),
                                    _p(step) if step is not None else None), "dropout")
    return out


def dropout_bwd_add_(dx: torch.Tensor, u: torch.Tensor, p: float, seed: int, step: Optional[torch.Tensor] = None):
    _chk_bf16(dx, u)
    assert u.dim() == 2 and u.shape == dx.shape and u.stride(1) == 1 and dx.stride(1) == 1
    N.check(_lib().vla_dropout_bwd_add_bf16(_st(), _p(u), _p(dx), u.shape[0], u.shape[1], u.stride(0), dx.stride(0), float(p), int(seed) & (2 ** 64 - 1),
                                            _p(step) if step is not None else None), "dropout_bwd_add")
    return dx


def inc_i32_(t: torch.Tensor):
    assert t.dtype == torch.int32 and t.numel() >= 1
    N.check(_lib().vla_inc_i32(_st(), _p(t)), "inc_i32")
    return t


def zero_(t: torch.Tensor):
    assert t.is_contiguous()
    N.check(_lib().vla_fill_zero(_st(), _p(t), t.numel() * t.element_size()), "fill_zero")
    return t


def head_index_prep(pos1, pos0, cnt0, gather, scatter, guard, B: int, S: int, Np: int, row0: int):
    N.check(_lib().vla_head_index_prep(_st(), _p(pos1), _p(pos0), _p(cnt0), _p(gather), _p(scatter), _p(guard), B, S, Np, row0), "head_index_prep")


def embed_grad(dx, ids, qidx, out, Np: int):
    B, L = ids.shape
    V, D = out.shape
    N.check(_lib().vla_embed_grad(_st(), _p(dx), _p(ids), _p(qidx), _p(out), B, L, Np, D, V), "embed_grad")
    return out


def token_ce(logits, tgt, out_f32):
    V = logits.shape[-1]
    N.check(_lib().vla_token_ce(_st(), _p(logits), V, _p(tgt), logits.numel() // V, V, _p(out_f32)), "token_ce")
    return out_f32


TOKENIZER_LEN, N_BINS = 151643, 256
TOKEN_METRIC_NAMES = ("action_accuracy", "l1_loss", "next_actions_accuracy", "next_actions_l1_loss")


def token_row_class(labels: torch.Tensor, shift: int = 1, tokenizer_len: int = TOKENIZER_LEN, n_bins: int = N_BINS,
                    action_dim: Optional[int] = None, out: Optional[torch.Tensor] = None):
    from .constants import ACTION_DIM
    assert labels.is_cuda and labels.dtype == torch.int64 and labels.is_contiguous() and labels.dim() == 2
    B, L = labels.shape
    if out is None:
        out = torch.empty(B, L - shift, device=labels.device, dtype=torch.uint8)
    assert out.dtype == torch.uint8 and out.is_contiguous() and out.numel() == B * (L - shift)
    N.check(_lib().vla_token_row_class(_st(), _p(labels), _p(out), B, L, shift, tokenizer_len - (n_bins + 1),
                                       ACTION_DIM if action_dim is None else action_dim), "token_row_class")
    return out


def token_ce_metrics(logits, tgt, row_class, out_f32, counters_u64, pred_ids=None, tokenizer_len: int = TOKENIZER_LEN,
                     n_bins: int = N_BINS, terms: Optional[torch.Tensor] = None):
    _chk_bf16(logits)
    assert logits.dim() == 2 and logits.stride(1) == 1
    rows, V = logits.shape
    assert tgt.dtype == torch.int64 and tgt.is_contiguous() and tgt.numel() == rows
    assert row_class.dtype == torch.uint8 and row_class.is_contiguous() and row_class.numel() == rows
    assert out_f32.dtype == torch.float32 and out_f32.numel() >= 2
    assert counters_u64.dtype in (torch.int64, torch.uint64) and counters_u64.is_contiguous() and counters_u64.numel() == 6
    assert pred_ids is None or (pred_ids.dtype == torch.int32 and pred_ids.is_contiguous() and pred_ids.numel() == rows)
    if terms is not None:
        assert terms.dtype == torch.float32 and terms.is_contiguous() and terms.numel() == rows and terms.device == logits.device
        N.check(_lib().vla_token_ce_metrics_ordered(_st(), _p(logits), logits.stride(0), _p(tgt), _p(row_class), rows, V, _p(out_f32),
                                                    _p(counters_u64), _p(pred_ids), tokenizer_len, n_bins, _p(terms)), "token_ce_metrics_ordered")
        return out_f32
    N.check(_lib().vla_token_ce_metrics(_st(), _p(logits), logits.stride(0), _p(tgt), _p(row_class), rows, V, _p(out_f32),
                                        _p(counters_u64), _p(pred_ids), tokenizer_len, n_bins), "token_ce_metrics")
    return out_f32


def token_metrics_finish(counters, n_bins: int = N_BINS, min_action: float = -1.0, max_action: float = 1.0, out=None) -> dict:
    assert counters.dtype in (torch.int64, torch.uint64) and counters.is_contiguous() and counters.numel() == 6
    if out is None:
        out = torch.empty(4, device=counters.device, dtype=torch.float32)
    assert out.dtype == torch.float32 and out.is_contiguous() and out.numel() == 4
    N.check(_lib().vla_token_metrics_finish(_st(), _p(counters), (max_action - min_action) / (n_bins - 1), _p(out)), "token_metrics_finish")
    return {k: out[i] for i, k in enumerate(TOKEN_METRIC_NAMES)}


def token_ce_bwd(logits, tgt, sums_f32, gscale: float, out):
    V = logits.shape[-1]
    N.check(_lib().vla_token_ce_bwd(_st(), _p(logits), V, _p(tgt), logits.numel() // V, V, _p(sums_f32), gscale, _p(out), V),
            "token_ce_bwd")
    return out


def add_scalar_f32_(x: torch.Tensor, s: torch.Tensor):
    N.check(_lib().vla_add_scalar_f32(_st(), _p(x), _p(s), x.numel()), "add_scalar_f32")
    return x


def image_normalize_u8_(img_u8: torch.Tensor, out: torch.Tensor, c0: int, mean, std):
    assert img_u8.dtype == torch.uint8 and img_u8.is_contiguous() and img_u8.dim() == 4 and img_u8.shape[-1] == 3
    B, H, W, _ = img_u8.shape
    assert out.is_contiguous() and out.shape[0] == B and tuple(out.shape[2:]) == (H, W) and out.dtype in (BF16, torch.float32)
    m3, s3 = (C.c_float * 3)(*[float(x) for x in mean]), (C.c_float * 3)(*[float(x) for x in std])
    N.check(_lib().vla_image_normalize_u8(_st(), _p(img_u8), _p(out), B, H, W, out.shape[1], c0, m3, s3,
                                          int(out.dtype == torch.float32)), "image_normalize_u8")
    return out


AUG_CROP, AUG_BRIGHTNESS, AUG_CONTRAST, AUG_SATURATION, AUG_HUE, AUG_DRAW = 1, 2, 4, 8, 16, 32
AUG_NPARAM = 9
AUG_P_U, AUG_P_Y1, AUG_P_X1, AUG_P_Y2, AUG_P_X2, AUG_P_BRIGHT, AUG_P_CONTRAST, AUG_P_SAT, AUG_P_HUE = range(9)


def image_augment_normalize_(frames_u8: torch.Tensor, out: torch.Tensor, norms, ops_mask: int, cfg7, params: torch.Tensor,
                             seed: int = 0, rank: int = 0, step: int = 0, frames_out: Optional[torch.Tensor] = None):
    assert frames_u8.dtype == torch.uint8 and frames_u8.is_contiguous() and frames_u8.dim() == 5 and frames_u8.shape[-1] == 3
    B, n_img, H, W, _ = frames_u8.shape
    nb = len(norms)
    assert out.is_contiguous() and tuple(out.shape) == (B, 3 * nb * n_img, H, W) and out.dtype in (BF16, torch.float32)
    assert params.dtype == torch.float32 and params.is_contiguous() and tuple(params.shape) == (B * n_img, AUG_NPARAM)
    assert frames_out is None or (frames_out.dtype == torch.uint8 and frames_out.is_contiguous() and frames_out.shape == frames_u8.shape)
    mean = (C.c_float * (3 * nb))(*[float(x) for mu, _ in norms for x in mu])
    std = (C.c_float * (3 * nb))(*[float(x) for _, sd in norms for x in sd])
    cfg = (C.c_float * 7)(*[float(x) for x in cfg7])
    n = B * n_img
    slab = None
    if ops_mask & AUG_CONTRAST:
        slab = torch.empty(_lib().vla_augment_slab_floats(n, H, W), device=frames_u8.device, dtype=torch.float32)
        N.check(_lib().vla_augment_stats(_st(), _p(frames_u8), _p(params), _p(slab), n, H, W, n_img, ops_mask, cfg, seed, rank, step),
                "augment_stats")
    N.check(_lib().vla_augment_apply(_st(), _p(frames_u8), _p(params), _p(slab), _p(out), _p(frames_out), n, H, W, n_img, nb, mean, std,
                                     int(out.dtype == torch.float32), ops_mask, cfg, seed, rank, step), "augment_apply")
    return out


def action_tokenize(actions_f32: torch.Tensor, bins_f64: torch.Tensor, tokenizer_len: int, lo: float = -1.0, hi: float = 1.0):
    assert actions_f32.dtype == torch.float32 and actions_f32.is_contiguous() and bins_f64.dtype == torch.float64 and bins_f64.is_contiguous()
    ids = torch.empty(actions_f32.shape, device=actions_f32.device, dtype=torch.int64)
    N.check(_lib().vla_action_tokenize(_st(), _p(actions_f32), _p(bins_f64), _p(ids), actions_f32.numel(), bins_f64.numel(), lo, hi,
                                       tokenizer_len), "action_tokenize")
    return ids


def normalize_bounds(x_f32: torch.Tensor, low: torch.Tensor, high: torch.Tensor, mask: Optional[torch.Tensor] = None,
                     zero_mask: Optional[torch.Tensor] = None):
    D = x_f32.shape[-1]
    assert x_f32.dtype == torch.float32 and x_f32.is_contiguous() and x_f32.numel() > 0
    for t, dt in ((low, torch.float32), (high, torch.float32), (mask, torch.uint8), (zero_mask, torch.uint8)):
        assert t is None or (t.dtype == dt and t.is_contiguous() and t.numel() == D and t.device == x_f32.device), "per-dimension statistics: [D] on x's device"
    out = torch.empty_like(x_f32)
    N.check(_lib().vla_normalize_bounds(_st(), _p(x_f32), _p(out), x_f32.numel(), D, _p(low), _p(high), _p(mask), _p(zero_mask)), "normalize_bounds")
    return out


def collate_tokens(prompt_flat: torch.Tensor, prompt_off: torch.Tensor, actions_f32: torch.Tensor, bins_f64: torch.Tensor, L: int, *,
                   tokenizer_len: int, lo: float = -1.0, hi: float = 1.0, pad_id: int, ignore_index: int = -100, num_tokens: int = 64,
                   seed: int = 0, rank: int = 0, step: int = 0):
    B, n_act = actions_f32.shape
    dev = actions_f32.device
    assert actions_f32.dtype == torch.float32 and actions_f32.is_contiguous() and bins_f64.dtype == torch.float64 and bins_f64.is_contiguous()
    assert prompt_flat.dtype == torch.int64 and prompt_flat.is_contiguous() and prompt_flat.dim() == 1
    assert prompt_off.dtype == torch.int32 and prompt_off.is_contiguous() and tuple(prompt_off.shape) == (B + 1,)
    assert prompt_flat.device == dev and prompt_off.device == dev and bins_f64.device == dev
    assert L > 0
    ids, labels = torch.empty(B, L, device=dev, dtype=torch.int64), torch.empty(B, L, device=dev, dtype=torch.int64)
    am = torch.empty(B, L, device=dev, dtype=torch.uint8)
    N.check(_lib().vla_collate_tokens(_st(), _p(prompt_flat) if prompt_flat.numel() else None, _p(prompt_off), prompt_flat.numel(), _p(actions_f32),
                                      _p(bins_f64), _p(ids), _p(labels), _p(am), B, n_act, L, bins_f64.numel(), lo, hi, tokenizer_len, pad_id,
                                      ignore_index, num_tokens, int(seed) & (2 ** 64 - 1), int(rank), int(step)), "collate_tokens")
    return ids, labels, am


def serve_tokens(prompt_flat: torch.Tensor, prompt_off: torch.Tensor, L: int, *, pad_id: int, num_tokens: int = 64, fill_id: int = 1,
                 stop_id: int = 2, action_label: int = 151387, ignore_index: int = -100):
    B, dev = prompt_off.numel() - 1, prompt_off.device
    assert prompt_flat.dtype == torch.int64 and prompt_flat.is_contiguous() and prompt_flat.dim() == 1
    assert prompt_off.dtype == torch.int32 and prompt_off.is_contiguous() and prompt_off.dim() == 1 and B >= 1
    assert prompt_flat.device == dev and prompt_off.is_cuda
    if L < num_tokens + 2:
        raise ValueError(f"serve_tokens: L = {L} cannot hold one prompt id, {num_tokens} placeholders and the stop id")
    ids, labels = torch.empty(B, L, device=dev, dtype=torch.int64), torch.empty(B, L, device=dev, dtype=torch.int64)
    am = torch.empty(B, L, device=dev, dtype=torch.uint8)
    hid_row, row_ok = torch.empty(B, device=dev, dtype=torch.int32), torch.empty(B, device=dev, dtype=torch.uint8)
    N.check(_lib().vla_serve_tokens(_st(), _p(prompt_flat) if prompt_flat.numel() else None, _p(prompt_off), prompt_flat.numel(), _p(ids),
                                    _p(labels), _p(am), _p(hid_row), _p(row_ok), B, int(L), num_tokens, fill_id, stop_id, action_label, pad_id,
                                    ignore_index), "serve_tokens")
    return ids, labels, am, hid_row, row_ok


def _chk_stats64(D, dev, low, high, mask):
    for t, dt in ((low, torch.float64), (high, torch.float64), (mask, torch.uint8)):
        assert t is None or (t.dtype == dt and t.is_contiguous() and t.numel() == D and t.device == dev), "per-dimension statistics: [D] on the operand's device"


def normalize_proprio_serve(x: torch.Tensor, low: torch.Tensor, high: torch.Tensor, mask: Optional[torch.Tensor] = None) -> torch.Tensor:
    D = x.shape[-1]
    assert x.is_cuda and x.dtype in (torch.float32, torch.float64) and x.is_contiguous() and x.numel() > 0
    _chk_stats64(D, x.device, low, high, mask)
    out = torch.empty(x.shape, device=x.device, dtype=torch.float32)
    N.check(_lib().vla_normalize_proprio_serve(_st(), _p(x), int(x.dtype == torch.float64), _p(out), x.numel(), D, _p(low), _p(high), _p(mask)),
            "normalize_proprio_serve")
    return out


def unnormalize_actions(pred: torch.Tensor, low: torch.Tensor, high: torch.Tensor, mask: Optional[torch.Tensor] = None,
                        row_ok: Optional[torch.Tensor] = None, out: Optional[torch.Tensor] = None) -> torch.Tensor:
    _chk_bf16(pred)
    B, Da = pred.shape[0], low.numel()
    p2 = pred.reshape(B, -1) if pred.dim() != 2 else pred
    assert p2.stride(1) == 1 and p2.shape[1] % Da == 0
    _chk_stats64(Da, pred.device, low, high, mask)
    assert row_ok is None or (row_ok.dtype == torch.uint8 and row_ok.is_contiguous() and row_ok.numel() == B and row_ok.device == pred.device)
    if out is None:
        out = torch.empty(pred.shape, device=pred.device, dtype=torch.float64)
    o2 = out.view(B, -1) if out.dim() != 2 else out
    assert out.dtype == torch.float64 and o2.stride(1) == 1 and o2.shape == p2.shape
    N.check(_lib().vla_unnormalize_actions(_st(), _p(p2), _p(o2), B, p2.shape[1], Da, p2.stride(0), o2.stride(0), _p(low), _p(high), _p(mask),
                                           _p(row_ok)), "unnormalize_actions")
    return out


def serve_gather_hidden(hs: torch.Tensor, hid_row: torch.Tensor, Np: int, T: int = 64, out: Optional[torch.Tensor] = None) -> torch.Tensor:
    _chk_bf16(hs)
    B, S, D = hs.shape
    assert hs.stride(2) == 1 and hid_row.dtype == torch.int32 and hid_row.is_contiguous() and hid_row.numel() == B and hid_row.device == hs.device
    if out is None:
        out = torch.empty(B, 1, T, D, device=hs.device, dtype=BF16)
    assert out.is_contiguous() and out.numel() == B * T * D and out.dtype == BF16
    N.check(_lib().vla_serve_gather_hidden(_st(), _p(hs), _p(hid_row), _p(out), B, S, Np, T, D, hs.stride(0), hs.stride(1)), "serve_gather_hidden")
    return out


def episode_sample(valid_off: torch.Tensor, episode_off: torch.Tensor, prompt_off: torch.Tensor, seed: int, rank: int, world: int, step: int,
                   Pmax: int, ep: torch.Tensor, row: torch.Tensor, out_off: torch.Tensor) -> None:
    E, B, dev = valid_off.numel() - 1, ep.numel(), valid_off.device
    for t, dt, n in ((valid_off, torch.int64, E + 1), (episode_off, torch.int64, E + 1), (prompt_off, torch.int32, E + 1), (ep, torch.int32, B),
                     (row, torch.int64, B), (out_off, torch.int32, B + 1)):
        assert t.is_cuda and t.device == dev and t.dtype == dt and t.dim() == 1 and t.numel() == n and t.is_contiguous(), "episode_sample: bad operand"
    N.check(_lib().vla_episode_sample(_st(), _p(valid_off), _p(episode_off), _p(prompt_off), E, int(seed) & (2 ** 64 - 1), int(rank), int(world),
                                      int(step), B, int(Pmax), _p(ep), _p(row), _p(out_off)), "episode_sample")


def episode_gather(frames: torch.Tensor, actions: torch.Tensor, proprio: torch.Tensor, episode_off: torch.Tensor, prompt_flat: torch.Tensor,
                   prompt_off: torch.Tensor, ep: torch.Tensor, row: torch.Tensor, out_off: torch.Tensor, out_frames: torch.Tensor,
                   out_actions: torch.Tensor, out_proprio: torch.Tensor, out_prompt: torch.Tensor, Pmax: int) -> None:
    B, E, T, dev = ep.numel(), episode_off.numel() - 1, frames.shape[0], frames.device
    chunk, A, Pd = out_actions.shape[1], actions.shape[1], proprio.shape[1]
    row_bytes = frames[0].numel()
    for t in (frames, actions, proprio, episode_off, prompt_flat, prompt_off, ep, row, out_off, out_frames, out_actions, out_proprio, out_prompt):
        assert t.is_cuda and t.device == dev and t.is_contiguous(), "episode_gather: operands are contiguous tensors on one device"
    assert frames.dtype == torch.uint8 and out_frames.dtype == torch.uint8 and tuple(out_frames.shape) == (B,) + tuple(frames.shape[1:])
    assert actions.dtype == torch.float32 and tuple(actions.shape) == (T, A) and out_actions.dtype == torch.float32 and tuple(out_actions.shape) == (B, chunk, A)
    assert proprio.dtype == torch.float32 and tuple(proprio.shape) == (T, Pd) and out_proprio.dtype == torch.float32 and tuple(out_proprio.shape) == (B, Pd)
    assert episode_off.dtype == torch.int64 and prompt_off.dtype == torch.int32 and prompt_off.numel() == E + 1 and prompt_flat.dtype == torch.int64
    assert ep.dtype == torch.int32 and row.dtype == torch.int64 and row.numel() == B and out_off.dtype == torch.int32 and out_off.numel() == B + 1
    assert out_prompt.dtype == torch.int64 and out_prompt.numel() == B * Pmax
    N.check(_lib().vla_episode_gather(_st(), _p(frames), _p(actions), _p(proprio), _p(episode_off), _p(prompt_flat) if prompt_flat.numel() else None,
                                      _p(prompt_off), _p(ep), _p(row), _p(out_off), _p(out_frames), _p(out_actions), _p(out_proprio),
                                      _p(out_prompt) if out_prompt.numel() else None, B, E, T, row_bytes, chunk, A, Pd, prompt_flat.numel(), int(Pmax)),
            "episode_gather")


def mixture_sample(valid_off: torch.Tensor, episode_off: torch.Tensor, prompt_off: torch.Tensor, dataset_off: torch.Tensor,
                   quota_off: torch.Tensor, seed: int, rank: int, world: int, step: int, Pmax: int, ds: torch.Tensor, ep: torch.Tensor,
                   row: torch.Tensor, out_off: torch.Tensor) -> None:
    E, D, B, dev = valid_off.numel() - 1, dataset_off.numel() - 1, ep.numel(), valid_off.device
    for t, dt, n in ((valid_off, torch.int64, E + 1), (episode_off, torch.int64, E + 1), (prompt_off, torch.int32, E + 1),
                     (dataset_off, torch.int32, D + 1), (quota_off, torch.int64, D + 1), (ds, torch.int32, B), (ep, torch.int32, B),
                     (row, torch.int64, B), (out_off, torch.int32, B + 1)):
        assert t.is_cuda and t.device == dev and t.dtype == dt and t.dim() == 1 and t.numel() == n and t.is_contiguous(), "mixture_sample: bad operand"
    N.check(_lib().vla_mixture_sample(_st(), _p(valid_off), _p(episode_off), _p(prompt_off), _p(dataset_off), _p(quota_off), E, D,
                                      int(seed) & (2 ** 64 - 1), int(rank), int(world), int(step), B, int(Pmax), _p(ds), _p(ep), _p(row),
                                      _p(out_off)), "mixture_sample")


def normalize_bounds_rows(x_f32: torch.Tensor, sel: torch.Tensor, low: torch.Tensor, high: torch.Tensor, mask: Optional[torch.Tensor] = None,
                          zero_mask: Optional[torch.Tensor] = None):
    R, D = x_f32.shape[0], x_f32.shape[-1]
    assert x_f32.dim() >= 2 and x_f32.dtype == torch.float32 and x_f32.is_contiguous() and x_f32.numel() > 0
    assert low.dim() == 2 and low.shape[1] == D, "per-set statistics: [n_sets, D]"
    n_sets, dev = low.shape[0], x_f32.device
    assert sel.dtype == torch.int32 and sel.is_contiguous() and tuple(sel.shape) == (R,) and sel.device == dev, "sel: int32 [R] on x's device"
    for t, dt in ((low, torch.float32), (high, torch.float32), (mask, torch.uint8), (zero_mask, torch.uint8)):
        assert t is None or (t.dtype == dt and t.is_contiguous() and tuple(t.shape) == (n_sets, D) and t.device == dev), \
            "per-set statistics: [n_sets, D] on x's device"
    out = torch.empty_like(x_f32)
    N.check(_lib().vla_normalize_bounds_rows(_st(), _p(x_f32), _p(out), R, x_f32.numel() // R, D, _p(sel), n_sets, _p(low), _p(high), _p(mask),
                                             _p(zero_mask)), "normalize_bounds_rows")
    return out


def heldout_sweep(val_off: torch.Tensor, episode_off: torch.Tensor, prompt_off: torch.Tensor, dataset_off: Optional[torch.Tensor], rank: int,
                  world: int, batch_j: int, stride: int, Pmax: int, ds: torch.Tensor, ep: torch.Tensor, row: torch.Tensor, out_off: torch.Tensor,
                  valid: torch.Tensor) -> None:
    E, B, dev = val_off.numel() - 1, ep.numel(), val_off.device
    D = 1 if dataset_off is None else dataset_off.numel() - 1
    for t, dt, n in ((val_off, torch.int64, E + 1), (episode_off, torch.int64, E + 1), (prompt_off, torch.int32, E + 1),
                     (dataset_off, torch.int32, D + 1), (ds, torch.int32, B), (ep, torch.int32, B), (row, torch.int64, B),
                     (out_off, torch.int32, B + 1), (valid, torch.uint8, B)):
        assert t is None or (t.is_cuda and t.device == dev and t.dtype == dt and t.dim() == 1 and t.numel() == n and t.is_contiguous()), \
            "heldout_sweep: bad operand"
    N.check(_lib().vla_heldout_sweep(_st(), _p(val_off), _p(episode_off), _p(prompt_off), _p(dataset_off), E, D, int(rank), int(world),
                                     int(batch_j), int(stride), B, int(Pmax), _p(ds), _p(ep), _p(row), _p(out_off), _p(valid)), "heldout_sweep")


def heldout_l1_accumulate(pred: torch.Tensor, target: torch.Tensor, ds: Optional[torch.Tensor], valid: torch.Tensor, acc: torch.Tensor,
                          cnt: torch.Tensor) -> None:
    _chk_bf16(pred, target)
    B, Cc, A = pred.shape
    D, dev = acc.shape[0], pred.device
    assert pred.is_contiguous() and target.is_contiguous() and tuple(target.shape) == (B, Cc, A) and target.device == dev
    assert acc.dtype == torch.float64 and acc.is_contiguous() and tuple(acc.shape) == (D, Cc, A) and acc.device == dev
    assert cnt.dtype == torch.int64 and cnt.is_contiguous() and tuple(cnt.shape) == (D,) and cnt.device == dev
    assert valid.dtype == torch.uint8 and valid.is_contiguous() and tuple(valid.shape) == (B,) and valid.device == dev
    assert ds is None or (ds.dtype == torch.int32 and ds.is_contiguous() and tuple(ds.shape) == (B,) and ds.device == dev)
    N.check(_lib().vla_heldout_l1_accumulate(_st(), _p(pred), _p(target), _p(ds), _p(valid), B, Cc, A, D, _p(acc), _p(cnt)), "heldout_l1_accumulate")


_DIGEST_SCRATCH = {}


def state_digest(t: torch.Tensor, salt: int = 0, out: Optional[torch.Tensor] = None, scratch: Optional[torch.Tensor] = None) -> torch.Tensor:
    assert t.is_cuda and t.element_size() == 2 and t.is_contiguous(), f"state_digest: a contiguous CUDA tensor of 16-bit elements, got {t.dtype} {t.device}"
    n = t.numel()
    if n == 0:
        raise ValueError("state_digest: an empty view has no digest")
    if out is None:
        out = torch.empty(1, device=t.device, dtype=torch.int64)
    assert out.dtype == torch.int64 and out.numel() == 1 and out.device == t.device, "state_digest: out is int64 [1] on t's device"
    if scratch is None:
        scratch = _DIGEST_SCRATCH.get(t.device)
        if scratch is None:
            scratch = _DIGEST_SCRATCH[t.device] = torch.empty(_lib().vla_state_digest_slots(), device=t.device, dtype=torch.int64)
    assert scratch.dtype == torch.int64 and scratch.is_contiguous() and scratch.device == t.device and scratch.numel() >= 1
    N.check(_lib().vla_state_digest(_st(), _p(t), n, int(salt) & (2 ** 64 - 1), _p(scratch), scratch.numel(), _p(out)), "state_digest")
    return out


def digest_value(d) -> int:
    return int(d.item() if isinstance(d, torch.Tensor) else d) & (2 ** 64 - 1)
```

Baseline: 1312.

## Fuse bias column-sums into weight-gradient TN GEMMs and group them into one launch

Adds a colsum variant of the TN GEMM kernels that reduces the A-operand tile already staged in LDS into per-column bias gradients, so the separate colsum passes no longer reread the activation gradients from memory. It also adds a persistent grouped launcher that covers batched, accumulating and row-grouped problems and can cap workgroups, and the adapter backward batches its weight-gradient GEMMs through it. In exchange the GEMM inner loop gains extra LDS reads and adds, a cross-wave reduction at the end, and a bias round trip through bf16 where the old path accumulated in fp32 buffers.

```diff
diff --git a/include/vla_gemm_tn_bias.h b/include/vla_gemm_tn_bias.h
--- /dev/null
+++ b/include/vla_gemm_tn_bias.h
@@ -0,0 +1,18 @@
+#ifndef VLA_GEMM_TN_BIAS_H
+#define VLA_GEMM_TN_BIAS_H
+
+#include "vla_native.h"
+
+#ifdef __cplusplus
+extern "C" {
+#endif
+
+int vla_gemm_bf16_tn_colsum(void* stream, const vla_gemm_tn_desc* desc , void* colsum, long long colsum_stride);
+
+int vla_gemm_bf16_tn_grouped_ex(void* stream, const vla_gemm_tn_desc* descs , int count, void* const* colsum ,
+                                const long long* colsum_stride , int max_workgroups);
+
+#ifdef __cplusplus
+}
+#endif
+#endif
diff --git a/vla_adapter_amd/csrc/gemm_tn.hip b/vla_adapter_amd/csrc/gemm_tn.hip
--- a/vla_adapter_amd/csrc/gemm_tn.hip
+++ b/vla_adapter_amd/csrc/gemm_tn.hip
@@ -1,6 +1,8 @@
 #include <algorithm>
+#include <vector>
 #include "gemm_epilogue.h"
 #include "gemm_params.h"
+#include "../../include/vla_gemm_tn_bias.h"
 
 namespace {
 
@@ -17,14 +19,30 @@
   int gA, gB; long long sgA, sgB;
   int cgA, cgsA;
   int tiles_n2, ntiles, split, mslice;
+  bf16_t* cs; long long sCs; int cs_acc; float* wcs;
 };
+
+__device__ __forceinline__ unsigned cs_word(const char* tile, int r, int lane) {
+  const int f = ((r & 3) << 2) | ((r >> 2) & 3);
+  return *reinterpret_cast<const unsigned*>(tile + 256 * r + (((lane >> 2) ^ f) << 4) + ((lane & 3) << 2));
+}
+__device__ __forceinline__ void cs_store(const TnP& p, int bz, int zb, int c, float s) {
+  if (p.wcs != nullptr) { p.wcs[(long long)bz * p.N1 + c] = s; return; }
+  bf16_t* o = p.cs + (long long)zb * p.sCs + c;
+  float v = rbf(s);
+  if (p.cs_acc) v += bf2f(*o);
+  *o = f2bf(v);
+}
 
 __device__ __forceinline__ bf16x4 tr_read(const char* p) {
   return __builtin_amdgcn_ds_read_tr16_b64_v4i16((__attribute__((address_space(3))) bf16x4*)p);
 }
 
+template <bool CS>
 __device__ __forceinline__ void tn_tile(const TnP& p, const int swz, const int bz, char* smem) {
-  const int tid = threadIdx.x, lane = tid & 63;
+  int tid = threadIdx.x;
+  if (CS) asm volatile("" : "+v"(tid));
+  const int lane = tid & 63;
   const int wid = __builtin_amdgcn_readfirstlane(tid >> 6);
   const int wr = wid >> 2, wc = wid & 3;
   const int b1 = swz / p.tiles_n2, b2 = swz - b1 * p.tiles_n2;
@@ -79,6 +97,8 @@
 #pragma unroll
     for (int b = 0; b < 4; ++b) acc[a][b] = f32x4{0.f, 0.f, 0.f, 0.f};
 
+  const bool docs = CS && p.cs != nullptr && b2 == 0;
+  float cs0 = 0.f, cs1 = 0.f;
   if (nt > 0) stage(0, 0);
   int buf = 0;
   for (int t = 0; t < nt; ++t) {
@@ -88,6 +108,13 @@
     if (t + 1 < nt) stage(buf ^ 1, t + 1);
     const char* sb = smem + buf * STAGE_BYTES;
     const int valid = m_end - (m_begin + t * TBK);
+    if (CS && docs) {
+#pragma unroll
+      for (int j = 0; j < 8; ++j) {
+        const unsigned w = cs_word(sb, wid * 8 + j, lane);
+        if (wid * 8 + j < valid) { cs0 += bf_lo(w); cs1 += bf_hi(w); }
+      }
+    }
     bf16x8 fm[2][4], fn[2][2];
 #pragma unroll
     for (int ks = 0; ks < 2; ++ks) {
@@ -122,6 +149,18 @@
     buf ^= 1;
   }
 
+  if (CS && docs) {
+    float* sc = reinterpret_cast<float*>(smem);
+    __syncthreads();
+    sc[wid * 128 + 2 * lane] = cs0; sc[wid * 128 + 2 * lane + 1] = cs1;
+    __syncthreads();
+    if (tid < 128 && n1_0 + tid < p.N1) {
+      float s = sc[tid];
+#pragma unroll
+      for (int w = 1; w < 8; ++w) s += sc[w * 128 + tid];
+      cs_store(p, bz, zb, n1_0 + tid, s);
+    }
+  }
   const int w1 = n1_0 + wr * 64, w2 = n2_0 + wc * 32;
   const int lq = lane >> 4, lr = lane & 15;
   if (p.ws != nullptr) {
@@ -162,8 +201,11 @@
           Q[ni][mi] = __builtin_amdgcn_mfma_f32_16x16x32_bf16(FN[ks][ni], FM[ks][mi], Q[ni][mi], 0, 0, 0);     \
   } while (0)
 
+template <bool CS>
 __device__ __forceinline__ void tn256_tile(const TnP& p, const int swz, const int zb, char* smem) {
-  const int tid = threadIdx.x, lane = tid & 63;
+  int tid = threadIdx.x;
+  if (CS) asm volatile("" : "+v"(tid));
+  const int lane = tid & 63;
   const int wid = __builtin_amdgcn_readfirstlane(tid >> 6);
   const int wr = wid >> 2, wc = wid & 3;
   const int b1 = swz / p.tiles_n2, b2 = swz - b1 * p.tiles_n2;
@@ -264,6 +306,9 @@
 #pragma unroll
         for (int e = 0; e < 4; ++e) acc[a][b][c][e] = f32x4{0.f, 0.f, 0.f, 0.f};
 
+  const bool docs = CS && p.cs != nullptr && b2 == 0;
+  float csum[2][2] = {{0.f, 0.f}, {0.f, 0.f}};
+  unsigned csw[8];
   bf16x8 fm[2][4], fn0[2][2], fn1[2][2];
   int d = 0;
   for (int t = 0; t < nt; ++t) {
@@ -274,6 +319,10 @@
       read_b(kb + 0 * T2_HT, fn0);
       read_a(kb + 1 * T2_HT, fm);
       read_b(kb + 2 * T2_HT, fn1);
+      if (CS && docs) {
+#pragma unroll
+        for (int j = 0; j < 8; ++j) csw[j] = cs_word(kb + 1 * T2_HT, wid * 8 + j, lane);
+      }
       __builtin_amdgcn_sched_barrier(0);
       if (t + 1 < nt) {
         stage_a(sn + 3, 1, t + 1);
@@ -286,12 +335,21 @@
       VLA_BARRIER();
       __builtin_amdgcn_s_setprio(1);
       TN_MMA_QUADRANT(acc[0][0], fn0, fm);
+      if (CS && docs) {
+#pragma unroll
+        for (int j = 0; j < 8; ++j)
+          if (wid * 8 + j < valid) { csum[0][0] += bf_lo(csw[j]); csum[0][1] += bf_hi(csw[j]); }
+      }
       TN_MMA_QUADRANT(acc[0][1], fn1, fm);
       __builtin_amdgcn_s_setprio(0);
       VLA_BARRIER();
     }
     {
       read_a(kb + 3 * T2_HT, fm);
+      if (CS && docs) {
+#pragma unroll
+        for (int j = 0; j < 8; ++j) csw[j] = cs_word(kb + 3 * T2_HT, wid * 8 + j, lane);
+      }
       __builtin_amdgcn_sched_barrier(0);
       if (t + 2 < nt) {
         stage_b(so + 0, 0, t + 2); stage_a(so + 1, 0, t + 2); stage_b(so + 2, 1, t + 2);
@@ -305,6 +363,11 @@
       VLA_BARRIER();
       __builtin_amdgcn_s_setprio(1);
       TN_MMA_QUADRANT(acc[1][1], fn1, fm);
+      if (CS && docs) {
+#pragma unroll
+        for (int j = 0; j < 8; ++j)
+          if (wid * 8 + j < valid) { csum[1][0] += bf_lo(csw[j]); csum[1][1] += bf_hi(csw[j]); }
+      }
       TN_MMA_QUADRANT(acc[1][0], fn0, fm);
       __builtin_amdgcn_s_setprio(0);
       VLA_BARRIER();
@@ -312,6 +375,22 @@
     d ^= 1;
   }
   if (wr == 0) VLA_BARRIER();
+
+  if (CS && docs) {
+    float* sc = reinterpret_cast<float*>(smem);
+#pragma unroll
+    for (int h = 0; h < 2; ++h) {
+      const int tc = ((2 * lane) >> 6) * 128 + h * 64 + ((2 * lane) & 63);
+      sc[wid * 256 + tc] = csum[h][0]; sc[wid * 256 + tc + 1] = csum[h][1];
+    }
+    __syncthreads();
+    if (tid < 256 && n1_0 + tid < p.N1) {
+      float s = sc[tid];
+#pragma unroll
+      for (int w = 1; w < 8; ++w) s += sc[w * 256 + tid];
+      cs_store(p, zb, zb, n1_0 + tid, s);
+    }
+  }
 
   const int lq = lane >> 4, lr = lane & 15;
   bf16_t* Cb = p.C + (long long)zb * p.sC;
@@ -336,12 +415,22 @@
 
 __global__ __launch_bounds__(512) void gemm_tn256_kernel(TnP p) {
   extern __shared__ __attribute__((aligned(16))) char smem[];
-  tn256_tile(p, xcd_order(blockIdx.x, p.ntiles), blockIdx.z, smem);
+  tn256_tile<false>(p, xcd_order(blockIdx.x, p.ntiles), blockIdx.z, smem);
 }
 
 __global__ __launch_bounds__(512) void gemm_tn_kernel(TnP p) {
   extern __shared__ __attribute__((aligned(16))) char smem[];
-  tn_tile(p, xcd_order(blockIdx.x, p.ntiles), blockIdx.z, smem);
+  tn_tile<false>(p, xcd_order(blockIdx.x, p.ntiles), blockIdx.z, smem);
+}
+
+__global__ __launch_bounds__(512) void gemm_tn256_cs_kernel(TnP p) {
+  extern __shared__ __attribute__((aligned(16))) char smem[];
+  tn256_tile<true>(p, xcd_order(blockIdx.x, p.ntiles), blockIdx.z, smem);
+}
+
+__global__ __launch_bounds__(512, 4) void gemm_tn_cs_kernel(TnP p) {
+  extern __shared__ __attribute__((aligned(16))) char smem[];
+  tn_tile<true>(p, xcd_order(blockIdx.x, p.ntiles), blockIdx.z, smem);
 }
 
 constexpr int TN_GROUP_MAX = 48;
@@ -366,7 +455,8 @@
   p.gA = p.gB = 0; p.sgA = p.sgB = 0;
   p.cgA = g.cgA; p.cgsA = g.cgsA;
   p.tiles_n2 = g.tiles_n2; p.ntiles = 0; p.split = 1; p.mslice = g.M;
-  tn_tile(p, t - G.start[pi], 0, smem);
+  p.cs = nullptr; p.sCs = 0; p.cs_acc = 0; p.wcs = nullptr;
+  tn_tile<false>(p, t - G.start[pi], 0, smem);
 }
 
 __global__ __launch_bounds__(512) void gemm_tn256_grouped_kernel(TnGroup G) {
@@ -383,7 +473,49 @@
   p.gA = p.gB = 0; p.sgA = p.sgB = 0;
   p.cgA = g.cgA; p.cgsA = g.cgsA;
   p.tiles_n2 = g.tiles_n2; p.ntiles = 0; p.split = 1; p.mslice = g.M;
-  tn256_tile(p, t - G.start[pi], 0, smem);
+  p.cs = nullptr; p.sCs = 0; p.cs_acc = 0; p.wcs = nullptr;
+  tn256_tile<false>(p, t - G.start[pi], 0, smem);
+}
+
+constexpr int TNX_GROUP_MAX = 16;
+struct TnGX {
+  const bf16_t* A; const bf16_t* B; bf16_t* C; bf16_t* cs;
+  long long sA, sB, sC, sCs, sgB;
+  int M, N1, N2, lda, ldb, ldc, cgA, cgsA, gB, tiles_n2, ntiles, acc;
+  float alpha;
+};
+struct TnGroupX { TnGX g[TNX_GROUP_MAX]; int start[TNX_GROUP_MAX + 1]; int count, total; };
+
+template <int TILE>
+__device__ __forceinline__ void tn_groupx_walk(const TnGroupX& G, char* smem) {
+  for (int v = blockIdx.x; v < G.total; v += gridDim.x) {
+    int pi = 0;
+    while (pi + 1 < G.count && v >= G.start[pi + 1]) ++pi;
+    const TnGX& g = G.g[pi];
+    const int local = xcd_order(v - G.start[pi], G.start[pi + 1] - G.start[pi]), zb = local / g.ntiles;
+    TnP p;
+    p.A = g.A; p.B = g.B; p.C = g.C; p.R = g.acc ? g.C : nullptr; p.ws = nullptr;
+    p.M = g.M; p.N1 = g.N1; p.N2 = g.N2; p.lda = g.lda; p.ldb = g.ldb; p.ldc = g.ldc; p.ldr = g.ldc;
+    p.sA = g.sA; p.sB = g.sB; p.sC = g.sC; p.sR = g.sC;
+    p.alpha = g.alpha;
+    p.gA = 0; p.gB = g.gB; p.sgA = 0; p.sgB = g.sgB;
+    p.cgA = g.cgA; p.cgsA = g.cgsA;
+    p.tiles_n2 = g.tiles_n2; p.ntiles = g.ntiles; p.split = 1; p.mslice = g.M;
+    p.cs = g.cs; p.sCs = g.sCs; p.cs_acc = g.acc; p.wcs = nullptr;
+    if constexpr (TILE == 256) tn256_tile<true>(p, local - zb * g.ntiles, zb, smem);
+    else tn_tile<true>(p, local - zb * g.ntiles, zb, smem);
+    if (v + (int)gridDim.x < G.total) __syncthreads();
+  }
+}
+
+__global__ __launch_bounds__(512, 4) void gemm_tn_groupx_kernel(TnGroupX G) {
+  extern __shared__ __attribute__((aligned(16))) char smem[];
+  tn_groupx_walk<128>(G, smem);
+}
+
+__global__ __launch_bounds__(512) void gemm_tn256_groupx_kernel(TnGroupX G) {
+  extern __shared__ __attribute__((aligned(16))) char smem[];
+  tn_groupx_walk<256>(G, smem);
 }
 
 constexpr int TN256_MIN_TILES = 128;
@@ -429,9 +561,31 @@
   }
 }
 
-}
-
-extern "C" int vla_gemm_bf16_tn(void* stream, const vla_gemm_tn_desc* d) {
+__global__ void tn_colsum_finalize_kernel(const float* __restrict__ wcs, bf16_t* __restrict__ cs, int N1, long long sCs, int split, int acc) {
+  const int b = blockIdx.y, c = blockIdx.x * blockDim.x + threadIdx.x;
+  if (c >= N1) return;
+  const float* w = wcs + (long long)b * split * N1 + c;
+  float s = w[0];
+  for (int i = 1; i < split; ++i) s += w[(long long)i * N1];
+  bf16_t* o = cs + b * sCs + c;
+  float v = rbf(s);
+  if (acc) v += bf2f(*o);
+  *o = f2bf(v);
+}
+
+int launch_tn(void* stream, const vla_gemm_tn_desc* d, void* colsum, long long colsum_stride);
+
+}
+
+extern "C" int vla_gemm_bf16_tn(void* stream, const vla_gemm_tn_desc* d) { return launch_tn(stream, d, nullptr, 0); }
+
+extern "C" int vla_gemm_bf16_tn_colsum(void* stream, const vla_gemm_tn_desc* d, void* colsum, long long colsum_stride) {
+  VLA_REQUIRE(colsum && ((uintptr_t)colsum & 1) == 0, "gemm_tn_colsum: null / unaligned colsum");
+  return launch_tn(stream, d, colsum, colsum_stride);
+}
+
+namespace {
+int launch_tn(void* stream, const vla_gemm_tn_desc* d, void* colsum, long long colsum_stride) {
   VLA_REQUIRE(d && d->A && d->B && d->C, "gemm_tn: null operand");
   VLA_REQUIRE(d->M > 0 && d->N1 > 0 && d->N2 > 0 && d->batch > 0, "gemm_tn: empty problem");
   VLA_REQUIRE(d->N1 % 8 == 0 && d->N2 % 8 == 0, "gemm_tn: N1 and N2 must be multiples of 8 (16-B column chunks)");
@@ -449,6 +603,7 @@
   const int split = pl.split;
   if (split > 1)
     VLA_REQUIRE(d->ws && ((uintptr_t)d->ws & 15) == 0 && d->N2 % 4 == 0, "gemm_tn: split needs an fp32 workspace [batch, split, N1, N2]");
+  if (colsum && d->R) VLA_REQUIRE(d->R == d->C, "gemm_tn_colsum: an addend must be C itself (accumulation): the column sums accumulate with it");
   TnP p;
   p.A = (const bf16_t*)d->A; p.B = (const bf16_t*)d->B; p.C = (bf16_t*)d->C; p.R = (const bf16_t*)d->R;
   p.ws = split > 1 ? d->ws : nullptr;
@@ -461,24 +616,106 @@
   p.ntiles = ((d->N1 + 127) / 128) * p.tiles_n2;
   p.split = split;
   p.mslice = split > 1 ? ((d->M + split - 1) / split + TBK - 1) / TBK * TBK : d->M;
+  p.cs = (bf16_t*)colsum; p.sCs = colsum_stride; p.cs_acc = d->R != nullptr;
+  p.wcs = colsum && split > 1 ? d->ws + (long long)d->batch * split * d->N1 * d->N2 : nullptr;
   hipStream_t st = (hipStream_t)stream;
   if (pl.kernel == VLA_KERNEL_TN_256) {
-    if (int rc = vla_lds_limit<gemm_tn256_kernel>(T2_LDS, "gemm_tn256_kernel")) return rc;
     p.tiles_n2 = (d->N2 + 255) / 256;
     p.ntiles = ((d->N1 + 255) / 256) * p.tiles_n2;
-    hipLaunchKernelGGL(gemm_tn256_kernel, dim3(p.ntiles, 1, d->batch), dim3(512), T2_LDS, st, p);
+    if (colsum) {
+      if (int rc = vla_lds_limit<gemm_tn256_cs_kernel>(T2_LDS, "gemm_tn256_cs_kernel")) return rc;
+      hipLaunchKernelGGL(gemm_tn256_cs_kernel, dim3(p.ntiles, 1, d->batch), dim3(512), T2_LDS, st, p);
+    } else {
+      if (int rc = vla_lds_limit<gemm_tn256_kernel>(T2_LDS, "gemm_tn256_kernel")) return rc;
+      hipLaunchKernelGGL(gemm_tn256_kernel, dim3(p.ntiles, 1, d->batch), dim3(512), T2_LDS, st, p);
+    }
     VLA_CHECK_LAUNCH("gemm_bf16_tn (256)");
     return VLA_OK;
   }
-  if (int rc = vla_lds_limit<gemm_tn_kernel>(LDS_BYTES, "gemm_tn_kernel")) return rc;
-  hipLaunchKernelGGL(gemm_tn_kernel, dim3(p.ntiles, 1, d->batch * split), dim3(512), LDS_BYTES, st, p);
+  if (colsum) {
+    if (int rc = vla_lds_limit<gemm_tn_cs_kernel>(LDS_BYTES, "gemm_tn_cs_kernel")) return rc;
+    hipLaunchKernelGGL(gemm_tn_cs_kernel, dim3(p.ntiles, 1, d->batch * split), dim3(512), LDS_BYTES, st, p);
+  } else {
+    if (int rc = vla_lds_limit<gemm_tn_kernel>(LDS_BYTES, "gemm_tn_kernel")) return rc;
+    hipLaunchKernelGGL(gemm_tn_kernel, dim3(p.ntiles, 1, d->batch * split), dim3(512), LDS_BYTES, st, p);
+  }
   VLA_CHECK_LAUNCH("gemm_bf16_tn");
+  if (split > 1 && colsum) {
+    hipLaunchKernelGGL(tn_colsum_finalize_kernel, dim3((d->N1 + 255) / 256, d->batch), dim3(256), 0, st, (const float*)p.wcs, p.cs, d->N1,
+                       colsum_stride, split, p.cs_acc);
+    VLA_CHECK_LAUNCH("gemm_tn_colsum_finalize");
+  }
   if (split > 1) {
     const long long total = (long long)d->N1 * d->N2 / 4;
     const unsigned nblk = (unsigned)((total + 255) / 256 < 1024 ? (total + 255) / 256 : 1024);
     hipLaunchKernelGGL(tn_finalize_kernel, dim3(nblk, d->batch), dim3(256), 0, st, (const float*)d->ws, (const bf16_t*)d->R, (bf16_t*)d->C,
                        d->N1, d->N2, d->ldc, d->ldr, d->sC, d->sR, p.alpha, split);
     VLA_CHECK_LAUNCH("gemm_tn_finalize");
+  }
+  return VLA_OK;
+}
+}
+
+extern "C" int vla_gemm_bf16_tn_grouped_ex(void* stream, const vla_gemm_tn_desc* descs, int count, void* const* colsum,
+                                           const long long* colsum_stride, int max_workgroups) {
+  VLA_REQUIRE(descs && count > 0 && max_workgroups >= 0, "gemm_tn_grouped_ex: no problems / negative workgroup limit");
+  const int forced = tn_forced();
+  auto on256 = [&](const vla_gemm_tn_desc* d) { return plan_tn(d, 0, forced, false).kernel == VLA_KERNEL_TN_256; };
+  for (int i = 0; i < count; ++i) {
+    const vla_gemm_tn_desc* d = descs + i;
+    VLA_REQUIRE(d->A && d->B && d->C && d->M > 0 && d->N1 > 0 && d->N2 > 0 && d->batch > 0, "gemm_tn_grouped_ex: null operand / empty problem");
+    VLA_REQUIRE(d->split <= 1 && d->a_group == 0, "gemm_tn_grouped_ex: no contraction split, no row groups on A");
+    VLA_REQUIRE(!d->R || (d->R == d->C && d->ldr == d->ldc && d->sR == d->sC), "gemm_tn_grouped_ex: an addend must be C itself (accumulation)");
+    VLA_REQUIRE(d->N1 % 8 == 0 && d->N2 % 8 == 0 && d->lda % 8 == 0 && d->ldb % 8 == 0 && d->ldc % 4 == 0, "gemm_tn_grouped_ex: N1, N2, lda, ldb % 8, ldc % 4");
+    VLA_REQUIRE(((uintptr_t)d->A & 15) == 0 && ((uintptr_t)d->B & 15) == 0 && ((uintptr_t)d->C & 7) == 0, "gemm_tn_grouped_ex: alignment");
+    VLA_REQUIRE(d->sA % 8 == 0 && d->sB % 8 == 0 && d->sC % 4 == 0, "gemm_tn_grouped_ex: batch strides must keep the alignment");
+    VLA_REQUIRE(d->b_group >= 0 && d->b_group % 64 == 0 && d->b_group_stride % 8 == 0, "gemm_tn_grouped_ex: row groups on B must be multiples of 64 rows");
+    VLA_REQUIRE(d->a_col_group >= 0 && d->a_col_group % 8 == 0 && d->a_col_group_stride % 8 == 0 &&
+                    (d->a_col_group == 0 || d->a_col_group_stride >= d->a_col_group), "gemm_tn_grouped_ex: bad column groups");
+    if (colsum && colsum[i]) VLA_REQUIRE(((uintptr_t)colsum[i] & 1) == 0 && colsum_stride, "gemm_tn_grouped_ex: unaligned colsum / no strides");
+  }
+  std::vector<int> order(count);
+  for (int i = 0; i < count; ++i) order[i] = i;
+  std::stable_sort(order.begin(), order.end(), [&](int a, int b) { return descs[a].M > descs[b].M; });
+  for (int k = 1; k >= 0; --k) {
+    const int tile = k ? 256 : 128;
+    TnGroupX G;
+    int cnt = 0, total = 0;
+    auto flush = [&]() -> int {
+      if (cnt == 0) return VLA_OK;
+      G.start[cnt] = total; G.count = cnt; G.total = total;
+      const int grid = max_workgroups > 0 ? std::min(total, max_workgroups) : total;
+      if (k == 1) {
+        if (int rc = vla_lds_limit<gemm_tn256_groupx_kernel>(T2_LDS, "gemm_tn256_groupx_kernel")) return rc;
+        hipLaunchKernelGGL(gemm_tn256_groupx_kernel, dim3(grid), dim3(512), T2_LDS, (hipStream_t)stream, G);
+      } else {
+        if (int rc = vla_lds_limit<gemm_tn_groupx_kernel>(LDS_BYTES, "gemm_tn_groupx_kernel")) return rc;
+        hipLaunchKernelGGL(gemm_tn_groupx_kernel, dim3(grid), dim3(512), LDS_BYTES, (hipStream_t)stream, G);
+      }
+      VLA_CHECK_LAUNCH("gemm_bf16_tn_grouped_ex");
+      cnt = 0; total = 0;
+      return VLA_OK;
+    };
+    for (int oi = 0; oi < count; ++oi) {
+      const int i = order[oi];
+      const vla_gemm_tn_desc* d = descs + i;
+      if ((on256(d) ? 1 : 0) != k) continue;
+      TnGX& g = G.g[cnt];
+      g.A = (const bf16_t*)d->A; g.B = (const bf16_t*)d->B; g.C = (bf16_t*)d->C;
+      g.cs = colsum ? (bf16_t*)colsum[i] : nullptr;
+      g.sA = d->sA; g.sB = d->sB; g.sC = d->sC; g.sCs = g.cs ? colsum_stride[i] : 0; g.sgB = d->b_group_stride;
+      g.M = d->M; g.N1 = d->N1; g.N2 = d->N2; g.lda = d->lda; g.ldb = d->ldb; g.ldc = d->ldc;
+      g.cgA = d->a_col_group; g.cgsA = d->a_col_group_stride; g.gB = d->b_group;
+      g.tiles_n2 = (d->N2 + tile - 1) / tile;
+      g.ntiles = ((d->N1 + tile - 1) / tile) * g.tiles_n2;
+      g.acc = d->R != nullptr;
+      g.alpha = d->alpha == 0.f ? 1.f : d->alpha;
+      G.start[cnt] = total;
+      total += g.ntiles * d->batch;
+      if (++cnt == TNX_GROUP_MAX)
+        if (int rc = flush()) return rc;
+    }
+    if (int rc = flush()) return rc;
   }
   return VLA_OK;
 }
diff --git a/vla_adapter_amd/engine.py b/vla_adapter_amd/engine.py
--- a/vla_adapter_amd/engine.py
+++ b/vla_adapter_amd/engine.py
@@ -553,6 +553,7 @@
         self._prep_key = None
         self.rope_tab = None
         self.ref_softmax = bool(int(os.environ.get("VLA_HEAD_REF_SOFTMAX", "0")))
+        self.dw_max_workgroups = int(os.environ.get("VLA_HEAD_DW_WORKGROUPS", "0"))
 
     _BLK_PRO = [("q_proj", "w_x", "b_x", 0), ("k_self", "w_x", "b_x", 1), ("v_self", "w_x", "b_x", 2),
                 ("k_adapter", "w_adp", "b_adp", 0), ("v_adapter", "w_adp", "b_adp", 1),
@@ -653,7 +654,7 @@
         self.dO2, self.dFF = e(nb, R, D), e(nb, R, D)
         self.probs = e(nb, B, self.H, T, T + Ka + Kt, dt=torch.float32)
         self.stats = e(nb, R, 2, dt=torch.float32)
-        bkeys = tuple(k for k in ("b_x", "b_adp", "b_task", "b_o", "b_ffn", "fc1_b", "fc2_b", "p_fc1_b", "p_fc2_b") if k in self.P.offsets)
+        bkeys = tuple(k for k in (() if self.pro else ("b_x",)) + ("fc1_b", "fc2_b", "p_fc1_b", "p_fc2_b") if k in self.P.offsets)
         shapes = [("dgate", (nb,)), ("ln_dw", (nb, D)), ("ln_db", (nb, D)), ("ln1_dw", (self.Din,)), ("ln1_db", (self.Din,)),
                   ("ln2_dw", (D,)), ("ln2_db", (D,)), ("d_pf", (B, D))] + [("b:" + k, tuple(self.P.offsets[k][1])) for k in bkeys]
         self.acc32 = z(sum(rup(math.prod(sh), 4) for _, sh in shapes), dt=torch.float32)
@@ -832,20 +833,21 @@
             for i in range(nb):
                 ops.copy_rows3d(self.HSref[i + 1], self.h_task_c[i], B, Kt, D, S * D, D, Kt * D, D)
             h_task, tg = self.h_task_c, None
-        ops.gemm_tn(self.dQKVx, self.X[:nb], out=G("w_x"))
-        ops.gemm_tn(self.dO2, self.AOx, out=G("w_o"))
-        ops.gemm_tn(self.dFF, self.LNo, out=G("w_ffn"))
-        ops.colsum_(self.dQKVx, self.b_f32["b_x"]); ops.colsum_(self.dO2, self.b_f32["b_o"]); ops.colsum_(self.dFF, self.b_f32["b_ffn"])
+        tp = ops.tn_problem
+        probs = ops.TnProblems([tp(self.dQKVx, self.X[:nb], G("w_x"), colsum=G("b_x") if self.pro else None),
+                                tp(self.dO2, self.AOx, G("w_o"), colsum=G("b_o")), tp(self.dFF, self.LNo, G("w_ffn"), colsum=G("b_ffn"))])
+        probs.max_workgroups = self.dw_max_workgroups
         if self.pro:
-            ops.gemm_tn(self.dKV_adp, h_adp, out=G("w_adp"))
-            ops.gemm_tn(self.dKV_task, h_task, out=G("w_task"), rows=B * Kt, b_group=tg)
-            ops.colsum_(self.dKV_adp, self.b_f32["b_adp"]); ops.colsum_(self.dKV_task, self.b_f32["b_task"])
-        else:
+            probs.append(tp(self.dKV_adp, h_adp, G("w_adp"), colsum=G("b_adp")))
+            probs.append(tp(self.dKV_task, h_task, G("w_task"), rows=B * Kt, b_group=tg, colsum=G("b_task")))
+            ops.gemm_tn_grouped(probs)
+        else:
+            ops.gemm_tn_grouped(probs)
             gkv = G("w_x")[:, self.D:]
             ops.gemm_tn(self.dKV_adp, h_adp, out=gkv, accumulate=True)
             ops.gemm_tn(self.dKV_task, h_task, out=gkv, accumulate=True, rows=B * Kt, b_group=tg)
             bkv = self.b_f32["b_x"][:, self.D:]
-            ops.colsum_(self.dKV_adp, bkv); ops.colsum_(self.dKV_task, bkv)
+            ops.colsum_(self.dQKVx, self.b_f32["b_x"]); ops.colsum_(self.dKV_adp, bkv); ops.colsum_(self.dKV_task, bkv)
         for k, t in self.b_f32.items():
             ops.cast_f32_bf16(t, out=G(k))
         ops.cast_f32_bf16(self.ln_dw, out=G("ln_w")); ops.cast_f32_bf16(self.ln_db, out=G("ln_b"))
diff --git a/vla_adapter_amd/native.py b/vla_adapter_amd/native.py
--- a/vla_adapter_amd/native.py
+++ b/vla_adapter_amd/native.py
@@ -177,6 +177,12 @@
 }
 DIGEST_SYMBOLS = sorted(DIGEST_PROTOS)
 
+TN_BIAS_PROTOS = {
+    "vla_gemm_bf16_tn_colsum": ([_P, C.POINTER(GemmTnDesc), _P, _L], _I),
+    "vla_gemm_bf16_tn_grouped_ex": ([_P, C.POINTER(GemmTnDesc), _I, C.POINTER(C.c_void_p), C.POINTER(C.c_longlong), _I], _I),
+}
+TN_BIAS_SYMBOLS = sorted(TN_BIAS_PROTOS)
+
 _lib = None
 
 
@@ -189,7 +195,7 @@
             f"{LIB_PATH} not found: build it with `python -c 'import __graft_entry__ as g; g.build()'` "
             f"(or `make -C {os.path.join(_HERE, 'csrc')}`).  There is no CPU/PyTorch fallback.")
     lib = C.CDLL(LIB_PATH)
-    for name, (args, res) in list(_PROTOS.items()) + list(SERVE_PROTOS.items()) + list(EPISODE_PROTOS.items()) + list(MIXTURE_PROTOS.items()) + list(HELDOUT_PROTOS.items()) + list(DIGEST_PROTOS.items()):
+    for name, (args, res) in list(_PROTOS.items()) + list(SERVE_PROTOS.items()) + list(EPISODE_PROTOS.items()) + list(MIXTURE_PROTOS.items()) + list(HELDOUT_PROTOS.items()) + list(DIGEST_PROTOS.items()) + list(TN_BIAS_PROTOS.items()):
         fn = getattr(lib, name, None)
         if fn is None:
             raise NativeLibraryMissing(f"{LIB_PATH} does not export {name}: it was built from an older source tree, rebuild (make -C csrc)")
diff --git a/vla_adapter_amd/ops.py b/vla_adapter_amd/ops.py
--- a/vla_adapter_amd/ops.py
+++ b/vla_adapter_amd/ops.py
@@ -191,8 +191,9 @@
 
 
 def gemm_tn(a: torch.Tensor, b: torch.Tensor, *, out: Optional[torch.Tensor] = None, alpha: float = 1.0, accumulate: bool = False,
-            a_group=None, b_group=None, a_cols=None, rows: Optional[int] = None, split: Optional[int] = None) -> torch.Tensor:
-    _chk_bf16(a, b, out)
+            a_group=None, b_group=None, a_cols=None, rows: Optional[int] = None, split: Optional[int] = None,
+            colsum: Optional[torch.Tensor] = None) -> torch.Tensor:
+    _chk_bf16(a, b, out, colsum)
     assert a.stride(-1) == 1 and b.stride(-1) == 1 and a.dim() == b.dim()
     batched = a.dim() == 3
     nb = a.shape[0] if batched else 1
@@ -227,11 +228,15 @@
         split = split_c.value
     if split and split > 1:
         key = (torch.cuda.current_stream().cuda_stream, str(a.device))
-        need = nb * split * N1 * N2
+        need = nb * split * N1 * (N2 + (1 if colsum is not None else 0))
         ws = _TN_WS.get(key)
         if ws is None or ws.numel() < need:
             ws = _TN_WS[key] = torch.empty(max(need, 4 << 20), device=a.device, dtype=torch.float32)
         d.split, d.ws = split, ws.data_ptr()
+    if colsum is not None:
+        assert tuple(colsum.shape) == ((nb, N1) if batched else (N1,)) and colsum.stride(-1) == 1
+        N.check(_lib().vla_gemm_bf16_tn_colsum(_st(), C.byref(d), _p(colsum), colsum.stride(0) if batched else 0), "gemm_bf16_tn_colsum")
+        return out
     N.check(_lib().vla_gemm_bf16_tn(_st(), C.byref(d)), "gemm_bf16_tn")
     return out
 
@@ -239,23 +244,51 @@
 TN_GROUP_MAX = 48
 
 
-def tn_problem(a: torch.Tensor, b: torch.Tensor, out: torch.Tensor, alpha: float = 1.0, a_cols=None) -> "N.GemmTnDesc":
-    _chk_bf16(a, b, out)
-    assert a.dim() == 2 and b.dim() == 2 and a.stride(1) == 1 and b.stride(1) == 1 and out.stride(1) == 1 and a.shape[0] == b.shape[0]
+def tn_problem(a: torch.Tensor, b: torch.Tensor, out: torch.Tensor, alpha: float = 1.0, a_cols=None, accumulate: bool = False,
+               b_group=None, rows: Optional[int] = None, colsum: Optional[torch.Tensor] = None) -> "N.GemmTnDesc":
+    _chk_bf16(a, b, out, colsum)
+    assert a.dim() == b.dim() == out.dim() and a.dim() in (2, 3) and a.stride(-1) == 1 and b.stride(-1) == 1 and out.stride(-1) == 1
+    batched = a.dim() == 3
+    nb = a.shape[0] if batched else 1
+    M = rows if rows is not None else a.shape[-2]
+    assert rows is not None or b.shape[-2] == M
     d = N.GemmTnDesc()
-    N1, a_ptr = a.shape[1], a.data_ptr()
+    N1, a_ptr = a.shape[-1], a.data_ptr()
     if a_cols is not None:
         N1, cg, cgs, off = a_cols
         d.a_col_group, d.a_col_group_stride = cg, cgs
         a_ptr += off * 2
-    assert tuple(out.shape) == (N1, b.shape[1]), f"out shape {tuple(out.shape)} != {(N1, b.shape[1])}"
+    shape = (nb, N1, b.shape[-1]) if batched else (N1, b.shape[-1])
+    assert tuple(out.shape) == shape, f"out shape {tuple(out.shape)} != {shape}"
     d.A, d.B, d.C = a_ptr, b.data_ptr(), out.data_ptr()
-    d.M, d.N1, d.N2, d.lda, d.ldb, d.ldc, d.batch, d.alpha = a.shape[0], N1, b.shape[1], a.stride(0), b.stride(0), out.stride(0), 1, alpha
-    d._keep = (a, b, out)
+    d.M, d.N1, d.N2, d.lda, d.ldb, d.ldc, d.batch, d.alpha = M, N1, b.shape[-1], a.stride(-2), b.stride(-2), out.stride(-2), nb, alpha
+    d.sA, d.sB, d.sC = (a.stride(0), b.stride(0), out.stride(0)) if batched else (0, 0, 0)
+    if accumulate:
+        d.R, d.ldr, d.sR = out.data_ptr(), out.stride(-2), d.sC
+    if b_group is not None:
+        d.b_group, d.b_group_stride = b_group
+    if colsum is not None:
+        assert tuple(colsum.shape) == ((nb, N1) if batched else (N1,)) and colsum.stride(-1) == 1
+    d._colsum = colsum
+    d._ex = batched or accumulate or b_group is not None or colsum is not None
+    d._keep = (a, b, out, colsum)
     return d
 
 
-def gemm_tn_grouped(problems):
+class TnProblems(list):
+    max_workgroups = 0
+
+
+def gemm_tn_grouped(problems, max_workgroups: Optional[int] = None):
+    if max_workgroups is None:
+        max_workgroups = getattr(problems, "max_workgroups", 0)
+    if max_workgroups > 0 or any(getattr(d, "_ex", False) for d in problems):
+        n = len(problems)
+        arr = (N.GemmTnDesc * n)(*problems)
+        cs = (C.c_void_p * n)(*[None if getattr(d, "_colsum", None) is None else d._colsum.data_ptr() for d in problems])
+        st = (C.c_longlong * n)(*[d._colsum.stride(0) if getattr(d, "_colsum", None) is not None and d._colsum.dim() == 2 else 0 for d in problems])
+        N.check(_lib().vla_gemm_bf16_tn_grouped_ex(_st(), arr, n, cs, st, max_workgroups), "gemm_bf16_tn_grouped_ex")
+        return
     for i in range(0, len(problems), TN_GROUP_MAX):
         chunk = problems[i:i + TN_GROUP_MAX]
         arr = (N.GemmTnDesc * len(chunk))(*chunk)
```

After: 1316, median of 6. No clear change (+0.3%).
